# honglianghe/CDNet

Hardware: AMD Instinct MI355X
Metric: tiles/sec (train fwd+bwd+Adam), 256x256 (higher is better)
Workload: dtype fp32

## Files before the change

### cdnet_amd/_lib.py

```python
import ctypes as C
import os

_HERE = os.path.dirname(os.path.abspath(__file__))
LIB_PATH = os.environ.get('CDNET_LIB_PATH') or os.path.join(_HERE, 'libcdnet_hip.so')

_vp, _i, _sz, _f, _u = C.c_void_p, C.c_int, C.c_size_t, C.c_float, C.c_uint

class WgradReduceDesc(C.Structure):
    _fields_ = [('slab', C.c_void_p), ('dw', C.c_void_p)] + [(n, C.c_int) for n in (
        'ksplit', 'npar', 'ci_blocks', 'co_blocks', 'taps', 'CI', 'CO', 'Csrc_real', 'Cin_real', 'src_coff', 'Cout', 'mode', 'block0', 'blocks')]


SIGNATURES = {
    'cdnet_abi_version': (_i, []),
    'cdnet_abi_sizeof': (_sz, [C.c_char_p]),
    'cdnet_last_error': (C.c_char_p, []),
    'cdnet_build_info': (C.c_char_p, []),
    'cdnet_spin': (_i, [_i, _vp]),
    'cdnet_box_copy': (_i, [_vp, _vp, _sz, _vp]),
    'cdnet_box_mfma': (_i, [_vp, _vp, _vp, _i, _i, _i, _vp]),
    'cdnet_ddm_codes': (_i, [_vp, _i, _i, _i, _i, _vp, _i, _i, _vp, _vp, _vp]),
    'cdnet_ddm_normalize': (_i, [_vp, _vp, _i, _i, _i, _vp, _vp]),
    'cdnet_probmaps': (_i, [_vp, _vp, _i, _i, _i, _i, _vp, _vp, _vp]),
    'cdnet_tta_boost_argmax': (_i, [_vp, _vp, _vp, _vp, _i, _i, _vp, _i, _i, _vp, _vp, _vp, _vp, _vp, _vp]),
    'cdnet_fuse_sum': (_i, [_vp, _i, _i, _i, _i, _i, _i, _vp, _i, _i, _vp]),
    'cdnet_upsample_bilinear_backward': (_i, [_vp, _i, _i, _i, _i, _i, _i, _i, _i, _vp, _vp]),
    'cdnet_s2d_to_nhwc': (_i, [_vp, _i, _i, _i, _i, _vp, _vp]),
    'cdnet_fuse_sum_f32': (_i, [_vp, _i, _i, _i, _i, _i, _i, _vp, _i, _i, _vp]),
    'cdnet_upsample_bilinear_backward_f32': (_i, [_vp, _i, _i, _i, _i, _i, _i, _i, _i, _vp, _vp]),
    'cdnet_s2d_to_nhwc_f32': (_i, [_vp, _i, _i, _i, _i, _vp, _vp]),
    'cdnet_bn_backward_stats': (_i, [_vp, _vp, _vp, _vp, _vp, _sz, _vp, _vp]),
    'cdnet_bn_backward_apply': (_i, [_vp, _vp, _vp, _vp]),
    'cdnet_bn_backward_finalize': (_i, [_vp, _vp, _vp, _vp, _vp, _i, _vp, _vp]),
    'cdnet_conv_ws_eligible': (_i, [_vp]),
    'cdnet_grad_sum': (_i, [_vp, _i, _vp, C.c_longlong, _i, _vp, _vp]),
    'cdnet_grad_sum_f32': (_i, [_vp, _i, _vp, C.c_longlong, _i, _vp, _vp]),
    'cdnet_label_pair_histogram': (_i, [_vp, _vp, _i, _i, _i, _i, _vp, _vp, _vp, _vp, _vp, _vp]),
    'cdnet_remap_label': (_i, [_vp, _i, _i, _i, _vp, _vp, _vp, _vp]),
    'cdnet_label_areas': (_i, [_vp, _i, _i, _i, _vp, _vp, _vp]),
    'cdnet_label_apply': (_i, [_vp, _i, _i, _i, _vp, _vp, _vp]),
    'cdnet_label_csr_workspace_bytes': (_sz, [_i]),
    'cdnet_label_csr': (_i, [_vp, _i, _i, _i, _vp, _sz, _vp, _vp, _vp, _vp, _vp]),
    'cdnet_hausdorff_tile_pixels': (_i, []),
    'cdnet_hausdorff_chunk_pixels': (_i, []),
    'cdnet_hausdorff_pairs': (_i, [_vp] * 8 + [_i, _i, _i, _vp, _i, _vp, _i, _vp, _vp, _vp]),
    'cdnet_watershed_workspace_bytes': (_sz, [_i, _i, _i]),
    'cdnet_watershed_process': (_i, [_vp, _i, _i, _i, _i, _vp, _sz, _vp, _vp, _vp, _vp]),
    'cdnet_fill_label_process': (_i, [_vp, _i, _i, _i, _i, _vp, _sz, _vp, _vp]),
    'cdnet_label_process': (_i, [_vp, _i, _i, _i, _i, _vp, _sz, _vp, _vp]),
    'cdnet_instance_redilate_workspace_bytes': (_sz, [_i, _i, _i, _i]),
    'cdnet_instance_redilate': (_i, [_vp, _i, _i, _i, _i, _i, _vp, _sz, _vp, _vp, _vp]),
    'cdnet_instance_redilate_lds_rows': (_i, []),
    'cdnet_instance_redilate_lds_cols': (_i, []),
    'cdnet_label_count': (_i, [_vp, _i, _i, _i, _vp, _vp, _vp, _vp]),
    'cdnet_tile_postproc_workspace_bytes': (_sz, [_i, _i, _i, _i]),
    'cdnet_tile_postproc': (_i, [_vp, _vp, _vp, _i, _i, _i, _i, _vp, _i, _i, _i, _i, _vp, _sz] + [_vp] * 10),
    'cdnet_cc_workspace_bytes': (_sz, [_i, _i, _i]),
    'cdnet_cc_chain': (_i, [_vp, _i, _i, _i, _i, _i, _i, _vp, _sz, _vp, _vp, _vp, _vp, _vp, _vp]),
    'cdnet_mask_views_argmax': (_i, [_vp, _i, _i, _i, _vp, _i, _i, _vp, _vp, _vp]),
    'cdnet_tile_mask_postproc_workspace_bytes': (_sz, [_i, _i, _i, _i]),
    'cdnet_tile_mask_postproc': (_i, [_vp, _i, _i, _i, _i, _i, _i, _vp, _sz] + [_vp] * 8),
    'cdnet_dilate_labels': (_i, [_vp, _i, _i, _i, _i, _vp, _vp]),
    'cdnet_conv_packed_weight_elems': (_sz, [_i] * 6),
    'cdnet_pack_conv_weights': (_i, [_vp, _vp] + [_i] * 7 + [_vp]),
    'cdnet_pack_conv_weights_scaled': (_i, [_vp, _vp, _vp] + [_i] * 7 + [_vp]),
    'cdnet_pack_batch_table_bytes': (_sz, [_i]),
    'cdnet_pack_conv_weights_batch': (_i, [_vp, _i, _vp, _sz, _i, _vp]),
    'cdnet_conv_forward': (_i, [_vp, _vp]),
    'cdnet_src_materialize': (_i, [_vp, _i, _i, _i, _vp, _vp]),
    'cdnet_input_pack': (_i, [_vp, _i, _i, _i, _i, _vp, _vp]),
    'cdnet_input_pack_f32': (_i, [_vp, _i, _i, _i, _i, _vp, _vp]),
    'cdnet_bn_fold_eval': (_i, [_vp, _vp, _vp, _vp, _vp, _f, _i, _vp, _vp, _vp]),
    'cdnet_bn_finalize_train': (_i, [_vp, _i, _i, _f, _vp, _vp, _vp, _f, _f, _vp, _vp, _vp, _vp, _vp, _vp, _vp]),
    'cdnet_dam_head_forward': (_i, [_vp, _vp, _vp, _vp, _i, _i, _i, _vp, _vp, _vp, _vp]),
    'cdnet_final_conv1x1': (_i, [_vp, _vp, _vp, _i, _i, _i, _i, _vp, _vp]),
    'cdnet_bias_grad_workspace_floats': (_sz, [_i]),
    'cdnet_bias_grad': (_i, [_vp, _sz, _i, _vp, _sz, _vp, _vp]),
    'cdnet_bias_grad_f32': (_i, [_vp, _sz, _i, _vp, _sz, _vp, _vp]),
    'cdnet_final_conv1x1_backward_workspace_floats': (_sz, []),
    'cdnet_final_conv1x1_backward': (_i, [_vp, _vp, _vp, _i, _i, _i, _i, _vp, _vp, _sz, _vp, _vp, _vp]),
    'cdnet_conv_wgrad_slab_floats': (_sz, [_i] * 6),
    'cdnet_conv_backward_weight': (_i, [_vp, _i, _i, _i, _vp] + [_i] * 9 + [_vp, _vp, _i, _vp]),
    'cdnet_wgrad_reduce_desc_fill': (_i, [_i] * 9 + [_vp, _vp, _i, _i, _vp]),
    'cdnet_wgrad_reduce_batch': (_i, [_vp, _i, _i, _vp]),
    'cdnet_bn_backward_workspace_floats': (_sz, [_i]),
    'cdnet_bn_backward': (_i, [_vp, _vp, _vp, _vp, _vp, _sz, _vp, _vp, _vp]),
    'cdnet_dam_head_backward_workspace_floats': (_sz, [_i, _i, _i]),
    'cdnet_dam_head_backward': (_i, [_vp] * 7 + [_i, _i, _i, _vp, _vp, _vp, _vp, _sz, _vp, _vp]),
    'cdnet_dam_head_backward_fused_blocks': (_i, []),
    'cdnet_dam_head_backward_fused_scratch_bytes': (_i, []),
    'cdnet_dam_head_backward_fused_workspace_floats': (_sz, []),
    'cdnet_dam_head_backward_fused': (_i, [_vp] * 7 + [_i, _i, _i, _vp, _vp, _vp, _vp, _sz, _vp, _vp]),
    'cdnet_dam_loss_workspace_floats': (_sz, [_i, _i]),
    'cdnet_dam_loss': (_i, [_vp] * 7 + [_i, _i, _i, _i, _vp, _sz, _vp, _vp, _vp, _vp, _vp]),
    'cdnet_dam_loss_classes_workspace_floats': (_sz, [_i, _i, _i]),
    'cdnet_dam_loss_classes': (_i, [_vp] * 7 + [_i, _i, _i, _i, _i, _vp, _sz, _vp, _vp, _vp, _vp, _vp]),
    'cdnet_dam_loss_terms': (_i, [_vp] * 7 + [_i, _i, _i, _i, _i, _vp, _sz, _vp, _vp, _vp, _vp, _vp, _u]),
    'cdnet_mask_loss_workspace_floats': (_sz, [_i, _i]),
    'cdnet_mask_loss': (_i, [_vp, _vp, _vp, _i, _i, _i, _u, _vp, _sz, _vp, _vp, _vp]),
    'cdnet_variance_loss_workspace_bytes': (_sz, [_i, _i, _i, _i]),
    'cdnet_variance_loss': (_i, [_vp, _vp, _i, _i, _i, _i, _i, _f, _vp, _sz, _vp, _vp, _vp, _vp, _vp, _vp]),
    'cdnet_boundary_loss_workspace_bytes': (_sz, [_i, _i, _i, _i, _i]),
    'cdnet_boundary_loss': (_i, [_vp, _vp, _i, _i, _i, _i, _i, _f, _vp, _sz, _vp, _vp, _vp, _vp]),
    'cdnet_boundary_loss_scratch_bytes': (_i, []),
    'cdnet_dam_val_sums_workspace_floats': (_sz, [_i, _i]),
    'cdnet_dam_val_sums': (_i, [_vp] * 8 + [_i, _i, _i, _vp, _sz, _vp, _vp]),
    'cdnet_dam_val_sums_classes_workspace_floats': (_sz, [_i, _i, _i]),
    'cdnet_dam_val_sums_classes': (_i, [_vp] * 8 + [_i, _i, _i, _i, _vp, _sz, _vp, _vp]),
    'cdnet_adam_step': (_i, [_vp, _vp, _vp, _vp, _sz, _f, _f, _f, _f, _f, _i, _f, _vp]),
    'cdnet_moment_step': (_i, [_vp, _vp, _vp, _vp, _vp, _sz, C.c_double, C.c_double, _f, _i, _i, _f, _f, _f, _f, _i, _f, _vp]),
    'cdnet_sgd_step': (_i, [_vp, _vp, _vp, _sz, _f, _f, _f, _i, _f, _vp]),
    'cdnet_window_pack': (_i, [_vp] + [_i] * 9 + [_vp, _vp]),
    'cdnet_window_pack_f32': (_i, [_vp] + [_i] * 9 + [_vp, _vp]),
    'cdnet_window_stitch': (_i, [_vp] + [_i] * 9 + [_vp, _vp]),
    'cdnet_label_encoding_workspace_bytes': (_sz, [_i, _i, _i, _i]),
    'cdnet_label_encoding_instances_workspace_bytes': (_sz, [_i, _i, _i, _i]),
    'cdnet_label_encoding_instances': (_i, [_vp, _i, _i, _i, _i, _vp, _vp, _vp, _sz, _vp, _vp, _vp, _vp, _vp, _vp]),
    'cdnet_augment_workspace_bytes': (_sz, [_i, _i, _i]),
    'cdnet_augment_batch': (_i, [_vp, _vp, _i, _i, _vp, _vp, _sz, _vp, _vp, _vp, _i, _vp, _vp, _vp]),
    'cdnet_augment_geo_workspace_bytes': (_sz, [_i, _i, _i, _i]),
    'cdnet_augment_batch_geo': (_i, [_vp, _vp, _vp, _vp, _i, _i, _i, _vp, _vp, _sz, _vp, _vp, _vp, _i, _vp, _vp, _vp]),
    'cdnet_label_encoding': (_i, [_vp, _i, _i, _i, _i, _vp, _vp, _vp, _sz, _vp, _vp, _vp, _vp, _vp, _vp]),
    'cdnet_weight_map_radius': (_i, [C.c_double, C.c_double]),
    'cdnet_weight_map': (_i, [_vp, _i, _i, C.c_double, C.c_double, _vp, _vp]),
}

_lib = None


class CdnetHipError(RuntimeError):
    pass


def load():
    global _lib
    if _lib is not None:
        return _lib
    import torch
    if not os.path.exists(LIB_PATH):
        raise CdnetHipError('libcdnet_hip.so is not built: run `python -m cdnet_amd.csrc.build` '
                            '(or __graft_entry__.build()). There is no CPU fallback.')
    lib = C.CDLL(LIB_PATH)
    for name, (res, args) in SIGNATURES.items():
        fn = getattr(lib, name)
        fn.restype = res
        fn.argtypes = args
    if lib.cdnet_abi_version() != 5:
        raise CdnetHipError('ABI version mismatch (libcdnet_hip.so is version %d, this binding 5): rebuild with python -m cdnet_amd.csrc.build' % lib.cdnet_abi_version())
    _lib = lib
    return lib


def check(status, what=''):
    if status != 0:
        msg = load().cdnet_last_error().decode(errors='replace')
        raise CdnetHipError('%s failed (code %d): %s' % (what, status, msg))


def call(name, *args):
    check(getattr(load(), name)(*args), name)


def entry(name, f32):
    return name + '_f32' if f32 else name


_RAW_STREAM = None


# ... 18 lines not shown
```

### cdnet_amd/csrc/bn_bwd.hip

```cpp
#include "train_util.h"

using namespace cdnet;

namespace {

struct GradIn {
    const unsigned short *g;
    int Hg, Wg;
    int oy, ox;
    int pooled;
    int coff, cstride;
};

struct BnBwdArgs {
    const unsigned short *raw;
    const unsigned short *res;
    int f16;
    const float *scale, *shift;
    int relu;
    const float *mean, *invstd;
    GradIn gin[3];
    int ngin;
    int N, H, W, C;
    float *partial;
// ... 429 lines not shown
                const float v = fmaf(x[q][j], sc[j], sh[j]);
                a[q] = relu ? fmaxf(v, 0.f) : v;
            }
            int bi = 0;
            float best = a[0];
#pragma unroll
            for (int q = 1; q < 4; ++q)
                if (ok[q] && a[q] > best) { best = a[q]; bi = q; }
            const float gpool = pok ? gv[j] : 0.f;
#pragma unroll
            for (int q = 0; q < 4; ++q) {
                const float pt = (bi == q) ? gpool : 0.f;
                float gsum;
                if (NF == 0) gsum = 0.f + pt;
                else if (NF == 1) gsum = (0.f + (kp == 0 ? pt : g[q][0][j])) + (kp == 0 ? g[q][0][j] : pt);
                else gsum = ((0.f + (kp == 0 ? pt : g[q][0][j])) + (kp == 0 ? g[q][0][j] : (kp == 1 ? pt : g[q][NF - 1][j]))) +
                            (kp == 2 ? pt : g[q][NF - 1][j]);
                const float dz = (!ok[q] || (relu && !(a[q] > 0.f))) ? 0.f : gsum;
                const float xh = (x[q][j] - mu[j]) * is[j];
                if (APPLY) o[q][j] = k1[j] * (dz - k2[j] - xh * k3[j]);
                else { s1[j] += dz; s2[j] = fmaf(dz, xh, s2[j]); }
            }
        }
        if (APPLY) {
#pragma unroll
            for (int q = 0; q < 4; ++q)
                if (ok[q]) *reinterpret_cast<bn_f32x4 *>(draw + (size_t)pix[q] * A.C + c0) = o[q];
        }
    }
    if (!APPLY) bn_write_partial<4>(A.partial, A.C, VPP, s1, s2);
}

template <bool F32, bool APPLY>
__global__ __launch_bounds__(256) void bn_bwd_generic_kernel(BnBwdArgs A) {
    const int VPP = A.C / 8;
    const int slot = (int)threadIdx.x % VPP, c0 = slot * 8;
    float sc[8], sh[8], mu[8], is[8], k1[8], k2[8], k3[8], s1[8], s2[8];
    bn_load_const(A, c0, APPLY, sc, sh, mu, is, k1, k2, k3);
#pragma unroll
    for (int j = 0; j < 8; ++j) { s1[j] = 0.f; s2[j] = 0.f; }
    const unsigned HW = (unsigned)(A.H * A.W), npix = (unsigned)A.N * HW;
    const unsigned ppb = 256 / VPP;
    const unsigned step = gridDim.x * ppb;
    for (unsigned p0 = first_pixel(ppb, VPP); p0 < npix; p0 += step * BN_U) {
        float dz[BN_U][8], xh[BN_U][8];
#pragma unroll
        for (int u = 0; u < BN_U; ++u) {
            const unsigned p = p0 + u * step;
            if (p < npix) dz8_at<F32>(A, p, HW, c0, sc, sh, mu, is, dz[u], xh[u]);
            else if (!APPLY) {
#pragma unroll
                for (int j = 0; j < 8; ++j) { dz[u][j] = 0.f; xh[u][j] = 0.f; }
            }
        }
#pragma unroll
        for (int u = 0; u < BN_U; ++u) {
            const unsigned p = p0 + u * step;
            if (!APPLY) {
#pragma unroll
                for (int j = 0; j < 8; ++j) { s1[j] += dz[u][j]; s2[j] = fmaf(dz[u][j], xh[u][j], s2[j]); }
                continue;
            }
            if (p >= npix) continue;
            float o32[8];
#pragma unroll
            for (int j = 0; j < 8; ++j) o32[j] = k1[j] * (dz[u][j] - k2[j] - xh[u][j] * k3[j]);
            if (F32) {
                if (A.draw) stf8(A.draw, (size_t)p * A.C + c0, o32);
                if (A.dz_out) stf8(A.dz_out, (size_t)p * A.C + c0, dz[u]);
                continue;
            }
            V16 o, z;
#pragma unroll
            for (int j = 0; j < 8; ++j) { o.h[j] = f2bf(o32[j]); z.h[j] = f2bf(dz[u][j]); }
            if (A.draw) *reinterpret_cast<uint4 *>(A.draw + (size_t)p * A.C + c0) = o.u;
            if (A.dz_out) *reinterpret_cast<uint4 *>(A.dz_out + (size_t)p * A.C + c0) = z.u;
        }
    }
    if (!APPLY) bn_write_partial<8>(A.partial, A.C, VPP, s1, s2);
}

__global__ __launch_bounds__(256) void bn_bwd_finalize_kernel(const float *__restrict__ partial, int nb, int C, float M, const float *gamma,
                                                              const float *invstd, float *dgamma, float *dbeta, float *k1, float *k2,
                                                              float *k3) {
    __shared__ double s_a[256], s_b[256];
    const int c = blockIdx.x;
    const int lane = threadIdx.x;
    double s1 = 0.0, s2 = 0.0;
    for (int b = lane; b < nb; b += 256) { s1 += (double)partial[((size_t)b * 2) * C + c]; s2 += (double)partial[((size_t)b * 2 + 1) * C + c]; }
    s_a[lane] = s1; s_b[lane] = s2;
    __syncthreads();
#pragma unroll
    for (int o = 128; o > 0; o >>= 1) {
        if (lane < o) { s_a[lane] += s_a[lane + o]; s_b[lane] += s_b[lane + o]; }
        __syncthreads();
    }
    s1 = s_a[0]; s2 = s_b[0];
    if (lane == 0) {
        if (dbeta) dbeta[c] = (float)s1;
        if (dgamma) dgamma[c] = (float)s2;
        k1[c] = gamma[c] * invstd[c];
        k2[c] = (float)(s1 / M);
        k3[c] = (float)(s2 / M);
    }
}

__global__ void bn_ktab_copy_kernel(const float *scale, const float *shift, const float *mean, const float *invstd, int C, float *ktab) {
    const int c = blockIdx.x * blockDim.x + threadIdx.x;
    if (c < C) { ktab[c] = scale[c]; ktab[C + c] = shift[c]; ktab[2 * C + c] = mean[c]; ktab[3 * C + c] = invstd[c]; }
}

}

static int fill_bn_args(const cdnet_bn_bwd_args *a, BnBwdArgs &A, const char *who) {
    CDNET_REQUIRE(a && a->raw, "%s: null pointer", who);
    CDNET_REQUIRE(a->C % 8 == 0 && a->C >= 8 && a->C <= 2048 , "%s: C=%d unsupported", who, a->C);
    CDNET_REQUIRE(a->ngin >= 1 && a->ngin <= 3, "%s: ngin=%d", who, a->ngin);
    A.raw = a->raw; A.res = a->res; A.f16 = a->f16; A.scale = a->scale; A.shift = a->shift; A.relu = a->relu;
    A.mean = a->mean; A.invstd = a->invstd;
    for (int k = 0; k < 3; ++k) {
        A.gin[k].g = a->gin[k].g; A.gin[k].Hg = a->gin[k].Hg; A.gin[k].Wg = a->gin[k].Wg;
        A.gin[k].oy = a->gin[k].oy; A.gin[k].ox = a->gin[k].ox; A.gin[k].pooled = a->gin[k].pooled;
        A.gin[k].coff = a->gin[k].coff; A.gin[k].cstride = a->gin[k].cstride ? a->gin[k].cstride : a->C;
        if (k < a->ngin) CDNET_REQUIRE(a->gin[k].g, "%s: null gradient input %d", who, k);
    }
    A.ngin = a->ngin; A.N = a->N; A.H = a->H; A.W = a->W; A.C = a->C;
    A.partial = nullptr; A.k1 = A.k2 = A.k3 = nullptr; A.draw = nullptr; A.dz_out = nullptr;
    return CDNET_OK;
}

enum BnPath { BN_WINDOW, BN_FLAT, BN_GENERIC };
struct BnPlan {
    BnPath path;
    bool f32;
    int nb;
    int kp, nflat;
    bool flat_sources;
};

static size_t bn_npix(const BnBwdArgs &A) { return (size_t)A.N * A.H * A.W; }

static BnPlan bn_plan_plain(const BnBwdArgs &A) {
    const bool f32 = A.f16 == 2;
    return BnPlan{BN_FLAT, f32, bn_grid(bn_npix(A), A.C, f32 ? 4 : 8, BN_U), 0, 0, true};
}

static BnPlan bn_plan(const BnBwdArgs &A, const void *draw, const void *dz_out) {
    bool simple = true;
    int npool = 0, kp = 0, nflat = 0;
    for (int k = 0; k < A.ngin; ++k) {
        const GradIn &g = A.gin[k];
        const bool same = !g.pooled && g.oy == 0 && g.ox == 0 && g.Hg == A.H && g.Wg == A.W;
        simple = simple && same;
        if (g.pooled) { ++npool; kp = k; }
        else if (same) ++nflat;
    }
    const bool window = npool == 1 && nflat == A.ngin - 1 && nflat <= 2 && A.mean && A.scale && !A.res && draw && !dz_out;
    const bool flat = !window && simple && A.mean && A.scale && draw && ((A.res != nullptr) == (dz_out != nullptr));
    const bool f32 = A.f16 == 2, fits32 = A.C <= 1024;
    BnPlan P{BN_GENERIC, f32, 0, kp, nflat, flat};
    if (window && (!f32 || (fits32 && A.shift && A.invstd))) P.path = BN_WINDOW;
    else if (flat && (!f32 || fits32)) P.path = BN_FLAT;
    const int V = f32 && P.path != BN_GENERIC ? 4 : 8;
    P.nb = window ? bn_grid((size_t)A.N * ((A.H + 1) / 2) * ((A.W + 1) / 2), A.C, V, 1) : bn_grid(bn_npix(A), A.C, V, BN_U);
    return P;
}

template <bool APPLY>
static void launch(const BnPlan &P, const BnBwdArgs &A, hipStream_t st) {
    auto window = [&](auto nf) {
        constexpr int NF = decltype(nf)::value;
        if (P.f32) bn_bwd_window32_kernel<NF, APPLY><<<P.nb, 256, 0, st>>>(A, P.kp);
        else bn_bwd_window_kernel<NF, APPLY><<<P.nb, 256, 0, st>>>(A, P.kp);
    };
    auto flat = [&](auto ng, auto res) {
        constexpr int NG = decltype(ng)::value;
        constexpr bool RES = decltype(res)::value;
        if (P.f32) bn_bwd_flat32_kernel<NG, RES, APPLY><<<P.nb, 256, 0, st>>>(A);
        else bn_bwd_flat_kernel<NG, RES, APPLY><<<P.nb, 256, 0, st>>>(A);
    };
    using std::integral_constant;
    using std::true_type;
    using std::false_type;
    switch (P.path) {
        case BN_WINDOW:
            if (P.nflat == 0) window(integral_constant<int, 0>{});
            else if (P.nflat == 1) window(integral_constant<int, 1>{});
            else window(integral_constant<int, 2>{});
            break;
        case BN_FLAT:
            switch (A.ngin * 2 + (A.res ? 1 : 0)) {
                case 2: flat(integral_constant<int, 1>{}, false_type{}); break;
                case 3: flat(integral_constant<int, 1>{}, true_type{}); break;
                case 4: flat(integral_constant<int, 2>{}, false_type{}); break;
                case 5: flat(integral_constant<int, 2>{}, true_type{}); break;
                case 6: flat(integral_constant<int, 3>{}, false_type{}); break;
                default: flat(integral_constant<int, 3>{}, true_type{}); break;
            }
            break;
        case BN_GENERIC:
            if (P.f32) bn_bwd_generic_kernel<true, APPLY><<<P.nb, 256, 0, st>>>(A);
            else bn_bwd_generic_kernel<false, APPLY><<<P.nb, 256, 0, st>>>(A);
            break;
    }
}

static void bn_finalize(const BnBwdArgs &A, const float *partial, int nb, const float *gamma, float *dgamma, float *dbeta, float *k,
                        hipStream_t st) {
    bn_bwd_finalize_kernel<<<A.C, 256, 0, st>>>(partial, nb, A.C, (float)bn_npix(A), gamma, A.invstd, dgamma, dbeta, k, k + A.C, k + 2 * A.C);
}

static void bn_set_coeffs(BnBwdArgs &A, const float *k) { A.k1 = k; A.k2 = k + A.C; A.k3 = k + 2 * A.C; }

static BnBwdArgs bn_dz_as_source(const BnBwdArgs &A, const unsigned short *dz) {
    BnBwdArgs B = A;
    B.ngin = 1;
    B.gin[0].g = dz; B.gin[0].Hg = A.H; B.gin[0].Wg = A.W; B.gin[0].oy = 0; B.gin[0].ox = 0; B.gin[0].pooled = 0;
    B.gin[0].coff = 0; B.gin[0].cstride = A.C;
    B.res = nullptr; B.relu = 0; B.dz_out = nullptr;
    return B;
}

extern "C" int cdnet_bn_backward(const cdnet_bn_bwd_args *a, const float *gamma, float *dgamma, float *dbeta, float *workspace,
                                 size_t workspace_floats, uint16_t *draw, uint16_t *dz_out, void *stream) {
    BnBwdArgs A;
    int rc = fill_bn_args(a, A, "cdnet_bn_backward");
    if (rc) return rc;
    hipStream_t st = (hipStream_t)stream;
    const size_t npix = bn_npix(A);
    CDNET_REQUIRE(npix * (size_t)A.C < ((size_t)1 << 32) && npix < ((size_t)1 << 31), "cdnet_bn_backward: tensor too large for 32-bit pixel indexing");
    const BnPlan P = bn_plan(A, draw, dz_out);
    CDNET_REQUIRE(A.relu != 2 || (P.flat_sources && A.res), "cdnet_bn_backward: relu = 2 (mask from the stored output) needs same-size gradient sources and res");
    static const bool dz_reuse = !(getenv("CDNET_BN_DZ_REUSE") && atoi(getenv("CDNET_BN_DZ_REUSE")) == 0);
    const bool reuse = dz_reuse && P.path == BN_FLAT && A.mean && A.res && dz_out;
    A.draw = draw;
    A.rev = 1;
    if (A.mean) {
        CDNET_REQUIRE(gamma && A.invstd && workspace, "cdnet_bn_backward: BatchNorm layer needs gamma/invstd/workspace");
        const size_t need = (size_t)P.nb * 2 * A.C + 3 * (size_t)A.C;
        if (workspace_floats < need) { set_error("cdnet_bn_backward: workspace %zu < %zu floats", workspace_floats, need); return CDNET_E_WORKSPACE; }
        A.partial = workspace;
        A.dz_out = dz_reuse ? dz_out : nullptr;
        float *k = workspace + (size_t)P.nb * 2 * A.C;
        launch<false>(P, A, st);
        bn_finalize(A, A.partial, P.nb, gamma, dgamma, dbeta, k, st);
        bn_set_coeffs(A, k);
    }
    A.dz_out = dz_out;
    launch<true>(P, reuse ? bn_dz_as_source(A, dz_out) : A, st);
    return check_launch("cdnet_bn_backward");
}

static bool bn_plain_case(const BnBwdArgs &A, bool masked = false) {
    const GradIn &g = A.gin[0];
    return A.ngin == 1 && !g.pooled && g.oy == 0 && g.ox == 0 && g.Hg == A.H && g.Wg == A.W && A.mean && A.scale && A.shift && A.invstd && !A.res &&
           (A.relu == 1 || (masked && A.relu == 0)) && (g.cstride == 0 || g.cstride == A.C) && g.coff == 0;
}

extern "C" int cdnet_bn_backward_stats(const cdnet_bn_bwd_args *a, const float *gamma, float *dgamma, float *dbeta, float *workspace,
                                       size_t workspace_floats, float *ktab, void *stream) {
    BnBwdArgs A;
    int rc = fill_bn_args(a, A, "cdnet_bn_backward_stats");
    if (rc) return rc;
    CDNET_REQUIRE(bn_plain_case(A) && A.f16 != 2 && gamma && workspace && ktab, "cdnet_bn_backward_stats: plain 16-bit case only (one same-size gradient, BatchNorm + ReLU, no residual)");
    hipStream_t st = (hipStream_t)stream;
    const size_t npix = bn_npix(A);
    CDNET_REQUIRE(npix * (size_t)A.C < ((size_t)1 << 32) && npix < ((size_t)1 << 31), "cdnet_bn_backward_stats: tensor too large for 32-bit pixel indexing");
    const BnPlan P = bn_plan_plain(A);
    const size_t need = (size_t)P.nb * 2 * A.C;
    if (workspace_floats < need) { set_error("cdnet_bn_backward_stats: workspace %zu < %zu floats", workspace_floats, need); return CDNET_E_WORKSPACE; }
    A.partial = workspace;
    A.rev = 0;
    bn_ktab_copy_kernel<<<cdiv(A.C, 256), 256, 0, st>>>(A.scale, A.shift, A.mean, A.invstd, A.C, ktab);
    launch<false>(P, A, st);
    bn_finalize(A, A.partial, P.nb, gamma, dgamma, dbeta, ktab + 4 * A.C, st);
    return check_launch("cdnet_bn_backward_stats");
}

extern "C" int cdnet_bn_backward_finalize(const cdnet_bn_bwd_args *a, const float *gamma, float *dgamma, float *dbeta, const float *partial,
                                          int nb, float *ktab, void *stream) {
    BnBwdArgs A;
    int rc = fill_bn_args(a, A, "cdnet_bn_backward_finalize");
    if (rc) return rc;
    CDNET_REQUIRE(bn_plain_case(A) && gamma && partial && ktab && nb >= 1, "cdnet_bn_backward_finalize: plain case only");
    bn_finalize(A, partial, nb, gamma, dgamma, dbeta, ktab + 4 * A.C, (hipStream_t)stream);
    return check_launch("cdnet_bn_backward_finalize");
}

extern "C" int cdnet_bn_backward_apply(const cdnet_bn_bwd_args *a, const float *ktab, uint16_t *draw, void *stream) {
    BnBwdArgs A;
    int rc = fill_bn_args(a, A, "cdnet_bn_backward_apply");
    if (rc) return rc;
    CDNET_REQUIRE(bn_plain_case(A, true) && ktab && draw, "cdnet_bn_backward_apply: plain case only");
    CDNET_REQUIRE(A.f16 != 2 || A.C <= 1024, "cdnet_bn_backward_apply(f32): C=%d > 1024", A.C);
    A.rev = 1;
    A.draw = draw;
    bn_set_coeffs(A, ktab + 4 * A.C);
    launch<true>(bn_plan_plain(A), A, (hipStream_t)stream);
    return check_launch("cdnet_bn_backward_apply");
}

extern "C" size_t cdnet_bn_backward_workspace_floats(int C) { return (size_t)BN_MAX_BLOCKS * 2 * C + 3 * (size_t)C; }
```

### cdnet_amd/csrc/conv32ws.hip

```cpp
#include <type_traits>
#include "common.h"
#include "conv_args.h"
#include "launch.h"
#include <stdlib.h>

using namespace cdnet;


typedef __attribute__((ext_vector_type(8))) __bf16 bf16x8;
typedef __attribute__((ext_vector_type(2))) __bf16 bf16x2;
typedef __attribute__((ext_vector_type(16))) float f32x16;
typedef __attribute__((ext_vector_type(2))) float f32x2;
typedef unsigned u32x4 __attribute__((ext_vector_type(4)));
typedef float f32x4 __attribute__((ext_vector_type(4)));

namespace {

__device__ __forceinline__ void split8(const float *v, u32x4 &hi, u32x4 &lo) {
#pragma unroll
    for (int k = 0; k < 4; ++k) {
        const f32x2 x = {v[2 * k], v[2 * k + 1]};
        const bf16x2 h = __builtin_convertvector(x, bf16x2);
        const unsigned hb = __builtin_bit_cast(unsigned, h);
        float d0, d1;
        asm("v_sub_f32 %0, %1, %2" : "=v"(d0) : "v"(x[0]), "v"(__builtin_bit_cast(float, hb << 16)));
        asm("v_sub_f32 %0, %1, %2" : "=v"(d1) : "v"(x[1]), "v"(__builtin_bit_cast(float, hb & 0xffff0000u)));
        const f32x2 df = {d0, d1};
        const bf16x2 l = __builtin_convertvector(df, bf16x2);
        hi[k] = hb;
        lo[k] = __builtin_bit_cast(unsigned, l);
    }
}

__device__ __forceinline__ void glds_piece(const void *gbase, unsigned lane_bytes, unsigned lds_dst) {
    unsigned keep;
    asm volatile("s_mov_b32 %0, m0\n\ts_mov_b32 m0, %3\n\ts_nop 0\n\tglobal_load_lds_dwordx4 %1, %2\n\ts_mov_b32 m0, %0"
                 : "=&s"(keep) : "v"(lane_bytes), "s"(gbase), "s"(lds_dst) : "memory");
}

template <int BN>
struct Ws32Lds {
    static constexpr int TH = 16, TW = 16, CK = 16, TAPS = 9;
    static constexpr int PSTR = 32;
    static constexpr int NPIX = (TH + 2) * (TW + 2);
    static constexpr int A_PLANE = NPIX * PSTR;
    static constexpr int A_SLOT = 2 * A_PLANE;
    static constexpr int B_PLANE = TAPS * CK * BN * 2;
    static constexpr int W_SLOT = 2 * B_PLANE;
    static constexpr int STATS_BYTES = 2 * 4 * 2 * BN * 4;
    static constexpr int RAW_Q = 4 * 32 * 32 * 4;
    __host__ __device__ static int bytes(int ctot, bool bns = false) { return 2 * A_SLOT + 2 * W_SLOT + STATS_BYTES + 2 * ((ctot + 7) / 8 * 8) * 4 + (bns ? 2 * RAW_Q : 0); }
};

template <int BN, int XF, bool STATS, bool BNS = false, int NCS = 0, bool MIX = false, bool POOL = false>
__global__ __launch_bounds__(512) void conv_ws32_kernel(ConvArgs A) {
    static_assert(!BNS || (BN == 64 && !STATS), "the BatchNorm-backward statistics epilogue serves 64-channel blocks of backward-data launches");
    static_assert(!MIX || (!STATS && !BNS && NCS == 0), "one-tap chunks: inference launches with at least four nine-tap chunks");
    static_assert(!POOL || (!STATS && !BNS && !MIX && NCS == 0), "fused max-pool: plain inference launches with at least four chunks");
    using L = Ws32Lds<BN>;
    constexpr int TH = 16, TW = 16, CK = 16, TAPS = 9, PSTR = L::PSTR, HW_ = TW + 2, NPIX = L::NPIX;
    constexpr int NPW = BN / 32, MPW = 2;
    constexpr int VPP = CK / 8, NA = (NPIX * VPP + 255) / 256;
    const int NCH = A.nchunk;
    const int n0c = A.src[0].C / CK;
    constexpr int W1_SLOT = 2 * CK * BN * 2;

    extern __shared__ __attribute__((aligned(16))) unsigned char smem[];
    unsigned char *lds_a = smem;
    unsigned char *lds_w = smem + 2 * L::A_SLOT;
    float *s_stats = reinterpret_cast<float *>(lds_w + 2 * L::W_SLOT);
    float *s_xf = reinterpret_cast<float *>(lds_w + 2 * L::W_SLOT + L::STATS_BYTES);
    const int xfs_ = ((A.src[0].C + (A.nsrc > 1 ? A.src[1].C : 0)) + 7) / 8 * 8;
    unsigned char *lds_raw = lds_w + 2 * L::W_SLOT + L::STATS_BYTES + 2 * xfs_ * 4;

    const int tid = threadIdx.x, lane = tid & 63;
    const int wave = __builtin_amdgcn_readfirstlane(tid >> 6);
    const int c0n = A.src[0].C, ctot = c0n + (A.nsrc > 1 ? A.src[1].C : 0);
    const int xfs = (ctot + 7) / 8 * 8;
    const int cout_tile = blockIdx.y;
    const int cout0 = cout_tile * BN;

    const int tiles_x = A.W / TW, tiles_y = A.H / TH;
    const int tiles_img = tiles_x * tiles_y;
    const int T = A.N * tiles_img;
    int t_lo, t_hi;
    {
        const int G = (int)gridDim.x, b = (int)blockIdx.x;
        if ((G & 7) == 0) {
            const int xcd = b & 7, idx = b >> 3, nw = G >> 3;
            const long long x0 = (long long)T * xcd / 8, x1 = (long long)T * (xcd + 1) / 8;
            t_lo = (int)(x0 + (x1 - x0) * idx / nw);
            t_hi = (int)(x0 + (x1 - x0) * (idx + 1) / nw);
        } else {
            t_lo = (int)((long long)T * b / G);
            t_hi = (int)((long long)T * (b + 1) / G);
        }
    }
    const int ntl = t_hi - t_lo;
    const int S = ntl * NCH;
    if (S == 0) return;

    if (wave >= 4) {
        const int ptid = tid - 256, pw = wave - 4;
        const int slot = ptid % VPP;
        f32x4 pa[2][NA][2];
        unsigned eo[2][NA];
        int hyx[NA], doff[NA];
#pragma unroll
        for (int i = 0; i < NA; ++i) {
            const int pix = (ptid + i * 256) / VPP;
            const int hy = pix / HW_, hx = pix - hy * HW_;
            hyx[i] = ptid + i * 256 < NPIX * VPP ? ((hy << 8) | hx) : 0x1f1f;
            doff[i] = pix * PSTR + ((slot ^ (hy & 1)) * 16);
        }
        const unsigned src_bytes0 = (unsigned)A.N * A.src[0].Hs * (A.src[0].row_stride ? A.src[0].row_stride : A.src[0].Ws * A.src[0].C) * 4u;
        const unsigned src_bytes1 = A.nsrc > 1 ? (unsigned)A.N * A.src[1].Hs * (A.src[1].row_stride ? A.src[1].row_stride : A.src[1].Ws * A.src[1].C) * 4u : 0u;
        const __amdgpu_buffer_rsrc_t rsx0 = __builtin_amdgcn_make_buffer_rsrc(const_cast<unsigned short *>(A.src[0].x), 0, (int)src_bytes0, 0x00020000);
        const __amdgpu_buffer_rsrc_t rsx1 = __builtin_amdgcn_make_buffer_rsrc(const_cast<unsigned short *>(A.nsrc > 1 ? A.src[1].x : A.src[0].x), 0, (int)src_bytes1, 0x00020000);
        const __amdgpu_buffer_rsrc_t rsr0 = __builtin_amdgcn_make_buffer_rsrc(const_cast<unsigned short *>(A.src[0].res ? A.src[0].res : A.src[0].x), 0, (int)src_bytes0, 0x00020000);
        const __amdgpu_buffer_rsrc_t rsr1 = __builtin_amdgcn_make_buffer_rsrc(const_cast<unsigned short *>(A.nsrc > 1 && A.src[1].res ? A.src[1].res : A.src[0].x), 0, (int)src_bytes1, 0x00020000);
        auto bload = [](__amdgpu_buffer_rsrc_t r, unsigned voff) -> f32x4 {
            return __builtin_bit_cast(f32x4, __builtin_amdgcn_raw_buffer_load_b128(r, (int)voff, 0, 0));
        };
        auto bad_mask = [](int lo, int hi) -> unsigned {
            lo = lo < 0 ? 0 : (lo > 31 ? 31 : lo);
            hi = hi < lo ? lo : (hi > 31 ? 31 : hi);
            return ~(((1u << hi) - 1u) & ~((1u << lo) - 1u));
        };
        int ik = 0, ic = 0, in_, iy0, ix0;
        {
            in_ = t_lo / tiles_img;
            const int r = t_lo - in_ * tiles_img, ty = r / tiles_x;
            iy0 = ty * TH; ix0 = (r - ty * tiles_x) * TW;
        }
        int o_n = in_, o_y0 = iy0, o_x0 = ix0;
        int s_n = 0, s_y0 = 0, s_x0 = 0;
        bool s_ok = false;
        int kt = 0;
        int ck = 0;
        unsigned ge[NA];
        const int n0 = A.src[0].C / CK;
// ... 133 lines not shown
        auto stream_sync = [](auto n_c) {
            constexpr int N = decltype(n_c)::value;
            asm volatile("" ::: "memory");
            __builtin_amdgcn_s_waitcnt((N & 15) | (7 << 4) | (0 << 8) | ((N >> 4) << 14));
            __builtin_amdgcn_s_barrier();
            asm volatile("" ::: "memory");
        };
        using NHL = std::integral_constant<int, 2 * NA>;
        using I0 = std::integral_constant<int, 0>;
        using I1 = std::integral_constant<int, 1>;
        issue(I0{});
        issue(I1{});
        for (int c = ptid; c < ctot; c += 256) {
            const ConvSrc &Sx = c < c0n ? A.src[0] : A.src[1];
            const int cc = c < c0n ? c : c - c0n;
            s_xf[c] = Sx.scale ? Sx.scale[cc] : 1.f;
            s_xf[xfs + c] = Sx.shift ? Sx.shift[cc] : 0.f;
        }
        __syncthreads();
        dma_w(0);
        commit(I0{}, 0);
        issue(I0{});
        stream_sync(NHL{});
        auto interval = [&](auto rc, int k) {
            constexpr int R = decltype(rc)::value;
            dma_w(R);
            if (BNS) {
                if (kt == NCH - 1) dma_raw(0, o_n, o_y0, o_x0);
                else if (kt < 3 && s_ok) dma_raw(kt + 1, s_n, s_y0, s_x0);
            }
            commit(rc, k + 1);
            asm volatile("" ::: "memory");
            issue(rc);
            stream_sync(NHL{});
            if (BNS && ++kt == NCH) {
                kt = 0;
                s_n = o_n; s_y0 = o_y0; s_x0 = o_x0; s_ok = true;
                o_x0 += TW;
                if (o_x0 >= A.W) { o_x0 = 0; o_y0 += TH; if (o_y0 >= A.H) { o_y0 = 0; ++o_n; } }
            }
        };
        for (int k = 0; k < S; k += 2) {
            interval(I1{}, k);
            interval(I0{}, k + 1);
        }
        __syncthreads();
        return;
    }

    __syncthreads();
    const int wm = wave;
    const int half = lane >> 5, l31 = lane & 31;
    int abase[MPW][2];
#pragma unroll
    for (int mi = 0; mi < MPW; ++mi) {
        const int m = (wm * MPW + mi) * 32 + l31;
#pragma unroll
        for (int par = 0; par < 2; ++par) abase[mi][par] = ((m / TW) * HW_ + m % TW) * PSTR + ((half ^ ((m / TW + par) & 1)) * 16);
    }
    auto tpar = [](int t) { return (t / 3) & 1; };
    auto toff = [](int t) { return ((t / 3) * HW_ + (t % 3)) * PSTR; };
    const int bbase = half * BN * 16 + l31 * 16;
    f32x16 accA[MPW][NPW], accB[MPW][NPW];
    const unsigned pix_b = (unsigned)A.out_cstride * 4u;
    const unsigned l_off = (unsigned)(4 * half) * pix_b + (unsigned)l31 * 4u;
    char *const out_b = reinterpret_cast<char *>(reinterpret_cast<float *>(A.out) + A.out_coff + cout0);
    int p_n, p_y0, p_x0;
    {
        p_n = t_lo / tiles_img;
        const int r = t_lo - p_n * tiles_img, ty = r / tiles_x;
        p_y0 = ty * TH; p_x0 = (r - ty * tiles_x) * TW;
    }
    float e_osc[NPW], e_osh[NPW];
    bool e_ok[NPW];
#pragma unroll
    for (int ni = 0; ni < NPW; ++ni) {
        const int co = cout0 + ni * 32 + l31;
        const bool cok = co < A.Cout;
        e_ok[ni] = cok && !(A.debug & 8);
        e_osc[ni] = (!BNS && A.oscale && cok) ? A.oscale[co] : 1.f;
        e_osh[ni] = BNS ? 0.f : fmaf((A.bias && cok) ? A.bias[co] : 0.f, e_osc[ni], (A.oshift && cok) ? A.oshift[co] : 0.f);
    }
    const bool orelu = A.orelu != 0;
    float b_sc[NPW], b_sh[NPW], b_mu[NPW], b_is[NPW], b_s1[NPW], b_s2[NPW], b_x = 0.f;
    if (BNS) {
#pragma unroll
        for (int ni = 0; ni < NPW; ++ni) {
            const int co = cout0 + ni * 32 + l31;
            b_sc[ni] = A.oscale[co]; b_sh[ni] = A.oshift[co]; b_mu[ni] = A.eres_scale[co]; b_is[ni] = A.eres_shift[co];
            b_s1[ni] = 0.f; b_s2[ni] = 0.f;
            e_osc[ni] = 1.f; e_osh[ni] = 0.f;
        }
    }
    const unsigned char *raw_w = lds_raw + wave * 4096 + (4 * half) * 128 + l31 * 4;
    auto bns_read = [&](int buf, int r) { b_x = *reinterpret_cast<const float *>(raw_w + buf * L::RAW_Q + ((r & 3) + 8 * (r >> 2)) * 128); };
    auto bns_acc = [&](const f32x16 (&P)[MPW][NPW], int e, float x) {
        const int b_ = e / 16, r = e % 16, mi = b_ / NPW, ni = b_ % NPW;
        const float act = fmaf(x, b_sc[ni], b_sh[ni]);
        const float dz = act > 0.f ? P[mi][ni][r] : 0.f;
        b_s1[ni] += dz;
        b_s2[ni] = fmaf(dz, (x - b_mu[ni]) * b_is[ni], b_s2[ni]);
    };

    float st_sum = 0.f, st_sq = 0.f;
    auto stat_elem = [&](const f32x16 (&P)[MPW][NPW], int s_, int par) {
        const int ni = s_ / (MPW * 16), mi = (s_ / 16) % MPW, r = s_ % 16;
        if (mi == 0 && r == 0) { st_sum = 0.f; st_sq = 0.f; }
        const float v = P[mi][ni][r];
        st_sum += v;
        st_sq = fmaf(v, v, st_sq);
        if (mi == MPW - 1 && r == 15) {
            float *sp = s_stats + par * (4 * 2 * BN);
            const float a = st_sum + __shfl_xor(st_sum, 32), b2 = st_sq + __shfl_xor(st_sq, 32);
            if (half == 0) {
                sp[(wave * 2 + 0) * BN + ni * 32 + l31] = a;
                sp[(wave * 2 + 1) * BN + ni * 32 + l31] = b2;
            }
        }
    };
    unsigned s_col[8];
#pragma unroll
    for (int c = 0; c < 8; ++c) s_col[c] = (unsigned)(c & 3) * pix_b + (unsigned)(c >> 2) * 8u * pix_b;
    char *row_base[4];
    const unsigned ppix_b = (unsigned)A.Cout * 4u;
    const unsigned pl_off = (unsigned)(2 * half) * ppix_b + (unsigned)l31 * 4u;
    char *const pool_b = POOL ? reinterpret_cast<char *>(reinterpret_cast<float *>(A.pool_out) + cout0) : nullptr;
    char *prow_base[2] = {nullptr, nullptr};
    float pl_t0 = 0.f, pl_t1 = 0.f;
    auto set_row_bases = [&]() {
        char *t0 = out_b + ((size_t)(p_n * A.H + p_y0 + wm * 4) * A.W + p_x0) * pix_b;
#pragma unroll
        for (int r = 0; r < 4; ++r) row_base[r] = t0 + (size_t)r * A.W * pix_b;
        if (POOL) {
            char *q0 = pool_b + ((size_t)(p_n * (A.H >> 1) + ((p_y0 + wm * 4) >> 1)) * (A.W >> 1) + (p_x0 >> 1)) * ppix_b;
            prow_base[0] = q0;
            prow_base[1] = q0 + (size_t)(A.W >> 1) * ppix_b;
        }
    };
    auto img_elem = [&](const f32x16 (&P)[MPW][NPW], int e) {
        const int b_ = e / 16, r = e % 16, mi = b_ / NPW, ni = b_ % NPW;
        float v = fmaf(P[mi][ni][r], e_osc[ni], e_osh[ni]);
        if (orelu) v = fmaxf(v, 0.f);
        if (e_ok[ni]) {
            char *sb = row_base[mi * 2 + (r >> 3)] + (s_col[((r >> 2) & 1) * 4 + (r & 3)] + (unsigned)(ni * 128));
            asm volatile("" : "+s"(sb));
            __builtin_nontemporal_store(v, (__attribute__((address_space(1))) float *)((__attribute__((address_space(1))) char *)sb + l_off));
        }
    };
    auto pool_sub = [&](const f32x16 (&P)[MPW][NPW], int u, int sub) {
        const int b_ = u / 4, k = u % 4, mi = b_ / NPW, ni = b_ % NPW, r0 = 2 * k;
        if (sub == 0) pl_t0 = fmaxf(fmaf(P[mi][ni][r0], e_osc[ni], e_osh[ni]), fmaf(P[mi][ni][r0 + 1], e_osc[ni], e_osh[ni]));
        else if (sub == 1) pl_t1 = fmaxf(fmaf(P[mi][ni][r0 + 8], e_osc[ni], e_osh[ni]), fmaf(P[mi][ni][r0 + 9], e_osc[ni], e_osh[ni]));
        else {
            float v = fmaxf(pl_t0, pl_t1);
            if (orelu) v = fmaxf(v, 0.f);
            if (e_ok[ni]) {
                char *sb = prow_base[mi] + ((unsigned)(((r0 >> 2) & 1) * 4 + ((r0 & 3) >> 1)) * ppix_b + (unsigned)(ni * 128));
                asm volatile("" : "+s"(sb));
                *(__attribute__((address_space(1))) float *)((__attribute__((address_space(1))) char *)sb + pl_off) = v;
            }
        }
    };
    constexpr int NEL = MPW * NPW * 16;

    int stats_tile = -1, stats_par = 0;
    auto flush_stats = [&]() {
        if (STATS && stats_tile >= 0 && tid < 2 * BN) {
            const int which = tid / BN, col = tid % BN;
            const float *sp = s_stats + stats_par * (4 * 2 * BN);
            float v = 0.f;
#pragma unroll
            for (int w4 = 0; w4 < 4; ++w4) v += sp[(w4 * 2 + which) * BN + col];
            const int co = cout0 + col;
            if (co < A.Cout) A.stats[((size_t)stats_tile * 2 + which) * A.Cout + co] = v;
        }
        stats_tile = -1;
    };

    auto interval_nt = [&](auto nt_c, auto first_c, auto epi_c, f32x16 (&C)[MPW][NPW], const f32x16 (&P)[MPW][NPW], int par, int sl) {
        constexpr int NT = decltype(nt_c)::value;
        constexpr int BPL = NT * CK * BN * 2;
        constexpr bool FIRST = decltype(first_c)::value;
        constexpr int EPI = decltype(epi_c)::value;
        static_assert(NT == 9 || (EPI == 0 && !FIRST), "one-tap chunks come after the nine-tap ones");
        if (A.debug & 1) return;
        bf16x8 ah[2][MPW], al[2][MPW], bh[2][NPW], bl[2][NPW];
        const unsigned char *la = lds_a + sl * L::A_SLOT, *lw = lds_w + sl * L::W_SLOT;
        constexpr int NRD = 2 * MPW + 2 * NPW;
        auto request_one = [&](int t, int i) {
            const int s2 = t & 1;
            const int tq = NT == 9 ? t : 4;
            const int ao = toff(tq), bo = bbase + t * 2 * BN * 16;
            if (i == 0) al[s2][0] = *reinterpret_cast<const bf16x8 *>(la + L::A_PLANE + abase[0][tpar(tq)] + ao);
            else if (i == 1) bh[s2][0] = *reinterpret_cast<const bf16x8 *>(lw + bo);
            else if (i == 2) ah[s2][0] = *reinterpret_cast<const bf16x8 *>(la + abase[0][tpar(tq)] + ao);
            else if (i == 3) bl[s2][0] = *reinterpret_cast<const bf16x8 *>(lw + BPL + bo);
            else if (NPW == 2 && i == 4) bh[s2][NPW - 1] = *reinterpret_cast<const bf16x8 *>(lw + bo + 512);
            else if (NPW == 2 && i == 5) bl[s2][NPW - 1] = *reinterpret_cast<const bf16x8 *>(lw + BPL + bo + 512);
            else if (i == NRD - 2) al[s2][1] = *reinterpret_cast<const bf16x8 *>(la + L::A_PLANE + abase[1][tpar(tq)] + ao);
            else if (i == NRD - 1) ah[s2][1] = *reinterpret_cast<const bf16x8 *>(la + abase[1][tpar(tq)] + ao);
        };
        auto gap = [&](int t, int m, int g) {
            if (t + 1 < NT && m < NRD) request_one(t + 1, m);
            if (EPI != 0) {
                constexpr int QEL = NEL / 4;
                if ((EPI == 1 || EPI == 5 || EPI == 6) && STATS && g % 3 == 1 && 2 * (g / 3) + 1 < NEL) { stat_elem(P, 2 * (g / 3), par); stat_elem(P, 2 * (g / 3) + 1, par); }
                if (EPI <= 4 && g % 6 == 3 && g / 6 < QEL) img_elem(P, (EPI - 1) * QEL + g / 6);
                if (POOL && EPI <= 4 && g % 6 == 5 && g / 6 < 12) pool_sub(P, (EPI - 1) * 4 + (g / 6) / 3, (g / 6) % 3);
                if (EPI == 5 && g % 3 != 1 && 2 * (g / 3) + (g % 3 == 2 ? 1 : 0) < NEL) img_elem(P, 2 * (g / 3) + (g % 3 == 2 ? 1 : 0));
                if ((EPI == 6 || EPI == 7) && g % 3 == 0 && g / 3 < NEL / 2) img_elem(P, (EPI - 6) * (NEL / 2) + g / 3);
                if (BNS && EPI <= 4) {
                    if (g == 1) bns_read((EPI - 1) & 1, 0);
                    if (g % 6 == 0 && g >= 6 && g / 6 - 1 < QEL) {
                        const int i = g / 6 - 1;
                        const float x = b_x;
                        if (i + 1 < QEL) bns_read((EPI - 1) & 1, i + 1);
                        bns_acc(P, (EPI - 1) * QEL + i, x);
                    }
                }
            }
            __builtin_amdgcn_sched_barrier(0);
        };
        static_assert(NT != 9 || (3 * (NEL / 2) <= TAPS * MPW * NPW * 3 && 6 * (NEL / 4) <= TAPS * MPW * NPW * 3 && 2 * (TAPS * MPW * NPW) >= NEL),
                      "the deferred epilogue fits the MFMA gaps of an interval");
#pragma unroll
        for (int i = 0; i < NRD; ++i) request_one(0, i);
        __builtin_amdgcn_sched_barrier(0);
#pragma unroll
        for (int t = 0; t < NT; ++t) {
#pragma unroll
            for (int mi = 0; mi < MPW; ++mi)
#pragma unroll
                for (int ni = 0; ni < NPW; ++ni) {
                    const int m0 = (mi * NPW + ni) * 3, g0 = t * MPW * NPW * 3 + m0;
                    if (FIRST && t == 0) {
                        const f32x16 z = {0.f, 0.f, 0.f, 0.f, 0.f, 0.f, 0.f, 0.f, 0.f, 0.f, 0.f, 0.f, 0.f, 0.f, 0.f, 0.f};
                        C[mi][ni] = __builtin_amdgcn_mfma_f32_32x32x16_bf16(al[t & 1][mi], bh[t & 1][ni], z, 0, 0, 0);
                    } else {
                        C[mi][ni] = __builtin_amdgcn_mfma_f32_32x32x16_bf16(al[t & 1][mi], bh[t & 1][ni], C[mi][ni], 0, 0, 0);
                    }
                    gap(t, m0, g0);
                    C[mi][ni] = __builtin_amdgcn_mfma_f32_32x32x16_bf16(ah[t & 1][mi], bl[t & 1][ni], C[mi][ni], 0, 0, 0);
                    gap(t, m0 + 1, g0 + 1);
                    C[mi][ni] = __builtin_amdgcn_mfma_f32_32x32x16_bf16(ah[t & 1][mi], bh[t & 1][ni], C[mi][ni], 0, 0, 0);
                    gap(t, m0 + 2, g0 + 2);
                }
        }
    };
    auto interval = [&](auto first_c, auto epi_c, f32x16 (&C)[MPW][NPW], const f32x16 (&P)[MPW][NPW], int par, int sl) {
        interval_nt(std::integral_constant<int, 9>{}, first_c, epi_c, C, P, par, sl);
    };
    using F_ = std::false_type;
    using T_ = std::true_type;
    using E0 = std::integral_constant<int, 0>;
    using E1 = std::integral_constant<int, 1>;
    using E2 = std::integral_constant<int, 2>;
    using E3 = std::integral_constant<int, 3>;
    using E4 = std::integral_constant<int, 4>;
    using E5 = std::integral_constant<int, 5>;
    using E6 = std::integral_constant<int, 6>;
    using E7 = std::integral_constant<int, 7>;
    auto tile_step = [&](auto has_prev, f32x16 (&C)[MPW][NPW], const f32x16 (&P)[MPW][NPW], int j, int q) {
        constexpr bool HP = decltype(has_prev)::value;
        const int par = (j + 1) & 1;
        if (HP) set_row_bases();
        if constexpr (NCS != 0) {
            if constexpr (NCS == 1) { if (HP) interval(T_{}, E5{}, C, P, par, q & 1); else interval(T_{}, E0{}, C, P, par, q & 1); }
            else { if (HP) interval(T_{}, E6{}, C, P, par, q & 1); else interval(T_{}, E0{}, C, P, par, q & 1); }
            if (HP && STATS) { stats_tile = t_lo + j - 1; stats_par = par; }
            __syncthreads();
            flush_stats();
            if constexpr (NCS == 2) {
                if (HP) interval(F_{}, E7{}, C, P, par, (q + 1) & 1); else interval(F_{}, E0{}, C, P, par, (q + 1) & 1);
                __syncthreads();
                if (NCH == 3) {
                    interval(F_{}, E0{}, C, P, par, (q + 2) & 1);
                    __syncthreads();
                }
            }
        } else {
            if (HP) interval(T_{}, E1{}, C, P, par, q & 1); else interval(T_{}, E0{}, C, P, par, q & 1);
            if (HP && STATS) { stats_tile = t_lo + j - 1; stats_par = par; }
            __syncthreads();
            flush_stats();
            if (HP) interval(F_{}, E2{}, C, P, par, (q + 1) & 1); else interval(F_{}, E0{}, C, P, par, (q + 1) & 1);
            __syncthreads();
            if (HP) interval(F_{}, E3{}, C, P, par, (q + 2) & 1); else interval(F_{}, E0{}, C, P, par, (q + 2) & 1);
            __syncthreads();
            if (HP) interval(F_{}, E4{}, C, P, par, (q + 3) & 1); else interval(F_{}, E0{}, C, P, par, (q + 3) & 1);
            __syncthreads();
            for (int i = 4; i < NCH; ++i) {
// ... 28 lines not shown
            for (int b_ = 0; b_ < NEL / 16; ++b_) {
                const int mi = b_ / NPW, ni = b_ % NPW;
                float xs[16];
#pragma unroll
                for (int r = 0; r < 16; ++r) xs[r] = rw[((size_t)(mi * 2 + (r >> 3)) * A.W + ((r >> 2) & 1) * 8 + (r & 3)) * A.Cout + ni * 32];
#pragma unroll
                for (int r = 0; r < 16; ++r) bns_acc(P, b_ * 16 + r, xs[r]);
            }
            float *row = A.stats + (size_t)(blockIdx.x * 4 + wave) * 2 * A.Cout + cout0 + l31;
#pragma unroll
            for (int ni = 0; ni < NPW; ++ni) {
                const float a = b_s1[ni] + __shfl_xor(b_s1[ni], 32), b2 = b_s2[ni] + __shfl_xor(b_s2[ni], 32);
                if (half == 0) { row[ni * 32] = a; row[A.Cout + ni * 32] = b2; }
            }
        }
        __syncthreads();
        flush_stats();
    };

    __syncthreads();
    tile_step(F_{}, accA, accB, 0, 0);
    int j = 1, q = NCH;
    for (; j + 1 < ntl; j += 2, q += 2 * NCH) {
        tile_step(T_{}, accB, accA, j, q);
        tile_step(T_{}, accA, accB, j + 1, q + NCH);
    }
    const bool tail = j < ntl;
    if (tail) tile_step(T_{}, accB, accA, j, q);
    if (S & 1) __syncthreads();
    if (tail) serial_epilogue(accB, j); else serial_epilogue(accA, ntl - 1);
}

}

namespace cdnet {

template <int BN>
static int try_launch_ws32(const ConvArgs &A, hipStream_t st, bool dry_run) {
    using L = Ws32Lds<BN>;
    int ctot = 0;
    for (int i = 0; i < A.nsrc; ++i) {
        if (A.src[i].pool) return -1;
        ctot += A.src[i].C;
        if (!in_mover_reach(A.src[i], A.N, 4)) return -1;
    }
    const bool bns = A.ws == 2;
    const bool mix = A.taps1 == 1 && A.nsrc == 2;
    if (mix && (bns || A.stats || A.src[0].C < 64)) return -1;
    if (bns && (BN != 64 || A.Cout % 64 != 0 || !A.eres || !A.oscale || !A.oshift || !A.eres_scale || !A.eres_shift || !A.stats || A.bias ||
                A.orelu || A.out_cstride != A.Cout || A.out_coff)) return -1;
    const int smem = L::bytes(ctot, bns);
    if (smem > 160 * 1024) return -1;
    const int T = (A.W / 16) * (A.H / 16) * A.N;
    int n_cu = 0;
    if (const int rc = cu_count(&n_cu)) return rc;
    const int ctiles = cdiv(A.Cout, BN);
    const int Gmax = n_cu / ctiles > 0 ? n_cu / ctiles : 1;
    if (!(A.debug & CONV_DBG_PERSIST_SMALL) && (long long)T * A.nchunk < 16LL * Gmax) return -1;
    bool all_plain = true, all_fast = true;
    for (int i = 0; i < A.nsrc; ++i) {
        const ConvSrc &s = A.src[i];
        all_plain = all_plain && !s.scale && !s.relu && !s.res;
        all_fast = all_fast && s.scale && s.shift && s.relu == 1 && !s.res;
    }
    dim3 grid(persistent_grid(n_cu, ctiles, T, bns ? 256 : 0, A.debug >> CONV_DBG_GRID_SHIFT), ctiles, 1);
    auto launch_n = [&](auto xf_c, auto st_c, auto ncs_c) -> int {
        constexpr int XF = decltype(xf_c)::value;
        constexpr bool STATS = decltype(st_c)::value;
        constexpr int NCS = decltype(ncs_c)::value;
        return launch_lds<conv_ws32_kernel<BN, XF, STATS, false, NCS>>(grid, 512, 160 * 1024, smem, st, "hipFuncSetAttribute(conv_ws32)", "conv_ws32_kernel", A);
    };
    auto launch = [&](auto xf_c, auto st_c) -> int {
        constexpr int XF = decltype(xf_c)::value;
        if (A.nchunk >= 4) return launch_n(xf_c, st_c, std::integral_constant<int, 0>{});
        if constexpr (BN == 64 && XF != 2) {
            if (A.nchunk == 1) return launch_n(xf_c, st_c, std::integral_constant<int, 1>{});
            return launch_n(xf_c, st_c, std::integral_constant<int, 2>{});
        }
        return -1;
    };
    const int xf = all_plain ? 0 : (all_fast ? 1 : 2);
    if (A.nchunk < 4 && (BN != 64 || xf == 2)) return -1;
    const bool pool = A.pool_out != nullptr;
    if (pool && (BN != 64 || bns || mix || A.stats || A.nchunk < 4 || xf != 0 || !A.orelu || A.out_coff || A.out_cstride != A.Cout)) return -1;
    if (dry_run) return CDNET_OK;
    if (bns) {
        if constexpr (BN == 64) {
            return with_int<0, 1, 2>(xf, [&](auto xf_c) {
                return launch_lds<conv_ws32_kernel<64, decltype(xf_c)::value, false, true>>(grid, 512, 160 * 1024, smem, st, "hipFuncSetAttribute(conv_ws32 bns)", "conv_ws32_kernel(bns)", A);
            });
        }
        return -1;
    }
    if (mix) {
        return with_int<0, 2>(xf == 1 ? 2 : xf, [&](auto xf_c) {
            return launch_lds<conv_ws32_kernel<BN, decltype(xf_c)::value, false, false, 0, true>>(grid, 512, 160 * 1024, smem, st, "hipFuncSetAttribute(conv_ws32 mix)", "conv_ws32_kernel(mix)", A);
        });
    }
    if (!pool) return with_bool(A.stats != nullptr, [&](auto st_c) { return with_int<0, 1, 2>(xf, [&](auto xf_c) { return launch(xf_c, st_c); }); });
    if constexpr (BN == 64) {
        return launch_lds<conv_ws32_kernel<64, 0, false, false, 0, false, true>>(grid, 512, 160 * 1024, smem, st, "hipFuncSetAttribute(conv_ws32 pool)", "conv_ws32_kernel(pool)", A);
    }
    return -1;
}

int conv_forward_f32_ws(const ConvArgs &A, hipStream_t st, bool dry_run) {
    if (A.debug & CONV_DBG_ONE_TILE) return -1;
    if (A.taps != 9 || A.npar != 1 || A.ostride != 1 || A.tile != 16 || A.CK != 16 || (A.eres && A.ws != 2) || (A.ws && A.ws != 2)) return -1;
    if (A.taps1 != 0 && A.taps1 != 9 && !(A.taps1 == 1 && A.nsrc == 2)) return -1;
    if (A.H % 16 != 0 || A.W % 16 != 0 || A.nchunk < (A.ws == 2 ? 4 : 1)) return -1;
    if (A.BN == 64) return try_launch_ws32<64>(A, st, dry_run);
    if (A.BN == 32) return try_launch_ws32<32>(A, st, dry_run);
    return -1;
}

}
```

### cdnet_amd/csrc/dam_loss.hip

```cpp
#include "loss_util.h"
#include "launch.h"
#include "stage16.h"

using namespace cdnet;

namespace {

template <int ND> struct LossLay {
    static constexpr int PW = 9, TW = 9 + ND, SS = 9 + 2 * ND, SN = 9 + 3 * ND, SP = 9 + 4 * ND, SC = 9 + 5 * ND, SUMS = SC + 6;
    static constexpr int COEF = 6 + 4 * ND;
    static constexpr int TPB = ND > 9 ? 128 : 256;
};
template <int ND> __device__ __forceinline__ int dnext(int i) { return i == ND - 1 ? 1 : i + 1; }
template <int ND> __device__ __forceinline__ int dprev(int i) { return i == 1 ? ND - 1 : i - 1; }

struct LossIn {
    const float *mask, *point, *dirn;
    const unsigned char *label, *dirlab;
    const unsigned short *point_t;
    const unsigned char *weight;
    const int *single;
    int B, P;
    int quirk0;
    unsigned terms;
};

__global__ __launch_bounds__(1024) void loss_single_kernel(const unsigned char *dirlab, const unsigned char *label, int P, int nd, int *single, int *err) {
    __shared__ int s_min[16], s_max[16], s_lmax[16];
    const unsigned char *d = dirlab + (size_t)blockIdx.x * P;
    const unsigned char *l = label + (size_t)blockIdx.x * P;
    int mn = 255, mx = 0, lm = 0;
    const int tid = threadIdx.x;
    const bool vec = (P % 16 == 0) && ((reinterpret_cast<size_t>(d) | reinterpret_cast<size_t>(l)) % 16 == 0);
    if (vec) {
        const uint4 *d4 = reinterpret_cast<const uint4 *>(d), *l4 = reinterpret_cast<const uint4 *>(l);
        for (int i = tid; i < P / 16; i += 1024) {
            const uint4 dv = d4[i], lv = l4[i];
            const unsigned dw[4] = {dv.x, dv.y, dv.z, dv.w}, lw[4] = {lv.x, lv.y, lv.z, lv.w};
#pragma unroll
            for (int k = 0; k < 4; ++k)
#pragma unroll
                for (int b8 = 0; b8 < 4; ++b8) {
                    const int v = (dw[k] >> (8 * b8)) & 0xff, w = (lw[k] >> (8 * b8)) & 0xff;
                    mn = v < mn ? v : mn; mx = v > mx ? v : mx; lm = w > lm ? w : lm;
                }
        }
    } else {
        for (int i = tid; i < P; i += 1024) {
            int v = d[i]; mn = v < mn ? v : mn; mx = v > mx ? v : mx;
            v = l[i]; lm = v > lm ? v : lm;
        }
    }
#pragma unroll
    for (int m = 1; m < 64; m <<= 1) {
        const int a = __shfl_xor(mn, m), b2 = __shfl_xor(mx, m), c = __shfl_xor(lm, m);
        mn = a < mn ? a : mn; mx = b2 > mx ? b2 : mx; lm = c > lm ? c : lm;
    }
    if ((tid & 63) == 0) { s_min[tid >> 6] = mn; s_max[tid >> 6] = mx; s_lmax[tid >> 6] = lm; }
    __syncthreads();
    if (tid == 0) {
        for (int i = 1; i < 16; ++i) {
            mn = s_min[i] < mn ? s_min[i] : mn; mx = s_max[i] > mx ? s_max[i] : mx; lm = s_lmax[i] > lm ? s_lmax[i] : lm;
        }
        single[blockIdx.x] = (mn == mx) ? 1 : 0;
        if (mx > nd - 1 || lm > 2) atomicOr(err, 1);
    }
}

template <int ND>
__device__ __forceinline__ int dice_target(const LossIn &L, int b, int i) {
    if (L.single[b]) return 0;
    int t = L.dirlab[(size_t)b * L.P + i];
    t = t > ND - 1 ? ND - 1 : t;
    if (L.quirk0) return L.label[i] != 0 ? t : -1;
    return L.label[(size_t)b * L.P + i] != 0 ? t : -1;
}

template <int ND>
__global__ __launch_bounds__(LossLay<ND>::TPB) void loss_reduce_kernel(LossIn L, float *__restrict__ partial) {
    using Y = LossLay<ND>;
    constexpr int TPB = Y::TPB;
    __shared__ float acc[Y::SUMS][TPB];
    const int tid = threadIdx.x, b = blockIdx.y;
#pragma unroll
    for (int k = 0; k < Y::SUMS; ++k) acc[k][tid] = 0.f;
    const size_t ob = (size_t)b * L.P;
    for (int i = blockIdx.x * TPB + tid; i < L.P; i += gridDim.x * TPB) {
        float l3[3], p3[3], lp3[3], l9[ND], p9[ND], lp9[ND];
#pragma unroll
        for (int c = 0; c < 3; ++c) l3[c] = L.mask[((size_t)b * 3 + c) * L.P + i];
#pragma unroll
        for (int c = 0; c < ND; ++c) l9[c] = L.dirn[((size_t)b * ND + c) * L.P + i];
        softmax3(l3, p3, lp3);
        softmax_n<ND>(l9, p9, lp9);
        const float w = (L.terms & CDNET_LOSS_WMAP) ? (float)L.weight[ob + i] / 20.f : 1.f;
        int lab = L.label[ob + i], dl = L.dirlab[ob + i];
        lab = lab > 2 ? 2 : lab; dl = dl > ND - 1 ? ND - 1 : dl;
        acc[lab][tid] += p3[lab];
        acc[6 + lab][tid] += 1.f;
#pragma unroll
        for (int c = 0; c < 3; ++c) acc[3 + c][tid] += p3[c];
#pragma unroll
        for (int c = 0; c < ND; ++c) acc[Y::PW + c][tid] = fmaf(w, p9[c], acc[Y::PW + c][tid]);
        const int t = dice_target<ND>(L, b, i);
        if (t >= 0) {
            acc[Y::TW + t][tid] += w;
            acc[Y::SS + t][tid] = fmaf(w, p9[t], acc[Y::SS + t][tid]);
            if (t >= 1) {
                acc[Y::SN + t][tid] = fmaf(w, p9[dnext<ND>(t)], acc[Y::SN + t][tid]);
                acc[Y::SP + t][tid] = fmaf(w, p9[dprev<ND>(t)], acc[Y::SP + t][tid]);
            }
        }
        acc[Y::SC][tid] -= lp3[lab] * w;
        acc[Y::SC + 1][tid] -= lp9[dl] * w;
        const float dpt = L.point[ob + i] - h2f(L.point_t[ob + i]);
        acc[Y::SC + 2][tid] = fmaf(dpt, dpt, acc[Y::SC + 2][tid]);
        {
            int am = 0;
            float best = l9[0];
#pragma unroll
            for (int c = 1; c < ND; ++c) if (l9[c] > best) { best = l9[c]; am = c; }
            const bool pi = am == 1, ti = dl == 1;
            if (pi && ti) acc[Y::SC + 3][tid] += 1.f;
            if (pi && !ti) acc[Y::SC + 4][tid] += 1.f;
            if (!pi && ti) acc[Y::SC + 5][tid] += 1.f;
        }
    }
    __syncthreads();
    row_sum<TPB>(acc, tid, b, partial);
}

template <int ND>
__global__ __launch_bounds__(256) void loss_finalize_kernel(const float *__restrict__ partial, int nchunk, int B, int P,
                                                            float *__restrict__ sums, float *__restrict__ coef,
                                                            float *__restrict__ losses, const int *__restrict__ err, unsigned terms) {
    using Y = LossLay<ND>;
    constexpr int NS = Y::SUMS;
    const bool plain = !(terms & CDNET_LOSS_WMAP);
    __shared__ float s_sum[64 * NS];
    const int tid = threadIdx.x;
    for (int idx = tid; idx < B * NS; idx += 256) {
        const int b = idx / NS, k = idx % NS;
        const float s = chunk_sum<NS>(partial + (size_t)b * nchunk * NS + k, nchunk);
        s_sum[idx] = s;
        if (sums) sums[idx] = s;
    }
    __syncthreads();
    const float fB = (float)B;
    for (int b = tid; b < B; b += 256) {
        const float *S = s_sum + b * NS;
        float *cf = coef + (size_t)b * Y::COEF;
        mask_dice_coef(S, fB, cf);
        float bsum[ND];
        for (int i = 0; i < ND; ++i) bsum[i] = 0.f;
        for (int j = 0; j < ND; ++j) {
            {
                const float U = S[Y::PW + j] + S[Y::TW + j], Sij = S[Y::SS + j], m = j == 0 && !plain ? 2.f : 1.f;
                cf[6 + ND + j] = m * -2.f / (fB * (U + 1.f));
                bsum[j] += m * 2.f * (Sij + 1.f) / (fB * (U + 1.f) * (U + 1.f));
            }
            if (plain) { cf[6 + 2 * ND + j] = 0.f; cf[6 + 3 * ND + j] = 0.f; }
            else if (j >= 1) {
                const int in = dnext<ND>(j), ip = dprev<ND>(j);
                {   const float U = S[Y::PW + in] + S[Y::TW + j], Sij = S[Y::SN + j];
                    cf[6 + 2 * ND + j] = -2.f / (fB * (U + 1.f));
                    bsum[in] += 2.f * (Sij + 1.f) / (fB * (U + 1.f) * (U + 1.f)); }
                {   const float U = S[Y::PW + ip] + S[Y::TW + j], Sij = S[Y::SP + j];
                    cf[6 + 3 * ND + j] = -2.f / (fB * (U + 1.f));
                    bsum[ip] += 2.f * (Sij + 1.f) / (fB * (U + 1.f) * (U + 1.f)); }
            } else { cf[6 + 2 * ND] = 0.f; cf[6 + 3 * ND] = 0.f; }
        }
        for (int i = 0; i < ND; ++i) cf[6 + i] = bsum[i];
    }
    constexpr int T_PREV = 3 + ND, T_NEXT = T_PREV + ND - 1, NT = T_NEXT + ND - 1;
    __shared__ float s_term[NT];
    if (tid < NT) {
        int num, da, db;
        if (tid < 3) { num = tid; da = 3 + tid; db = 6 + tid; }
        else if (tid < T_PREV) { const int i = tid - 3; num = Y::SS + i; da = Y::PW + i; db = Y::TW + i; }
        else if (tid < T_NEXT) { const int i = tid - T_PREV + 1, j = dprev<ND>(i); num = Y::SN + j; da = Y::PW + i; db = Y::TW + j; }
        else { const int i = tid - T_NEXT + 1, j = dnext<ND>(i); num = Y::SP + j; da = Y::PW + i; db = Y::TW + j; }
        s_term[tid] = dice_term<NS>(s_sum, B, fB, num, da, db);
    }
    __syncthreads();
    if (tid == 0) {
        const float n = (float)B * (float)P;
        float ce = 0.f, dce = 0.f, mse = 0.f;
        for (int b = 0; b < B; ++b) { ce += s_sum[b * NS + Y::SC]; dce += s_sum[b * NS + Y::SC + 1]; mse += s_sum[b * NS + Y::SC + 2]; }
        ce /= n; dce /= n; mse /= n;
        float dice = 0.f;
        for (int c = 0; c < 3; ++c) dice += s_term[c];
        float wd = 0.f;
        for (int i = 0; i < ND; ++i) {
            if (i == 0) wd += 2.f * s_term[3];
            else wd += s_term[3 + i] - (1.f - s_term[T_PREV + i - 1]) - (1.f - s_term[T_NEXT + i - 1]);
        }
        wd /= (float)ND;
        if (plain) {
            wd = 0.f;
            for (int i = 0; i < ND; ++i) wd += s_term[3 + i];
        }
        losses[0] = (terms & CDNET_LOSS_CE) ? ce + dice + dce + wd + mse : dice + dce + wd + mse;
        losses[1] = dce; losses[2] = wd; losses[3] = mse; losses[4] = ce; losses[5] = dice;
        pixel_metrics<NS>(s_sum, Y::SC + 3, B, P, losses + 6);
        poison_on_error(err, losses, 11);
    }
}

template <int ND>
__global__ __launch_bounds__(256) void loss_grad_kernel(LossIn L, const float *__restrict__ coef, float *__restrict__ dmask,
                                                        float *__restrict__ dpoint, float *__restrict__ ddir) {
    const int b = blockIdx.y;
    const float *cf = coef + (size_t)b * LossLay<ND>::COEF;
    const float inv_n = 1.f / ((float)L.B * (float)L.P);
    const size_t ob = (size_t)b * L.P;
    for (int i = blockIdx.x * 256 + threadIdx.x; i < L.P; i += gridDim.x * 256) {
        float l3[3], p3[3], lp3[3], l9[ND], p9[ND], lp9[ND];
#pragma unroll
        for (int c = 0; c < 3; ++c) l3[c] = L.mask[((size_t)b * 3 + c) * L.P + i];
#pragma unroll
        for (int c = 0; c < ND; ++c) l9[c] = L.dirn[((size_t)b * ND + c) * L.P + i];
        softmax3(l3, p3, lp3);
        softmax_n<ND>(l9, p9, lp9);
        const float w = (L.terms & CDNET_LOSS_WMAP) ? (float)L.weight[ob + i] / 20.f : 1.f;
        int lab = L.label[ob + i], dl = L.dirlab[ob + i];
        lab = lab > 2 ? 2 : lab; dl = dl > ND - 1 ? ND - 1 : dl;
        float gp[3], dot = 0.f;
#pragma unroll
        for (int c = 0; c < 3; ++c) { gp[c] = cf[3 + c] + (c == lab ? cf[c] : 0.f); dot = fmaf(p3[c], gp[c], dot); }
#pragma unroll
        for (int c = 0; c < 3; ++c)
            dmask[((size_t)b * 3 + c) * L.P + i] = (L.terms & CDNET_LOSS_CE) ? p3[c] * (gp[c] - dot) + w * inv_n * (p3[c] - (c == lab ? 1.f : 0.f))
                                                                              : p3[c] * (gp[c] - dot);
        const int t = dice_target<ND>(L, b, i);
        float gq[ND], dotq = 0.f;
#pragma unroll
        for (int c = 0; c < ND; ++c) gq[c] = cf[6 + c];
        if (t >= 0) {
#pragma unroll
            for (int c = 0; c < ND; ++c) {
                float a = 0.f;
                if (c == t) a = cf[6 + ND + t];
                else if (t >= 1 && c == dnext<ND>(t)) a = cf[6 + 2 * ND + t];
                else if (t >= 1 && c == dprev<ND>(t)) a = cf[6 + 3 * ND + t];
                gq[c] += a;
            }
        }
#pragma unroll
        for (int c = 0; c < ND; ++c) { if (L.terms & CDNET_LOSS_WMAP) gq[c] *= w * (1.f / (float)ND); dotq = fmaf(p9[c], gq[c], dotq); }
#pragma unroll
        for (int c = 0; c < ND; ++c)
            ddir[((size_t)b * ND + c) * L.P + i] = p9[c] * (gq[c] - dotq) + w * inv_n * (p9[c] - (c == dl ? 1.f : 0.f));
        if (dpoint) dpoint[ob + i] = 2.f * inv_n * (L.point[ob + i] - h2f(L.point_t[ob + i]));
    }
}

template <int ND> struct ValLay {
    static constexpr int IQ = 10, PQ = 10 + ND, TQ = 10 + 2 * ND, VS = 10 + 3 * ND, SUMS = VS + 5;
    static constexpr int TPB = ND > 9 ? 128 : 256;
};
static_assert(ValLay<9>::SUMS == CDNET_VAL_SUMS, "cdnet_dam_val_sums row layout");

struct ValIn {
    const float *mask, *point, *dirn;
    const unsigned char *label, *dirlab, *weight;
    const unsigned short *point_t;
    int lut[17];
    int B, P;
};

template <int ND>
__global__ __launch_bounds__(ValLay<ND>::TPB) void val_sums_kernel(ValIn L, float *__restrict__ partial) {
    using Y = ValLay<ND>;
    constexpr int TPB = Y::TPB;
    __shared__ float acc[Y::SUMS][TPB];
    const int tid = threadIdx.x, b = blockIdx.y;
#pragma unroll
    for (int k = 0; k < Y::SUMS; ++k) acc[k][tid] = 0.f;
    const size_t ob = (size_t)b * L.P;
    for (int i = blockIdx.x * TPB + tid; i < L.P; i += gridDim.x * TPB) {
        float l3[3], p3[3], lp3[3], l9[ND], p9[ND], lp9[ND];
#pragma unroll
        for (int c = 0; c < 3; ++c) l3[c] = L.mask[((size_t)b * 3 + c) * L.P + i];
#pragma unroll
        for (int c = 0; c < ND; ++c) l9[c] = L.dirn[((size_t)b * ND + c) * L.P + i];
        softmax3(l3, p3, lp3);
        softmax_n<ND>(l9, p9, lp9);
        int lab = L.label[ob + i], dl = L.dirlab[ob + i];
        lab = lab > 2 ? 2 : lab; dl = dl > ND - 1 ? ND - 1 : dl;
        const float w = (float)L.weight[ob + i] / 20.f;
#pragma unroll
        for (int c = 0; c < 3; ++c) {
            acc[3 + c][tid] += p3[c];
            if (c == lab) { acc[c][tid] += p3[c]; acc[6 + c][tid] += 1.f; }
        }
        acc[9][tid] -= lp3[lab];
        p9[0] *= p3[0];
        const bool fg0 = L.label[i] != 0;
        const int tch = (fg0 && L.lut[dl] >= 0) ? L.lut[dl] : -1;
#pragma unroll
        for (int c = 0; c < ND; ++c) {
            acc[Y::PQ + c][tid] += p9[c];
            if (c == tch) { acc[Y::IQ + c][tid] += p9[c]; acc[Y::TQ + c][tid] += 1.f; }
        }
        acc[Y::VS][tid] -= w * lp9[dl];
        const float dpt = L.point[ob + i] - h2f(L.point_t[ob + i]) / 255.f;
        acc[Y::VS + 1][tid] = fmaf(dpt, dpt, acc[Y::VS + 1][tid]);
        int am = 0;
        if (l3[1] > l3[am]) am = 1;
        if (l3[2] > l3[am]) am = 2;
        const bool pi = am == 1, ti = lab == 1;
        if (pi && ti) acc[Y::VS + 2][tid] += 1.f;
        if (pi && !ti) acc[Y::VS + 3][tid] += 1.f;
        if (!pi && ti) acc[Y::VS + 4][tid] += 1.f;
    }
    __syncthreads();
    row_sum<TPB>(acc, tid, b, partial);
}

__global__ void val_sums_reduce_kernel(const float *__restrict__ partial, int nchunk, int B, int nsums, float *__restrict__ sums) {
    const int idx = blockIdx.x * blockDim.x + threadIdx.x;
    if (idx >= B * nsums) return;
    const int b = idx / nsums, k = idx % nsums;
    double s = 0.0;
    for (int ch = 0; ch < nchunk; ++ch) s += (double)partial[((size_t)b * nchunk + ch) * nsums + k];
    sums[idx] = (float)s;
}

}

static int known_classes(int direction_classes) { return direction_classes == 5 || direction_classes == 17 ? direction_classes : 9; }

template <int ND>
static size_t dam_loss_ws(int B, int P) {
    using Y = LossLay<ND>;
    const int nchunk = loss_nchunk(P, Y::TPB);
    return (size_t)B * nchunk * Y::SUMS + (size_t)B * Y::COEF + (size_t)B * Y::SUMS + 16 + (size_t)B;
}

template <int ND>
static int dam_loss_impl(LossIn L, int B, int P, float *workspace, float *losses, float *dmask, float *dpoint, float *ddir, hipStream_t st) {
    using Y = LossLay<ND>;
    const int nchunk = loss_nchunk(P, Y::TPB);
    float *partial = workspace;
    float *coef = partial + (size_t)B * nchunk * Y::SUMS;
    float *sums = coef + (size_t)B * Y::COEF;
    int *err = reinterpret_cast<int *>(sums + (size_t)B * Y::SUMS);
    int *single = reinterpret_cast<int *>(sums + (size_t)B * Y::SUMS + 16);
    if (hipMemsetAsync(err, 0, sizeof(int), st) != hipSuccess) return check_launch("cdnet_dam_loss(memset)");
    L.single = single;
    loss_single_kernel<<<B, 1024, 0, st>>>(L.dirlab, L.label, P, ND, single, err);
    loss_reduce_kernel<ND><<<dim3(nchunk, B), Y::TPB, 0, st>>>(L, partial);
    loss_finalize_kernel<ND><<<1, 256, 0, st>>>(partial, nchunk, B, P, sums, coef, losses, err, L.terms);
    if (dmask) loss_grad_kernel<ND><<<dim3(lin_grid((size_t)P, 256), B), 256, 0, st>>>(L, coef, dmask, dpoint, ddir);
    return check_launch("cdnet_dam_loss");
}

extern "C" size_t cdnet_dam_loss_classes_workspace_floats(int B, int P, int direction_classes) {
    size_t n = 0;
    with_int<5, 9, 17>(known_classes(direction_classes), [&](auto nd) { n = dam_loss_ws<decltype(nd)::value>(B, P); return CDNET_OK; });
    return n;
}
extern "C" size_t cdnet_dam_loss_workspace_floats(int B, int P) { return dam_loss_ws<9>(B, P); }

extern "C" int cdnet_dam_loss_terms(const float *mask, const float *point, const float *dirn, const uint8_t *label, const uint8_t *dirlab,
                                    const uint16_t *point_target_f16, const uint8_t *weight_u8, int B, int H, int W, int direction_classes,
                                    int quirk_sample0, float *workspace, size_t workspace_floats, float *losses, float *dmask,
                                    float *dpoint, float *ddir, void *stream, unsigned terms) {
    CDNET_REQUIRE(mask && point && dirn && label && dirlab && point_target_f16 && workspace && losses, "cdnet_dam_loss: null pointer");
    CDNET_REQUIRE((terms & ~(CDNET_LOSS_WMAP | CDNET_LOSS_CE | CDNET_LOSS_DICE)) == 0, "cdnet_dam_loss: terms %u has unknown bits", terms);
    CDNET_REQUIRE(terms & CDNET_LOSS_DICE, "cdnet_dam_loss: the DAM loss has no configuration without the dice terms (train_util_dam.py:297)");
    CDNET_REQUIRE(weight_u8 || !(terms & CDNET_LOSS_WMAP), "cdnet_dam_loss: CDNET_LOSS_WMAP needs the weight map");
    CDNET_REQUIRE(B >= 1 && B <= 64 && H > 0 && W > 0, "cdnet_dam_loss: batch %d not in [1,64]", B);
    CDNET_REQUIRE(direction_classes == 5 || direction_classes == 9 || direction_classes == 17,
                  "cdnet_dam_loss: direction_classes %d must be 5, 9 or 17 (options.py:45)", direction_classes);
    const int P = H * W;
    if (workspace_floats < cdnet_dam_loss_classes_workspace_floats(B, P, direction_classes)) { set_error("cdnet_dam_loss: workspace too small"); return CDNET_E_WORKSPACE; }
    if (dmask) CDNET_REQUIRE(dpoint && ddir, "cdnet_dam_loss: all three gradient outputs or none");
    LossIn L;
    L.mask = mask; L.point = point; L.dirn = dirn; L.label = label; L.dirlab = dirlab; L.point_t = point_target_f16;
    L.weight = weight_u8; L.single = nullptr; L.B = B; L.P = P; L.quirk0 = quirk_sample0; L.terms = terms;
    hipStream_t st = (hipStream_t)stream;
    return with_int<5, 9, 17>(direction_classes, [&](auto nd) { return dam_loss_impl<decltype(nd)::value>(L, B, P, workspace, losses, dmask, dpoint, ddir, st); });
}

extern "C" int cdnet_dam_loss_classes(const float *mask, const float *point, const float *dirn, const uint8_t *label, const uint8_t *dirlab,
                                      const uint16_t *point_target_f16, const uint8_t *weight_u8, int B, int H, int W, int direction_classes,
                                      int quirk_sample0, float *workspace, size_t workspace_floats, float *losses, float *dmask,
                                      float *dpoint, float *ddir, void *stream) {
    CDNET_REQUIRE(weight_u8, "cdnet_dam_loss: null pointer");
    return cdnet_dam_loss_terms(mask, point, dirn, label, dirlab, point_target_f16, weight_u8, B, H, W, direction_classes, quirk_sample0,
                                workspace, workspace_floats, losses, dmask, dpoint, ddir, stream,
                                CDNET_LOSS_WMAP | CDNET_LOSS_CE | CDNET_LOSS_DICE);
}

extern "C" int cdnet_dam_loss(const float *mask, const float *point, const float *dirn, const uint8_t *label, const uint8_t *dirlab,
                              const uint16_t *point_target_f16, const uint8_t *weight_u8, int B, int H, int W, int quirk_sample0,
                              float *workspace, size_t workspace_floats, float *losses, float *dmask, float *dpoint, float *ddir,
                              void *stream) {
    return cdnet_dam_loss_classes(mask, point, dirn, label, dirlab, point_target_f16, weight_u8, B, H, W, 9, quirk_sample0, workspace,
                                  workspace_floats, losses, dmask, dpoint, ddir, stream);
}

template <int ND>
static int val_sums_impl(ValIn L, int B, int P, float *workspace, float *sums, hipStream_t st) {
    using Y = ValLay<ND>;
    const int nchunk = loss_nchunk(P, Y::TPB);
    val_sums_kernel<ND><<<dim3(nchunk, B), Y::TPB, 0, st>>>(L, workspace);
    val_sums_reduce_kernel<<<cdiv(B * Y::SUMS, 256), 256, 0, st>>>(workspace, nchunk, B, Y::SUMS, sums);
    return check_launch("cdnet_dam_val_sums");
}

extern "C" size_t cdnet_dam_val_sums_classes_workspace_floats(int B, int P, int direction_classes) {
    size_t n = 0;
    with_int<5, 9, 17>(known_classes(direction_classes), [&](auto nd) {
        using Y = ValLay<decltype(nd)::value>;
        n = (size_t)B * loss_nchunk(P, Y::TPB) * Y::SUMS;
        return CDNET_OK;
    });
    return n;
}
extern "C" size_t cdnet_dam_val_sums_workspace_floats(int B, int P) { return cdnet_dam_val_sums_classes_workspace_floats(B, P, 9); }

extern "C" int cdnet_dam_val_sums_classes(const float *mask, const float *point, const float *dirn, const uint8_t *label, const uint8_t *dirlab,
                                          const uint16_t *point_target_f16, const uint8_t *weight_u8, const int *dir_rank_host,
                                          int direction_classes, int B, int H, int W, float *workspace, size_t workspace_floats, float *sums,
                                          void *stream) {
    CDNET_REQUIRE(mask && point && dirn && label && dirlab && point_target_f16 && weight_u8 && dir_rank_host && workspace && sums,
                  "cdnet_dam_val_sums: null pointer");
    CDNET_REQUIRE(B >= 1 && B <= 64 && H > 0 && W > 0, "cdnet_dam_val_sums: batch %d not in [1,64]", B);
    CDNET_REQUIRE(direction_classes == 5 || direction_classes == 9 || direction_classes == 17,
                  "cdnet_dam_val_sums: direction_classes %d must be 5, 9 or 17 (options.py:45)", direction_classes);
    const int P = H * W;
    if (workspace_floats < cdnet_dam_val_sums_classes_workspace_floats(B, P, direction_classes)) { set_error("cdnet_dam_val_sums: workspace too small"); return CDNET_E_WORKSPACE; }
    ValIn L;
    L.mask = mask; L.point = point; L.dirn = dirn; L.label = label; L.dirlab = dirlab; L.weight = weight_u8; L.point_t = point_target_f16;
    for (int k = 0; k < 17; ++k) L.lut[k] = k < direction_classes ? dir_rank_host[k] : -1;
// ... 12 lines not shown
```

### cdnet_amd/engine.py

```python
import ctypes as C
import os
import torch

from . import _lib


class ConvSrc(C.Structure):
    _fields_ = [('x', C.c_void_p), ('res', C.c_void_p), ('scale', C.c_void_p), ('shift', C.c_void_p),
                ('C', C.c_int), ('Hs', C.c_int), ('Ws', C.c_int), ('pool', C.c_int), ('relu', C.c_int),
                ('off_y', C.c_int), ('off_x', C.c_int), ('f16', C.c_int), ('row_stride', C.c_int)]


class ConvArgs(C.Structure):
    _fields_ = [('src', ConvSrc * 2), ('nsrc', C.c_int), ('w', C.c_void_p), ('bias', C.c_void_p),
                ('oscale', C.c_void_p), ('oshift', C.c_void_p), ('orelu', C.c_int), ('out', C.c_void_p),
                ('Cout', C.c_int), ('out_cstride', C.c_int), ('out_coff', C.c_int), ('stats', C.c_void_p),
                ('N', C.c_int), ('H', C.c_int), ('W', C.c_int), ('taps', C.c_int), ('npar', C.c_int),
                ('ostride', C.c_int), ('nchunk', C.c_int), ('tile', C.c_int), ('CK', C.c_int), ('BN', C.c_int),
                ('out_f16', C.c_int), ('debug', C.c_int), ('ws', C.c_int), ('f32', C.c_int),
                ('eres', C.c_void_p), ('eres_scale', C.c_void_p), ('eres_shift', C.c_void_p), ('eres_f16', C.c_int), ('eres_relu', C.c_int),
                ('taps1', C.c_int), ('pad_', C.c_int), ('pool_out', C.c_void_p),
                ('dot_w', C.c_void_p), ('dot_b', C.c_void_p), ('dot_out', C.c_void_p)]


# ... 85 lines not shown
    if ck >= 16:
        ck = 16
    if ck == 16 and bn > 64:
        bn = 64
    return (16, ck, bn)


def dominant_kernel_name(precision, tiles=16):
    if precision == 'fp32':
        return 'conv_ws32_kernel<64,0,false>'
    quad = tiles * 256 * 256 * (64 + 64) * 2 >= (512 << 20)
    return 'conv_ws16_kernel<64,0,false,false,0,4,4,true,false,true,%s>' % ('true' if quad else 'false')


def packed_elems(Cout, nchunk, taps, CK, BN, npar):
    return _lib.load().cdnet_conv_packed_weight_elems(Cout, nchunk, taps, CK, BN, npar)


def _pack_dims(w, cfg, mode):
    _, CK, BN = cfg[:3]
    if mode == 0:
        Cout, Cin, KH, KW = w.shape
    elif mode == 1:
        Cin, Cout, KH, KW = w.shape
    elif mode in (4, 5, 6):
        Cout, ct, KH, KW = w.shape
        Cin = 4 * ct
    elif mode == 7:
        Cin, ct, KH, KW = w.shape
        Cout = 4 * ct
    else:
        Cin, Cout, KH, KW = w.shape
    taps = {2: 4, 3: 1, 4: 9, 5: 1, 6: 9, 7: 9}.get(mode, KH * KW)
    npar = 4 if mode in (2, 3) else 1
    return Cout, Cin, KH, KW, CK, BN, taps, npar


class PackJob(C.Structure):
    _fields_ = [('w', C.c_void_p), ('packed', C.c_void_p), ('Cout', C.c_int), ('Cin', C.c_int), ('KH', C.c_int), ('KW', C.c_int),
                ('CK', C.c_int), ('BN', C.c_int), ('mode', C.c_int), ('pad_', C.c_int)]


def pack_job(w, cfg, mode, out, split=False):
    Cout, Cin, KH, KW, CK, BN, taps, npar = _pack_dims(w, cfg, mode)
    assert out.numel() == packed_elems(Cout, Cin // CK, taps, CK, BN, npar) * (2 if split else 1)
    j = PackJob()
    j.w, j.packed, j.Cout, j.Cin, j.KH, j.KW, j.CK, j.BN = w.data_ptr(), out.data_ptr(), Cout, Cin, KH, KW, CK, BN
    j.mode = mode | (PACK_SPLIT if split else 0)
    return j


PACK_SPLIT = 16


def pack_weights(w, cfg, mode, Cin_pad=None, out=None, split=False, cout_scale=None):
    assert w.dtype == torch.float32 and w.is_cuda and w.is_contiguous()
    Cout, Cin, KH, KW, CK, BN, taps, npar = _pack_dims(w, cfg, mode)
    Cin_p = Cin if Cin_pad is None else Cin_pad
    if Cin_p != Cin:
        if mode == 0:
            wp = torch.zeros((Cout, Cin_p, KH, KW), dtype=torch.float32, device=w.device)
            wp[:, :Cin] = w
        else:
            raise NotImplementedError
        w, Cin = wp.contiguous(), Cin_p
    n = packed_elems(Cout, Cin // CK, taps, CK, BN, npar) * (2 if split else 1)
    if out is None or out.numel() != n:
        out = torch.empty((n,), dtype=torch.int16, device=w.device)
    if cout_scale is not None:
        assert mode == 0 and cout_scale.dtype == torch.float32 and cout_scale.numel() == Cout
        _lib.call('cdnet_pack_conv_weights_scaled', _lib.ptr(w), _lib.ptr(cout_scale), _lib.ptr(out), Cout, Cin, KH, KW, CK, BN,
                  mode | (PACK_SPLIT if split else 0), _lib.stream_ptr())
        return out
    _lib.call('cdnet_pack_conv_weights', _lib.ptr(w), _lib.ptr(out), Cout, Cin, KH, KW, CK, BN, mode | (PACK_SPLIT if split else 0),
              _lib.stream_ptr())
    return out


CONV_DEBUG = 0


def conv_forward(srcs, wpacked, Cout, cfg, taps=9, transposed=False, bias=None, oscale=None, oshift=None,
                 orelu=False, out=None, stats=None, H=None, W=None, out_dtype=torch.bfloat16, eres=None, query_ws=False, bns=None, taps1=0, pool_out=None, dot=None,
                 pad_chunks=0, debug_or=0):
    tile, CK, BN = cfg[:3]
    s0 = srcs[0]
    f32 = s0.f32
    assert all(s.f32 == f32 for s in srcs)
    if f32:
        out_dtype = torch.float32
    N = s0.N
    if H is None:
        H, W = s0.logical_hw()
        H, W = H + 0, W + 0
    ostride = 2 if transposed else 1
    npar = 4 if transposed else 1
    a = ConvArgs()
    nchunk = 0
    for i, s in enumerate(srcs):
        assert s.C % CK == 0, (s.C, CK)
        s.fill(a.src[i])
        nchunk += s.C // CK
    a.nsrc = len(srcs)
    if dot is not None:
        assert out is None and stats is None and eres is None and bns is None and pool_out is None and not f32 and not transposed
        a.dot_w, a.dot_b, a.dot_out = dot[0].data_ptr(), dot[1].data_ptr(), dot[2].data_ptr()
        assert dot[0].numel() == Cout and dot[0].dtype == torch.float32 and dot[2].dtype == torch.float32 and dot[2].numel() == N * H * W
    elif out is None:
        out = torch.empty((N, H * ostride, W * ostride, Cout), dtype=out_dtype, device=s0.x.device)
    ntiles = ((H + tile - 1) // tile) * ((W + tile - 1) // tile)
    if stats is True:
        stats = torch.empty((N * npar * ntiles, 2, Cout), dtype=torch.float32, device=s0.x.device)
    a.w, a.bias, a.oscale, a.oshift = _dp(wpacked), _dp(bias), _dp(oscale), _dp(oshift)
    a.orelu = int(orelu)
    a.out, a.Cout, a.out_cstride, a.out_coff = (None if out is None else out.data_ptr()), Cout, (Cout if out is None else out.shape[3]), 0
    a.stats = _dp(stats)
    a.N, a.H, a.W = N, H, W
    assert pad_chunks == 0 or (len(srcs) == 2 and taps == 9 and not f32 and all(s.scale is None and not s.relu and s.res is None and not s.f16 for s in srcs))
    a.taps, a.npar, a.ostride, a.nchunk = taps, npar, ostride, nchunk + pad_chunks
    a.tile, a.CK, a.BN = tile, CK, BN
    a.out_f16 = int(out is not None and out.dtype == torch.float16)
    a.ws = 0
    a.taps1 = taps1
    a.pool_out = _dp(pool_out)
    a.debug = CONV_DEBUG | debug_or
    a.f32 = int(f32)
    assert out is None or (out.dtype == torch.float32) == f32
    if eres is not None:
        assert not transposed and stats is None and not orelu and out.dtype == (torch.float32 if f32 else torch.bfloat16) and tuple(eres.x.shape) == tuple(out.shape)
        assert eres.f32 == f32
        a.eres, a.eres_scale, a.eres_shift = eres.x.data_ptr(), _dp(eres.scale), _dp(eres.shift)
        a.eres_f16, a.eres_relu = int(eres.f16), int(eres.relu)
    if bns is not None:
        raw, sc, sh, mu, inv, partial = bns
        assert eres is None and stats is None and bias is None and oscale is None and oshift is None and tuple(raw.shape) == tuple(out.shape)
        a.ws = 2
        a.eres, a.oscale, a.oshift, a.eres_scale, a.eres_shift, a.stats = raw.data_ptr(), sc.data_ptr(), sh.data_ptr(), mu.data_ptr(), inv.data_ptr(), partial.data_ptr()
    if query_ws:
        return int(_lib.load().cdnet_conv_ws_eligible(C.byref(a)))
    _lib.call('cdnet_conv_forward', C.byref(a), _lib.stream_ptr())
    return out, stats
```

### cdnet_amd/models/dam/model_unet_rev1.py

```python
import torch
import torch.nn as nn

from ... import _lib, runtime
from ...runtime import ConvLayer, Src, pooled, pad_offsets

VGG16_CFG = [64, 64, 'M', 128, 128, 'M', 256, 256, 256, 'M', 512, 512, 512, 'M', 512, 512, 512, 'M']


def vgg16_bn_features():
    layers, c = [], 3
    for v in VGG16_CFG:
        if v == 'M':
            layers.append(nn.MaxPool2d(kernel_size=2, stride=2))
        else:
            layers += [nn.Conv2d(c, v, kernel_size=3, padding=1), nn.BatchNorm2d(v), nn.ReLU(inplace=True)]
            c = v
    return nn.Sequential(*layers)


class revAttention(nn.Module):
    def __init__(self, in_channels):
        super().__init__()
        self.Conv1x1 = nn.Conv2d(in_channels, 1, kernel_size=1, bias=False)

# ... 93 lines not shown
        self.direction_conv = nn.Conv2d(64, self.DIRECTION_OUT, kernel_size=1)
        self.maskAtt = revAttention(self.DIRECTION_OUT)
        self.mask_conv = nn.Conv2d(64, 3, kernel_size=1)
        if self.VARIANT != 'rev1':
            self.residual = ResidualUnit(64, 64)
        if encoder_freeze:
            self.freeze_encoder()
        self._rt = None
        self._head_w = None
        self._head_ver = None

    def freeze_encoder(self):
        for p in self.backbone.parameters():
            p.requires_grad = False

    UNUSED_PREFIXES = ('final_conv.', 'child0.', 'child_conv1.')

    def _build_runtime(self):
        enc, i = [], 0
        mods = list(self.backbone.children())
        while i < len(mods):
            if isinstance(mods[i], nn.Conv2d):
                enc.append(('conv', ConvLayer('backbone.%d' % i, 'conv3', mods[i].weight, mods[i].bias, mods[i + 1]), str(i + 2)))
                i += 3
            else:
                enc.append(('pool', None, str(i)))
                i += 1
        dec = []
        for k, b in enumerate(self.upsample_blocks):
            dec.append((ConvLayer('upsample_blocks.%d.up' % k, 'convT4', b.up.weight, None, b.bn1),
                        ConvLayer('upsample_blocks.%d.conv2' % k, 'conv3', b.conv2.weight, None, b.bn2)))
        self._rt = dict(enc=enc, dec=dec, ru=[_RU('mask_feature', self.mask_feature),
                                               _RU('direction_feature', self.direction_feature),
                                               _RU('point_feature', self.point_feature)])
        if self.VARIANT != 'rev1':
            self._rt['ru_res'] = _RU('residual', self.residual)

    def conv_layers(self):
        if self._rt is None:
            self._build_runtime()
        out = [l for kind, l, _ in self._rt['enc'] if kind == 'conv']
        for up, c2 in self._rt['dec']:
            out += [up, c2]
        for ru in self._rt['ru']:
            out += ru.layers()
        if 'ru_res' in self._rt:
            out += self._rt['ru_res'].layers()
        return out

    def head_weight_block(self):
        ps = [self.point_conv.weight, self.direction_conv.weight, self.mask_conv.weight, self.point_conv.bias,
              self.direction_conv.bias, self.mask_conv.bias, self.directionAtt.Conv1x1.weight, self.maskAtt.Conv1x1.weight]
        if getattr(self, '_head_flat', None) is not None:
            return self._head_flat
        ver = tuple(p._version for p in ps)
        if self._head_w is None or self._head_ver != ver:
            with torch.no_grad():
                self._head_w = torch.cat([p.detach().reshape(-1).float() for p in ps]).contiguous()
            assert self._head_w.numel() == 855
            self._head_ver = ver
        return self._head_w

    def forward_features(self, x, training):
        if self._rt is None:
            self._build_runtime()
        if not x.is_cuda:
            raise RuntimeError('cdnet_amd.models.dam.model_unet_rev1.Unet runs on the MI355X only (no CPU fallback)')
        assert x.shape[1] == 3, 'the CDNet path feeds 3-channel tiles (child0/child_conv1 branches are never taken)'
        return self.forward_features_packed(runtime.input_pack(x.float()), training)

    def forward_features_packed(self, x16, training):
        if self._rt is None:
            self._build_runtime()
        t = Src(x16)
        t.is_input = True
        self._rt['enc'][0][1].needs_input_grad = False
        feats = {}
        enc, tp = self._rt['enc'], None
        for idx, (kind, layer, out_name) in enumerate(enc):
            if kind == 'conv':
                if not training and idx + 1 < len(enc) and enc[idx + 1][0] == 'pool' and not getattr(runtime, 'DEBUG_NORELU', False):
                    t, tp = layer.forward_eval_pool([t])
                else:
                    t = layer.forward([t], training)
            else:
                t, tp = (tp if tp is not None else pooled(t)), None
            if out_name in self.shortcut_features:
                feats[out_name] = t
            if out_name == self.bb_out_name:
                break
        for skip_name, (up, conv2) in zip(self.shortcut_features[::-1], self._rt['dec']):
            skip = feats[skip_name]
            u = up.forward([t], training)
            sh, sw = skip.logical_hw()
            uh, uw = u.logical_hw()
            u.off = pad_offsets((uh, uw), (sh, sw))
            tt = None if training else conv2.forward_eval_swapped([u, skip], H=sh, W=sw)
            t = tt if tt is not None else conv2.forward([u, skip], training, H=sh, W=sw)
        f1 = self._rt['ru'][0].forward(t, training, store=True)
        f2 = self._rt['ru'][1].forward(f1, training, store=True)
        if self.VARIANT == 'rev1':
            dot = None
            if not training and runtime.PRECISION != 'fp32':
                hw = self.head_weight_block()
                dot = (hw[0:64], hw[832:833])
            f3 = self._rt['ru'][2].forward(f2, training, dot=dot)
            return f1, f2, f3
        f3 = self._rt['ru'][2].forward(f2, training) if self.VARIANT == 'MandDandP' else None
        f1m = self._rt['ru_res'].forward(f1, training)
        return f1m, f2, f3

    def forward(self, *input):
        x = input[0]
        return self._head(self.forward_features(x, self.training))

    def forward_packed(self, x16):
        return self._head(self.forward_features_packed(x16, self.training))

    def _plain_head(self, feats):
        import ctypes as C
        f1m, f2, f3 = feats
        self._last_feats = feats
        N, H, W, _ = f1m.x.shape
        dev = f1m.x.device

        def cls(f, conv):
            K = conv.out_channels
            out = torch.empty((N, K, H, W), dtype=torch.float32, device=dev)
            hf = runtime.head_feat(f)
            w = conv.weight.detach().reshape(K, 64).contiguous()
            _lib.call('cdnet_final_conv1x1', C.byref(hf), _lib.ptr(w), _lib.ptr(conv.bias.detach()), K, N, H, W, _lib.ptr(out), _lib.stream_ptr())
            return out
        mask, direction = cls(f1m, self.mask_conv), cls(f2, self.direction_conv)
        if self.VARIANT == 'MandDandP':
            return mask, cls(f3, self.point_conv), direction
        return mask, direction

    def _head(self, feats):
        if getattr(self, 'VARIANT', 'rev1') != 'rev1':
            return self._plain_head(feats)
        f1, f2, f3 = feats
        N, H, W, _ = f1.x.shape
        dev = f1.x.device
        mask = torch.empty((N, 3, H, W), dtype=torch.float32, device=dev)
        direction = torch.empty((N, 9, H, W), dtype=torch.float32, device=dev)
        import ctypes as C
        if isinstance(f3, runtime.PointLogit):
            point = f3.point
            hf = [runtime.head_feat(f1), runtime.head_feat(f2), runtime.HeadFeat()]
        else:
            point = torch.empty((N, 1, H, W), dtype=torch.float32, device=dev)
            hf = [runtime.head_feat(f) for f in (f1, f2, f3)]
        _lib.call('cdnet_dam_head_forward', C.byref(hf[0]), C.byref(hf[1]), C.byref(hf[2]), _lib.ptr(self.head_weight_block()),
                  N, H, W, _lib.ptr(mask), _lib.ptr(point), _lib.ptr(direction), _lib.stream_ptr())
        self._last_feats = (f1, f2, f3)
        return mask, point, direction
```

### cdnet_amd/runtime.py

```python
import ctypes as C
import weakref
import torch

from . import _lib, engine
from .engine import Src

BN_EPS = 1e-5
BN_MOMENTUM = 0.1

import os as _os

PRECISION = _os.environ.get('CDNET_PRECISION', 'bf16')
assert PRECISION in ('bf16', 'fp32'), PRECISION


def set_precision(p):
    global PRECISION
    assert p in ('bf16', 'fp32'), p
    if p != PRECISION:
        PRECISION = p
        WEIGHTS_EPOCH[0] += 1


def act_dtype():
# ... 107 lines not shown
        if self.fold is None or self.fold_version != ver:
            if self.fold is None:
                self.fold = (torch.empty_like(self.scale), torch.empty_like(self.shift))
            _lib.call('cdnet_bn_fold_eval', _lib.ptr(bn.weight.detach()), _lib.ptr(bn.bias.detach()),
                      _lib.ptr(bn.running_mean), _lib.ptr(bn.running_var),
                      None if self.bias is None else _lib.ptr(self.bias.detach()), BN_EPS, self.Cout,
                      _lib.ptr(self.fold[0]), _lib.ptr(self.fold[1]), _lib.stream_ptr())
            self.fold_version = ver
        return self.fold

    def eval_pack(self, src_channels, allow_f32=False):
        if not EVAL_FOLD_WEIGHTS or not getattr(self, 'fold_eval', True) or self.kind not in ('conv3', 'conv1') or self.bn is None:
            return None
        f32 = PRECISION == 'fp32'
        if f32 and not allow_f32:
            return None
        cin_total = sum(src_channels)
        pad = cin_total if cin_total != self.Cin else None
        sc, sh = self.eval_fold()
        ver = (self.weight._version, self.fold_version, WEIGHTS_EPOCH[0], tuple(self.cfg), f32)
        if getattr(self, 'wpe', None) is None or self.wpe_version != ver:
            self.wpe = engine.pack_weights(self.weight.detach(), self.cfg, 0, Cin_pad=pad, out=getattr(self, 'wpe', None), cout_scale=sc, split=f32)
            self.wpe_version = ver
        return self.wpe, sh

    def forward_eval_swapped(self, srcs, relu=True, H=None, W=None):
        if PRECISION != 'bf16' or self.kind != 'conv3' or self.bn is None or len(srcs) != 2 or not EVAL_FOLD_WEIGHTS or not getattr(self, 'fold_eval', True):
            return None
        a, b = srcs
        if (a.C // 16) % 2 == 0 or (b.C // 16) % 2 or a.C % 16 or b.C % 16 or a.C + b.C != self.Cin:
            return None
        if any(s.scale is not None or s.relu or s.res is not None or s.f16 or s.pool for s in srcs):
            return None
        if H is None:
            H, W = b.logical_hw()
        if H % 16 or W % 16:
            return None
        self.prepare([s.C for s in srcs], H, W, a.N)
        if tuple(self.cfg[:2]) != (16, 16):
            return None
        sc, sh = self.eval_fold()
        ver = (self.weight._version, self.fold_version, WEIGHTS_EPOCH[0], tuple(self.cfg), a.C)
        if getattr(self, 'wps', None) is None or self.wps_version != ver:
            w = self.weight.detach()
            wz = torch.zeros((w.shape[0], 16, w.shape[2], w.shape[3]), dtype=w.dtype, device=w.device)
            wperm = torch.cat([w[:, a.C:], w[:, :a.C], wz], 1).contiguous()
            self.wps = engine.pack_weights(wperm, self.cfg, 0, cout_scale=sc)
            self.wps_version = ver
        kw = dict(oshift=sh, orelu=relu and not DEBUG_NORELU, H=H, W=W, pad_chunks=1)
        key = (a.N, H, W, a.C, b.C, a.off, b.off, engine.CONV_DEBUG, PRECISION)
        elig = self.__dict__.setdefault('_swapped_eligible', {})
        if key not in elig:
            elig[key] = engine.conv_forward([b, a], self.wps, self.Cout, self.cfg, 9, query_ws=True, **kw) == 2
        if not elig[key]:
            return None
        out, _ = engine.conv_forward([b, a], self.wps, self.Cout, self.cfg, 9, **kw)
        return Src(out)

    def forward_eval_pool(self, srcs):
        H, W = srcs[0].logical_hw()
        if PRECISION == 'bf16' and H % 2 == 0 and W % 2 == 0:
            self.prepare([s.C for s in srcs], H, W, srcs[0].N)
            ep = self.eval_pack([s.C for s in srcs])
            if ep is not None:
                N = srcs[0].N
                out = torch.empty((N, H, W, self.Cout), dtype=torch.bfloat16, device=srcs[0].x.device)
                pout = torch.empty((N, H // 2, W // 2, self.Cout), dtype=torch.bfloat16, device=srcs[0].x.device)
                kw = dict(oshift=ep[1], orelu=True, H=H, W=W, out=out, pool_out=pout)
                if engine.conv_forward(srcs, ep[0], self.Cout, self.cfg, self.taps, self.transposed, query_ws=True, **kw) == 2:
                    engine.conv_forward(srcs, ep[0], self.Cout, self.cfg, self.taps, self.transposed, **kw)
                    return Src(out), Src(pout)
        if PRECISION == 'fp32' and H % 2 == 0 and W % 2 == 0 and self.bn is not None and not DEBUG_NORELU:
            self.prepare([s.C for s in srcs], H, W, srcs[0].N)
            sc, sh = self.eval_fold()
            N = srcs[0].N
            out = torch.empty((N, H, W, self.Cout), dtype=torch.float32, device=srcs[0].x.device)
            pout = torch.empty((N, H // 2, W // 2, self.Cout), dtype=torch.float32, device=srcs[0].x.device)
            kw = dict(oscale=sc, oshift=sh, orelu=True, H=H, W=W, out=out, pool_out=pout)
            if engine.conv_forward(srcs, self.wp, self.Cout, self.cfg, self.taps, self.transposed, query_ws=True, **kw) == 1:
                engine.conv_forward(srcs, self.wp, self.Cout, self.cfg, self.taps, self.transposed, **kw)
                return Src(out), Src(pout)
        return self.forward(srcs, False), None

    def forward(self, srcs, training, relu=True, H=None, W=None, out_dtype=None, eres=None, debug_or=0):
        if PRECISION == 'fp32':
            out_dtype = torch.float32
        elif out_dtype is None:
            out_dtype = torch.bfloat16
        if H is None:
            H, W = srcs[0].logical_hw()
        if DEBUG_NORELU:
            relu = False
        self.prepare([s.C for s in srcs], H, W, srcs[0].N)
        bias = None if self.bias is None else self.bias.detach()
        if self.bn is None:
            out, _ = engine.conv_forward(srcs, self.wp, self.Cout, self.cfg, self.taps, self.transposed, bias=bias, H=H, W=W,
                                         out_dtype=out_dtype, eres=eres)
            if training:
                self.saved = (srcs, out, H, W)
                self.node_relu, self.node_res = False, None
                if TAPE is not None:
                    TAPE.append(self)
            return Src(out)
        if not training:
            ep = self.eval_pack([s.C for s in srcs])
            if ep is not None:
                out, _ = engine.conv_forward(srcs, ep[0], self.Cout, self.cfg, self.taps, self.transposed, oshift=ep[1],
                                             orelu=relu and eres is None, H=H, W=W, out_dtype=out_dtype, eres=eres, debug_or=debug_or)
                return Src(out)
            sc, sh = self.eval_fold()
            out, _ = engine.conv_forward(srcs, self.wp, self.Cout, self.cfg, self.taps, self.transposed, oscale=sc,
                                         oshift=sh, orelu=relu and eres is None, H=H, W=W, out_dtype=out_dtype, eres=eres, debug_or=debug_or)
            return Src(out)
        tile = self.cfg[0]
        N = srcs[0].N
        npar = 4 if self.transposed else 1
        T = N * npar * ((H + tile - 1) // tile) * ((W + tile - 1) // tile)
        if self.stats is None or self.stats.shape[0] != T:
            self.stats = torch.empty((T, 2, self.Cout), dtype=torch.float32, device=self.weight.device)
        raw, _ = engine.conv_forward(srcs, self.wp, self.Cout, self.cfg, self.taps, self.transposed, stats=self.stats,
                                     H=H, W=W, out_dtype=raw_dtype())
        count = float(N * H * W * npar)
        bn = self.bn
        _lib.call('cdnet_bn_finalize_train', _lib.ptr(self.stats), T, self.Cout, count, _lib.ptr(bn.weight.detach()),
                  _lib.ptr(bn.bias.detach()), None if bias is None else _lib.ptr(bias), BN_EPS,
                  BN_MOMENTUM if getattr(bn, 'momentum', None) is None else float(bn.momentum),
                  _lib.ptr(bn.running_mean), _lib.ptr(bn.running_var), _lib.ptr(self.scale), _lib.ptr(self.shift),
                  _lib.ptr(self.save_mean), _lib.ptr(self.save_invstd), _lib.stream_ptr())
        self.saved = (srcs, raw, H, W)
        self.node_relu, self.node_res = relu, None
        self.fold_version = None
        if TAPE is not None:
            TAPE.append(self)
        return Src(raw, self.scale, self.shift, relu=relu)


class FuseTerm(C.Structure):
    _fields_ = [('x', C.c_void_p), ('Hs', C.c_int), ('Ws', C.c_int), ('scale', C.c_void_p), ('shift', C.c_void_p),
                ('f16', C.c_int), ('pad_', C.c_int)]


class GradTerm(C.Structure):
    _fields_ = [('g', C.c_void_p), ('cstride', C.c_int), ('coff', C.c_int)]


class FuseNode:

    def __init__(self, name):
        self.name = name
        self.saved = None

    def forward(self, terms, relu, out=None, out_coff=0, training=False):
        for t in terms:
            assert t.res is None and not t.pool and not t.relu and t.row_stride == 0 and t.x.is_contiguous()
        N, Cc = terms[0].N, terms[0].C
        H, W = (max(t.Hs for t in terms), max(t.Ws for t in terms)) if out is None else (out.shape[1], out.shape[2])
        arr = (FuseTerm * len(terms))()
        for k, t in enumerate(terms):
            assert t.C == Cc
            arr[k].x, arr[k].Hs, arr[k].Ws = t.x.data_ptr(), t.Hs, t.Ws
            arr[k].scale, arr[k].shift = (None if t.scale is None else t.scale.data_ptr()), (None if t.shift is None else t.shift.data_ptr())
            arr[k].f16 = int(t.f16)
        f32 = terms[0].f32
        assert all(t.f32 == f32 for t in terms)
        if out is None:
            o, cs = torch.empty((N, H, W, Cc), dtype=torch.float32 if f32 else torch.bfloat16, device=terms[0].x.device), Cc
        else:
            o, cs = out, out.shape[3]
        assert (o.dtype == torch.float32) == f32
        if DEBUG_NORELU:
            relu = False
        _lib.call(_lib.entry('cdnet_fuse_sum', f32), C.byref(arr), len(terms), N, H, W, Cc, int(relu), _lib.ptr(o), cs, out_coff,
                  _lib.stream_ptr())
        if training:
            self.saved = (list(terms), o, relu, H, W, Cc, out_coff)
            if TAPE is not None:
                TAPE.append(self)
        return Src(o) if out is None else None

    def backward(self, tr, grads, add):
        terms, o, relu, H, W, Cc, coff = self.saved
        sliced = o.shape[3] != Cc
        if sliced:
            d, dcs, dco = tr.cat_grad(o, grads), o.shape[3], coff
            if d is None:
                return
        else:
            gl = tr.take(grads, id(o))
            if gl is None:
                return
            if relu and self._residual_tail(tr, grads, gl, terms, o, H, W, Cc):
                return
            if relu or len(gl) > 1 or gl[0].coff or gl[0].cstride not in (0, Cc):
                d = tr.buf(('dfuse', self.name), o.shape, o.dtype)
                tr.grad_sum(gl, o if relu else None, o.shape[0] * H * W, Cc, d)
            else:
                d = gl[0].t
            dcs, dco = 0, 0
        N = o.shape[0]
        for k, t in enumerate(terms):
            if t.Hs == H and t.Ws == W:
                add(t.x, tr.G(d, H, W, coff=dco, cstride=dcs))
            else:
                din = tr.buf(('dup', self.name, k), (N, t.Hs, t.Ws, Cc), d.dtype)
                _lib.call(_lib.entry('cdnet_upsample_bilinear_backward', d.dtype == torch.float32), _lib.ptr(d),
                          N, H, W, Cc, dcs, dco, t.Hs, t.Ws, _lib.ptr(din), _lib.stream_ptr())
                add(t.x, tr.G(din, t.Hs, t.Ws))


def _residual_tail(self, tr, grads, gl, terms, o, H, W, Cc):
    if DEBUG_NORELU:
        return False
    if len(terms) == 1:
        y = terms[0]
        P = tr._producer.get(id(y.x)) if y.scale is not None else None
        if P is None or P.bn is None or getattr(P, 'node_res', None) is not None or tr._readers.get(id(y.x), 0) != 1 or id(y.x) in grads \
                or tuple(y.x.shape) != tuple(o.shape) or getattr(P, 'fused_res_of', None) is not None or (y.Hs, y.Ws) != (H, W):
            return False
        P.node_relu, P.node_res = True, None
        grads[id(y.x)] = gl
        return True
    if len(terms) != 2 or len(gl) > 3:
        return False
    bn_t = [t for t in terms if t.scale is not None]
    if not bn_t or any((t.Hs, t.Ws) != (H, W) for t in terms):
        return False
    y = max(bn_t, key=lambda t: tr._tape_pos.get(id(tr._producer.get(id(t.x))), -1))
    x = terms[1] if terms[0] is y else terms[0]
    P = tr._producer.get(id(y.x))
    if P is None or P.bn is None or getattr(P, 'node_res', None) is not None or tr._readers.get(id(y.x), 0) != 1 or id(y.x) in grads \
            or tuple(y.x.shape) != tuple(o.shape) or getattr(P, 'fused_res_of', None) is not None:
        return False
    if any(g.pooled or g.oy or g.ox or (g.Hg, g.Wg) != (H, W) for g in gl):
        return False
    P.node_relu, P.node_res, P.node_res_grad_to = 2, o, x.x
    grads[id(y.x)] = gl
    return True


FuseNode._residual_tail = _residual_tail


def input_pack(x):
    assert x.dtype == torch.float32 and x.is_cuda and x.dim() == 4
    x = x.contiguous()
    N, Cc, H, W = x.shape
    out = torch.empty((N, H, W, 16), dtype=act_dtype(), device=x.device)
    _lib.call(_lib.entry('cdnet_input_pack', PRECISION == 'fp32'), _lib.ptr(x), N, Cc, H, W, _lib.ptr(out),
              _lib.stream_ptr())
    return out


POOL_MATERIALIZE = True
RU_MATERIALIZE = True
RU_FUSE = True
EVAL_FOLD_WEIGHTS = True
RU_EVAL_ONE_LAUNCH = True
RU_EVAL_POINT_DOT = True


class PointLogit:

    def __init__(self, point):
        self.point = point


def residual_unit_eval(c1, c2, cr, x, relu2=True, dot=None):
    if not (RU_EVAL_ONE_LAUNCH and EVAL_FOLD_WEIGHTS) or not getattr(c2, 'fold_eval', True) or x.pool or x.C % 16 or c2.Cout % 16:
        return None
    H, W = x.logical_hw()
    if H % 16 or W % 16 or x.C != cr.Cin:
        return None
    c2.prepare([c2.Cin], H, W, x.N)
    if tuple(c2.cfg[:2]) != (16, 16):
        return None
    ep = c2.eval_pack([c1.Cout], allow_f32=True)
    if ep is None:
        return None
    f32 = PRECISION == 'fp32'
    rver = (cr.weight._version, WEIGHTS_EPOCH[0], tuple(c2.cfg), f32)
    if getattr(c2, 'ru_wr', None) is None or c2.ru_wr_version != rver:
        c2.ru_wr = engine.pack_weights(cr.weight.detach(), c2.cfg, 0, out=getattr(c2, 'ru_wr', None), split=f32)
        c2.ru_wr_version = rver
    pad = 1 if (not f32 and (x.C // 16) % 2 == 1 and c2.cfg[1] == 16) else 0
    ver = (c2.wpe_version, rver, None if cr.bias is None else cr.bias._version, PRECISION, pad)
    if getattr(c2, 'ru_pack', None) is None or c2.ru_pack_version != ver:
        BN = c2.cfg[2]
        ntile = -(-c2.Cout // BN)
        a, b = ep[0].view(ntile, -1), c2.ru_wr.view(ntile, -1)
        parts = [a, b]
        if pad:
            parts.append(torch.zeros((ntile, 16 * BN), dtype=a.dtype, device=a.device))
        c2.ru_pack = torch.cat(parts, 1).contiguous().view(-1)
        c2.ru_shift = ep[1] if cr.bias is None else ep[1] + cr.bias.detach()
        c2.ru_pack_version = ver
    hC = c1.Cout
    keep = engine.CONV_DEBUG
    elig = c2.__dict__.setdefault('_ru_eligible', {})
    key = (x.N, H, W, x.C, hC, PRECISION, keep, bool(relu2))
    want_dot = dot is not None and RU_EVAL_POINT_DOT and relu2
    kw = dict(oshift=c2.ru_shift, H=H, W=W, taps1=1, pad_chunks=pad, debug_or=64)
    if key not in elig or (want_dot and key + ('dot',) not in elig):
        hp = Src(torch.empty((x.N, H, W, hC), dtype=act_dtype(), device=x.x.device))
        elig[key] = bool(not (keep & 32) and engine.conv_forward([hp, x], c2.ru_pack, c2.Cout, c2.cfg, 9, orelu=relu2, query_ws=True, **kw))
        if want_dot:
            d0 = (dot[0], dot[1], torch.empty((x.N, 1, H, W), dtype=torch.float32, device=x.x.device))
            elig[key + ('dot',)] = elig[key] and engine.conv_forward([hp, x], c2.ru_pack, c2.Cout, c2.cfg, 9, orelu=True, dot=d0, query_ws=True, **kw) == 2
    if not elig[key]:
        return None
    h = c1.forward([x], False, relu=True, debug_or=64)
    assert h.C == hC and not h.pool and h.scale is None
    if want_dot and elig[key + ('dot',)]:
        point = torch.empty((x.N, 1, H, W), dtype=torch.float32, device=x.x.device)
        engine.conv_forward([h, x], c2.ru_pack, c2.Cout, c2.cfg, 9, orelu=True, dot=(dot[0], dot[1], point), **kw)
        return PointLogit(point)
    out, _ = engine.conv_forward([h, x], c2.ru_pack, c2.Cout, c2.cfg, 9, orelu=relu2, **kw)
    return Src(out)


def materialize(s, H=None, W=None):
    if H is None:
        H, W = s.logical_hw()
    out = torch.empty((s.N, H, W, s.C), dtype=(torch.float32 if s.f32 else torch.bfloat16), device=s.x.device)
    cs = engine.ConvSrc()
    s.fill(cs)
    _lib.call('cdnet_src_materialize', C.byref(cs), s.N, H, W, _lib.ptr(out), _lib.stream_ptr())
    return Src(out)


def pooled(s, ceil_mode=False, materialized=None):
    assert not s.pool and s.res is None
    mode = 2 if ceil_mode else 1
    lazy = Src(s.x, s.scale, s.shift, relu=s.relu, pool=mode)
    if not (POOL_MATERIALIZE if materialized is None else materialized) and not s.f32:
        return lazy
# ... 9 lines not shown
```

### cdnet_amd/trainer.py

```python
import ctypes as C
import os

import torch

from . import _lib, engine, optim, runtime, streams
from .allreduce import BucketReducer, bucketed_allreduce
from .engine import Src
from .optim import HEAD_PARAMS, FlatState
from .synth import synthetic_batch


class GradIn(C.Structure):
    _fields_ = [('g', C.c_void_p), ('Hg', C.c_int), ('Wg', C.c_int), ('oy', C.c_int), ('ox', C.c_int),
                ('pooled', C.c_int), ('coff', C.c_int), ('cstride', C.c_int), ('pad_', C.c_int)]


class BnBwdArgs(C.Structure):
    _fields_ = [('raw', C.c_void_p), ('res', C.c_void_p), ('scale', C.c_void_p), ('shift', C.c_void_p),
                ('mean', C.c_void_p), ('invstd', C.c_void_p), ('gin', GradIn * 3), ('ngin', C.c_int),
                ('f16', C.c_int), ('relu', C.c_int), ('N', C.c_int), ('H', C.c_int), ('W', C.c_int), ('C', C.c_int)]


_WGRAD_WGS_DEEP, _WGRAD_WGS_SHALLOW = 128, 160
_WGRAD_WGS_KQ = 128
_WGRAD_WGS_F32 = 160
_RU_1X1_SIDE = True
WGRAD_STREAM = True
HEAD_BWD_FUSE = True
_WGRAD_DEFER = 0x100
_WGRAD_DEEP_HW = 16384


class _on_stream:
    __slots__ = ('s', 'prev')

    def __init__(self, s):
        self.s = s

    def __enter__(self):
        self.prev = torch.cuda.current_stream()
        torch.cuda.set_stream(self.s)

    def __exit__(self, *exc):
        torch.cuda.set_stream(self.prev)
        return False


class _G:
    __slots__ = ('t', 'Hg', 'Wg', 'oy', 'ox', 'pooled', 'coff', 'cstride', 'event', 'masked')

    def __init__(self, t, Hg, Wg, oy=0, ox=0, pooled=0, coff=0, cstride=0):
        self.t, self.Hg, self.Wg, self.oy, self.ox, self.pooled, self.coff, self.cstride = t, Hg, Wg, oy, ox, pooled, coff, cstride
        self.event = None
        self.masked = False


def _choose_ci_tiles(C_src, Cout):
    if Cout <= 32 and runtime.PRECISION != 'fp32':
        return 1
    best, best_cost = 2, None
    for ci_t in (2, 1, 4):
        CI, CO = ci_t * 32, (4 // ci_t) * 32
        cost = -(-C_src // CI) * CI * -(-Cout // CO) * CO
        if best_cost is None or cost < best_cost:
            best, best_cost = ci_t, cost
    return best


def _wgrad_wgs(beside, HW, Cout):
    if not beside:
        return 256
    if runtime.PRECISION == 'fp32':
        return _WGRAD_WGS_F32
    if Cout <= 32 and HW > 65536:
        return _WGRAD_WGS_KQ
    return _WGRAD_WGS_DEEP if HW <= _WGRAD_DEEP_HW or HW > 65536 else _WGRAD_WGS_SHALLOW


class GradTerm(C.Structure):
    _fields_ = [('g', C.c_void_p), ('cstride', C.c_int), ('coff', C.c_int)]


class Trainer:
    G = _G

    def __init__(self, model, lr=1e-3, weight_decay=1e-4, betas=(0.9, 0.99), eps=None, quirk_sample0=True,
                 world_size=1, bucket_mb=25, optimizer='adam', momentum=0.95):
        self.model = model
        self._pack_jobs = None
        self._pack_prec = None
        self._ar = None
        self.optimizer = str(optimizer).lower()
        if self.optimizer not in optim.OPTIMIZERS:
            raise ValueError('Optimizer {} not available (one of {})'.format(optimizer, ', '.join(optim.OPTIMIZERS)))
        if eps is None:
            eps = optim.RANGER_EPS if self.optimizer == 'ranger' else 1e-8
        self.lr, self.wd, self.betas, self.eps, self.momentum = lr, weight_decay, betas, eps, momentum
        self.quirk = int(quirk_sample0)
        self.world = world_size
        self.bucket = int(float(bucket_mb) * (1 << 20) // 4)
        self.flat = FlatState(model, self.optimizer)
        model._head_flat = self.flat.P[:self.flat.n_head] if self.flat.n_head == 855 else None
        self.dev = self.flat.P.device
        self._bufs = {}
        self._wss = {}
        self.losses = torch.zeros((11,), dtype=torch.float32, device=self.dev)
        self.alpha = 0.0
        self.dice, self.weight_map = 1, 1
        self.loss_var = torch.full((1,), -1.0, dtype=torch.float32, device=self.dev)
        self.boundary = 0
# ... 269 lines not shown
            torch.cuda.current_stream().wait_event(ev)
        else:
            self._flush_reduces()

    def _weights_done(self, params):
        if not self._rd_pending:
            self._overlap_done(params)
            return
        self._rd_params.append(params)
        if self._rd_bytes >= self._rd_mb * (1 << 20):
            self._flush_reduces()

    def _flush_reduces(self):
        if self._rd_pending:
            key = tuple(self._rd_pending)
            tab = self._rd_tables.get(key)
            if tab is None:
                lib = _lib.load()
                descs = (_lib.WgradReduceDesc * len(key))()
                b0 = 0
                for i, a in enumerate(key):
                    _lib.call('cdnet_wgrad_reduce_desc_fill', *a, b0, C.byref(descs[i]))
                    b0 += descs[i].blocks
                dev_tab = torch.frombuffer(bytearray(bytes(descs)), dtype=torch.uint8).to(self.dev)
                tab = self._rd_tables[key] = (dev_tab, len(key), b0)
            _lib.call('cdnet_wgrad_reduce_batch', _lib.ptr(tab[0]), tab[1], tab[2], _lib.stream_ptr())
        for params in self._rd_params:
            self._overlap_done(params)
        self._rd_pending, self._rd_params, self._rd_bytes = [], [], 0

    def _layer_backward(self, k, L, gl, grads, add, side):
        srcs, out, Hl, Wl = L.saved
        No, Ho, Wo, Co = out.shape
        params = (L.weight, L.bias, None if L.bn is None else L.bn.weight, None if L.bn is None else L.bn.bias)
        part = self._bn_partials.pop(id(out), None)
        if len(gl) == 1 and gl[0].masked:
            g = self._bn_backward_masked(L, out, gl[0], add)
        elif part is not None:
            assert len(gl) == 1, (L.name, len(gl))
            a, ktab = self._bn_backward_stats(L, out, gl[0], partial=part)
            g = self.buf(('draw', L.name), (No, Ho, Wo, Co), runtime.act_dtype())
            _lib.call('cdnet_bn_backward_apply', C.byref(a), _lib.ptr(ktab), _lib.ptr(g), _lib.stream_ptr())
        elif L.bn is not None or len(gl) > 1 or gl[0].pooled or gl[0].coff or (gl[0].cstride not in (0, Co)):
            g = self._bn_backward(L, out, gl, add)
        else:
            g = gl[0].t
        if side is None:
            self._weight_backward(L, srcs, g, Hl, Wl)
            self._weights_done(params)
            self._input_backward(L, srcs, g, Hl, Wl, add)
        else:
            ev = self._event(k)
            ev.record()
            beside = _RU_1X1_SIDE and L.kind == 'conv1' and isinstance(k, tuple) and getattr(L, 'needs_input_grad', True)
            if not beside:
                self._input_backward(L, srcs, g, Hl, Wl, add)
            side.wait_event(ev)
            with _on_stream(side):
                if beside:
                    ev2 = self._event(('beside', k))

                    def add_beside(tgt, g_):
                        g_.event = ev2
                        add(tgt, g_)
                    self._input_backward(L, srcs, g, Hl, Wl, add_beside)
                    ev2.record()
                self._weight_backward(L, srcs, g, Hl, Wl)
                self._weights_done(params)

    def _bn_backward_stats(self, L, out, g, partial):
        a = self._bn_args(L, out, [_G(g.t, g.Hg, g.Wg)], res=None, relu=1)
        ktab = self.buf(('ktab', L.name), (7, out.shape[3]), torch.float32)
        bn = L.bn
        _lib.call('cdnet_bn_backward_finalize', C.byref(a), _lib.ptr(bn.weight.detach()), _lib.ptr(bn.weight.grad), _lib.ptr(bn.bias.grad),
                  _lib.ptr(partial), partial.shape[0], _lib.ptr(ktab), _lib.stream_ptr())
        return a, ktab

    def _bn_backward_masked(self, L, out, g, add):
        No, Ho, Wo, Co = out.shape
        a = self._bn_args(L, out, [_G(g.t, g.Hg, g.Wg)], res=None, relu=0)
        draw = self.buf(('draw', L.name), (No, Ho, Wo, Co), runtime.act_dtype())
        ws = self._ws('bn', _lib.load().cdnet_bn_backward_workspace_floats(Co))
        bn = L.bn
        _lib.call('cdnet_bn_backward', C.byref(a), _lib.ptr(bn.weight.detach()), _lib.ptr(bn.weight.grad), _lib.ptr(bn.bias.grad),
                  _lib.ptr(ws), ws.numel(), _lib.ptr(draw), None, _lib.stream_ptr())
        add(L.node_res, _G(g.t, Ho, Wo))
        return draw

    def _stats_fusable(self, L, srcs, H, W, N, wpb, cfgb, cin_total):
        f32 = runtime.PRECISION == 'fp32'
        if not f32 or os.environ.get('CDNET_BN_STATS_FUSE', '1') != '1' or getattr(runtime, 'DEBUG_NORELU', False):
            return None
        if L.kind != 'conv3' or L.transposed or len(srcs) != 1:
            return None
        sx = srcs[0]
        if getattr(sx, 'is_input', False) or sx.scale is None or sx.shift is None or sx.relu is not True or sx.res is not None or sx.pool \
                or tuple(sx.off) != (0, 0) or sx.x.dtype != runtime.raw_dtype() or hasattr(sx, 'grad_to') or sx.row_stride:
            return None
        if f32 and cin_total % 64:
            return None
        P = self._producer.get(id(sx.x))
        if P is None or P.bn is None or getattr(P, 'node_res', None) is not None or getattr(P, 'node_relu', True) is not True \
                or self._readers.get(id(sx.x), 0) != 1 or tuple(sx.x.shape) != (N, H, W, cin_total):
            return None
        key = ('statsfusable', L.name, N, H, W, runtime.PRECISION)
        hit = self._bufs.get(key)
        if hit is None:
            part = torch.zeros((1024, 2, cin_total), dtype=torch.float32, device=self.dev)
            gin = self.buf(('din', L.name), (N, H, W, cin_total), runtime.act_dtype())
            gdummy = self.buf(('draw', L.name), (N, H, W, L.Cout), runtime.act_dtype())
            ok = engine.conv_forward([Src(gdummy)], wpb, cin_total, cfgb, taps=L.taps, out=gin, H=H, W=W, query_ws=True,
                                     bns=(sx.x, P.scale, P.shift, P.save_mean, P.save_invstd, part))
            hit = self._bufs[key] = (part if ok else False)
        if hit is False:
            return None
        return P, hit

    def _bn_args(self, L, out, gl, res, relu):
        a = BnBwdArgs()
        a.raw = out.data_ptr()
        a.res = None if res is None else res.data_ptr()
        if L.bn is not None:
            a.scale, a.shift = L.scale.data_ptr(), L.shift.data_ptr()
            a.mean, a.invstd = L.save_mean.data_ptr(), L.save_invstd.data_ptr()
        a.ngin = len(gl)
        assert 1 <= len(gl) <= 3, (L.name, len(gl))
        for k, g in enumerate(gl):
            a.gin[k].g = g.t.data_ptr()
            a.gin[k].Hg, a.gin[k].Wg, a.gin[k].oy, a.gin[k].ox = g.Hg, g.Wg, g.oy, g.ox
            a.gin[k].pooled, a.gin[k].coff, a.gin[k].cstride = int(g.pooled), g.coff, g.cstride or out.shape[3]
        a.f16 = {torch.bfloat16: 0, torch.float16: 1, torch.float32: 2}[out.dtype]
        a.relu = relu
        a.N, a.H, a.W, a.C = out.shape
        return a

    def _bn_backward(self, L, out, gl, add):
        No, Ho, Wo, Co = out.shape
        res = getattr(L, 'node_res', None)
        has_bn = L.bn is not None
        if len(gl) > 3:
            plain = [g for g in gl if not g.pooled and g.oy == 0 and g.ox == 0 and (g.Hg, g.Wg) == (Ho, Wo)]
            rest = [g for g in gl if g not in plain]
            assert len(rest) <= 2 and len(plain) >= 2, (L.name, len(gl))
            d = self.buf(('gsum', L.name), (No, Ho, Wo, Co), runtime.act_dtype())
            self.grad_sum(plain, None, No * Ho * Wo, Co, d)
            gl = rest + [_G(d, Ho, Wo)]
        a = self._bn_args(L, out, gl, res, int(getattr(L, 'node_relu', True)))
        draw = self.buf(('draw', L.name), (No, Ho, Wo, Co), runtime.act_dtype())
        dz = None
        if res is not None:
            dz = self.buf(('dz', L.name), (No, Ho, Wo, Co), runtime.act_dtype())
        ws = self._ws('bn', _lib.load().cdnet_bn_backward_workspace_floats(Co))
        bn = L.bn
        _lib.call('cdnet_bn_backward', C.byref(a), _lib.ptr(bn.weight.detach()) if has_bn else None,
                  _lib.ptr(bn.weight.grad) if has_bn else None, _lib.ptr(bn.bias.grad) if has_bn else None,
                  _lib.ptr(ws), ws.numel(), _lib.ptr(draw), _lib.ptr(dz), _lib.stream_ptr())
        if res is not None:
            add(getattr(L, 'node_res_grad_to', None) if getattr(L, 'node_res_grad_to', None) is not None else res, _G(dz, Ho, Wo))
            L.node_res_grad_to = None
        return draw

    def _side_stream(self):
        if not WGRAD_STREAM or self.dev.type != 'cuda':
            return None
        if self._wstream is None:
            self._wstream = streams.side_stream(self.dev)
            self._events = {}
        return self._wstream

    def _event(self, k):
        e = self._events.get(k)
        if e is None:
            e = self._events[k] = torch.cuda.Event()
        return e

    def _weight_backward(self, L, srcs, g, H, W):
        lib = _lib.load()
        N = g.shape[0]
        Cout = L.Cout
        cin_total = sum(s.C for s in srcs)
        cin_real = L.Cin
        mode = {'conv3': 0, 'conv1': 0, 'convT4': 2, 'convT2': 3, 'conv3s2': 6}[L.kind]
        taps, npar, ostride = L.taps, (4 if L.transposed else 1), (2 if L.transposed else 1)
        cap = _wgrad_wgs(self._side_active and getattr(L, 'needs_input_grad', True), H * W, Cout)
        coff = 0
        for s in srcs:
            ci_t = _choose_ci_tiles(s.C, Cout)
            CI, CO = ci_t * 32, (4 // ci_t) * 32
            other = -(-s.C // CI) * -(-Cout // CO) * npar
            ntiles = N * (-(-H // 8)) * (-(-W // 16))
            ksplit = max(1, min(ntiles, cap // other if other < cap else 1))
            nslab = lib.cdnet_conv_wgrad_slab_floats(s.C, Cout, taps, npar, ci_t, ksplit)
            defer = self._rd_mb > 0
            slab = self.buf(('wslab', L.name, coff), (nslab,), torch.float32) if defer else self._ws('slab', nslab, side=True)
            cs = engine.ConvSrc()
            s.fill(cs)
            csrc_real = min(s.C, cin_real - coff) if cin_total != cin_real else s.C
            _lib.call('cdnet_conv_backward_weight', C.byref(cs), coff, csrc_real, cin_real, _lib.ptr(g), Cout, N, H, W, taps,
                      npar, ostride, ci_t, ksplit, _lib.ptr(slab), _lib.ptr(L.weight.grad), mode | (_WGRAD_DEFER if defer else 0),
                      _lib.stream_ptr())
            if defer:
                self._rd_pending.append((s.C, coff, csrc_real, cin_real, Cout, taps, npar, ci_t, ksplit, slab.data_ptr(),
                                         L.weight.grad.data_ptr(), mode))
                self._rd_bytes += nslab * 4
            coff += s.C
        if L.bias is not None and L.bn is None:
            owner = getattr(L, 'bias_grad_from', None)
            if owner is not None:
                L.bias.grad.copy_(owner.bn.bias.grad)
            else:
                ws = self._ws('slab', lib.cdnet_bias_grad_workspace_floats(Cout), side=True)
                _lib.call(_lib.entry('cdnet_bias_grad', g.dtype == torch.float32), _lib.ptr(g), g.numel() // Cout, Cout,
                          _lib.ptr(ws), ws.numel(), _lib.ptr(L.bias.grad), _lib.stream_ptr())

    def _input_backward(self, L, srcs, g, H, W, add):
        if not getattr(L, 'needs_input_grad', True):
            return
        N = g.N if isinstance(g, Src) else g.shape[0]
        Cout = L.Cout
        cin_total = sum(s.C for s in srcs)
        wpb, cfgb = L.backward_pack(cin_total, H, W)
        if L.kind == 'conv3s2':
            Cp = cin_total // 4
            gs2d = self.buf(('ds2d', L.name), (N, H, W, cin_total), runtime.act_dtype())
            engine.conv_forward([Src(g)], wpb, cin_total, cfgb, taps=9, out=gs2d, H=H, W=W)
            gin = self.buf(('din', L.name), (N, 2 * H, 2 * W, Cp), runtime.act_dtype())
            _lib.call(_lib.entry('cdnet_s2d_to_nhwc', gin.dtype == torch.float32), _lib.ptr(gs2d), N, H, W, Cp, _lib.ptr(gin),
                      _lib.stream_ptr())
            add(srcs[0].x, _G(gin, 2 * H, 2 * W))
            return
        if not L.transposed:
            gin = self.buf(('din', L.name), (N, H, W, cin_total), runtime.act_dtype())
            fuse = None if isinstance(g, Src) else self._stats_fusable(L, srcs, H, W, N, wpb, cfgb, cin_total)
            if fuse is not None:
                P, part = fuse
                engine.conv_forward([Src(g)], wpb, cin_total, cfgb, taps=L.taps, out=gin, H=H, W=W,
                                    bns=(srcs[0].x, P.scale, P.shift, P.save_mean, P.save_invstd, part))
                self._bn_partials[id(srcs[0].x)] = part
            else:
                engine.conv_forward([g if isinstance(g, Src) else Src(g)], wpb, cin_total, cfgb, taps=L.taps, out=gin, H=H, W=W)
        else:
            gin = self.buf(('din', L.name), (N, H, W, cin_total), runtime.act_dtype())
            views = [Src(g, view=(a * 2 * W * Cout, H, W, 2 * Cout, 4 * W * Cout)) for a in (0, 1)]
            engine.conv_forward(views, wpb, cin_total, cfgb, taps=(9 if L.kind == 'convT4' else 1), out=gin, H=H, W=W)
        coff = 0
        for s in srcs:
            if getattr(s, 'is_input', False):
                coff += s.C
                continue
            tgt, pool = getattr(s, 'grad_to', (s.x, int(s.pool)))
            add(tgt, _G(gin, H, W, oy=s.off[0], ox=s.off[1], pooled=pool, coff=coff, cstride=cin_total))
            coff += s.C

    def _overlap_begin(self):
        self._ar = None
        if not self._reduce_active() or os.environ.get('CDNET_ALLREDUCE_OVERLAP', '1') == '0':
            return
        f = self.flat
        base = f.G.data_ptr()
        pend = {}
        owners = [p for L in self.tape if not isinstance(L, runtime.FuseNode) for p in (L.weight, L.bias, None if L.bn is None else L.bn.weight,
                                                 None if L.bn is None else L.bn.bias) if p is not None]
        for p in owners:
            off = (p.grad.data_ptr() - base) // 4
            if 0 <= off < f.n_used:
                pend[off] = off + p.numel()
        if f.n_head:
            pend[0] = f.n_head
        self._ar = BucketReducer(f.G, f.n_used, self.bucket, pend)

    def _overlap_done(self, params):
        if self._ar is None:
            return
        if params is None:
            self._ar.done([0])
        else:
            base = self.flat.G.data_ptr()
            self._ar.done([(p.grad.data_ptr() - base) // 4 for p in params if p is not None])

    def _reduce_active(self):
        return self.world > 1 or os.environ.get('CDNET_FORCE_ALLREDUCE', '0') == '1'

    def allreduce_and_step(self):
        f = self.flat
        gscale = 1.0
        works = None
        if self._reduce_active():
            if self._ar is not None:
                ranges = self._ar.finish(wait=False)
                works = self._ar.works
                self.ar_stats = dict(buckets=len(works), released_during_backward=self._ar.early)
                self._ar = None
# ... 179 lines not shown
```

### include/cdnet_hip.h

```cpp
#ifndef CDNET_HIP_H
#define CDNET_HIP_H

#include <stddef.h>
#include <stdint.h>

#ifdef __cplusplus
extern "C" {
#endif

#define CDNET_OK            0
#define CDNET_E_ARG         1
#define CDNET_E_WORKSPACE   2
#define CDNET_E_LAUNCH      3

#define CDNET_ABI_VERSION   5

int         cdnet_abi_version(void);
size_t      cdnet_abi_sizeof(const char *struct_name);
const char *cdnet_last_error(void);
const char *cdnet_build_info(void);
int         cdnet_spin(int microseconds, void *stream);
int         cdnet_box_copy(const void *src, void *dst, size_t bytes, void *stream);
int         cdnet_box_mfma(const uint32_t *seed, float *sink, unsigned long long *stamps, int workgroups, int waves_per_wg, int iters, void *stream);

// ... 107 lines not shown
int cdnet_pack_conv_weights_batch(const cdnet_pack_job *jobs, int n_jobs, void *table, size_t table_bytes, int upload,
                                  void *stream);
int cdnet_conv_forward(const cdnet_conv_args *args, void *stream);

int cdnet_input_pack(const float *x, int N, int C, int H, int W, void *out_bf16_nhwc16, void *stream);
int cdnet_input_pack_f32(const float *x, int N, int C, int H, int W, float *out_f32_nhwc16, void *stream);
int cdnet_bn_fold_eval(const float *gamma, const float *beta, const float *running_mean, const float *running_var,
                       const float *conv_bias, float eps, int C, float *scale, float *shift, void *stream);
int cdnet_bn_finalize_train(const float *stats, int T, int C, float count, const float *gamma, const float *beta,
                            const float *conv_bias, float eps, float momentum, float *running_mean,
                            float *running_var, float *scale, float *shift, float *save_mean, float *save_invstd,
                            void *stream);

typedef struct cdnet_head_feat {
    const uint16_t *raw;
    const uint16_t *res;
    const float *scale;
    const float *shift;
    int relu;
    int f16;
} cdnet_head_feat;

#define CDNET_HEAD_WEIGHT_FLOATS 855
int cdnet_dam_head_forward(const cdnet_head_feat *f1, const cdnet_head_feat *f2, const cdnet_head_feat *f3,
                           const float *head_weights, int N, int H, int W, float *mask, float *point,
                           float *direction, void *stream);
int cdnet_final_conv1x1(const cdnet_head_feat *f, const float *w, const float *b, int K, int N, int H, int W,
                        float *out, void *stream);
size_t cdnet_bias_grad_workspace_floats(int C);
int cdnet_bias_grad(const uint16_t *grad_out, size_t npix, int C, float *workspace, size_t workspace_floats, float *db, void *stream);
int cdnet_bias_grad_f32(const float *grad_out, size_t npix, int C, float *workspace, size_t workspace_floats, float *db, void *stream);
size_t cdnet_final_conv1x1_backward_workspace_floats(void);
int cdnet_final_conv1x1_backward(const cdnet_head_feat *f, const float *w, const float *dlogits, int K, int N, int H, int W,
                                 uint16_t *df, float *workspace, size_t workspace_floats, float *dw, float *db, void *stream);

int cdnet_conv_ws_eligible(const cdnet_conv_args *args);

int cdnet_src_materialize(const cdnet_conv_src *src, int N, int H, int W, uint16_t *out, void *stream);

size_t cdnet_conv_wgrad_slab_floats(int C_src, int Cout, int taps, int npar, int ci_tiles, int ksplit);
int cdnet_conv_backward_weight(const cdnet_conv_src *src, int src_coff, int Csrc_real, int Cin_real,
                               const uint16_t *grad_out, int Cout, int N, int H, int W, int taps, int npar,
                               int ostride, int ci_tiles, int ksplit, float *slab, float *dw, int mode, void *stream);

#define CDNET_WGRAD_DEFER_REDUCE 0x100
typedef struct cdnet_wgrad_reduce_desc {
    const float *slab;
    float *dw;
    int ksplit, npar, ci_blocks, co_blocks, taps, CI, CO, Csrc_real, Cin_real, src_coff, Cout, mode;
    int block0, blocks;
} cdnet_wgrad_reduce_desc;
int cdnet_wgrad_reduce_desc_fill(int C_src, int src_coff, int Csrc_real, int Cin_real, int Cout, int taps, int npar, int ci_tiles,
                                 int ksplit, const float *slab, float *dw, int mode, int block0, cdnet_wgrad_reduce_desc *out);
int cdnet_wgrad_reduce_batch(const cdnet_wgrad_reduce_desc *table_dev, int n, int total_blocks, void *stream);

typedef struct cdnet_grad_in {
    const uint16_t *g;
    int Hg, Wg;
    int oy, ox;
    int pooled;
    int coff, cstride;
    int pad_;
} cdnet_grad_in;

typedef struct cdnet_bn_bwd_args {
    const uint16_t *raw;
    const uint16_t *res;
    const float *scale, *shift;
    const float *mean, *invstd;
    cdnet_grad_in gin[3];
    int ngin;
    int f16, relu;
    int N, H, W, C;
} cdnet_bn_bwd_args;

size_t cdnet_bn_backward_workspace_floats(int C);
int cdnet_bn_backward_stats(const cdnet_bn_bwd_args *args, const float *gamma, float *dgamma, float *dbeta, float *workspace,
                            size_t workspace_floats, float *ktab, void *stream);
int cdnet_bn_backward_apply(const cdnet_bn_bwd_args *args, const float *ktab, uint16_t *draw, void *stream);
int cdnet_bn_backward_finalize(const cdnet_bn_bwd_args *args, const float *gamma, float *dgamma, float *dbeta, const float *partial,
                               int nb, float *ktab, void *stream);
int cdnet_bn_backward(const cdnet_bn_bwd_args *args, const float *gamma, float *dgamma, float *dbeta, float *workspace,
                      size_t workspace_floats, uint16_t *draw, uint16_t *dz_out, void *stream);

size_t cdnet_dam_head_backward_workspace_floats(int N, int H, int W);
int cdnet_dam_head_backward(const cdnet_head_feat *f1, const cdnet_head_feat *f2, const cdnet_head_feat *f3,
                            const float *head_weights, const float *dmask, const float *dpoint, const float *ddir,
                            int N, int H, int W, uint16_t *df1, uint16_t *df2, uint16_t *df3, float *workspace,
                            size_t workspace_floats, float *dhead_weights, void *stream);
int cdnet_dam_head_backward_fused_blocks(void);
int cdnet_dam_head_backward_fused_scratch_bytes(void);
size_t cdnet_dam_head_backward_fused_workspace_floats(void);
int cdnet_dam_head_backward_fused(const cdnet_head_feat *f1, const cdnet_head_feat *f2, const cdnet_head_feat *f3,
                                  const float *head_weights, const float *dmask, const float *dpoint, const float *ddir, int N, int H,
                                  int W, float *df1, float *df2, float *dz3, float *workspace, size_t workspace_floats,
                                  float *dhead_weights, void *stream);

size_t cdnet_dam_loss_workspace_floats(int B, int P);
int cdnet_dam_loss(const float *mask, const float *point, const float *direction, const uint8_t *label,
                   const uint8_t *dirlab, const uint16_t *point_target_f16, const uint8_t *weight_u8, int B, int H, int W,
                   int quirk_sample0, float *workspace, size_t workspace_floats, float *losses, float *dmask,
                   float *dpoint, float *ddir, void *stream);
size_t cdnet_dam_loss_classes_workspace_floats(int B, int P, int direction_classes);
int cdnet_dam_loss_classes(const float *mask, const float *point, const float *direction, const uint8_t *label,
                           const uint8_t *dirlab, const uint16_t *point_target_f16, const uint8_t *weight_u8, int B, int H, int W,
                           int direction_classes, int quirk_sample0, float *workspace, size_t workspace_floats, float *losses,
                           float *dmask, float *dpoint, float *ddir, void *stream);

#define CDNET_LOSS_WMAP 1u
#define CDNET_LOSS_CE   2u
#define CDNET_LOSS_DICE 4u

int cdnet_dam_loss_terms(const float *mask, const float *point, const float *direction, const uint8_t *label,
                         const uint8_t *dirlab, const uint16_t *point_target_f16, const uint8_t *weight_u8, int B, int H, int W,
                         int direction_classes, int quirk_sample0, float *workspace, size_t workspace_floats, float *losses,
                         float *dmask, float *dpoint, float *ddir, void *stream, unsigned terms);

size_t cdnet_mask_loss_workspace_floats(int B, int P);
int cdnet_mask_loss(const float *mask_logits, const uint8_t *label, const uint8_t *weight_u8, int B, int H, int W, unsigned terms,
                    float *workspace, size_t workspace_floats, float *losses, float *dmask, void *stream);

size_t cdnet_variance_loss_workspace_bytes(int B, int K, int H, int W);
int cdnet_variance_loss(const float *mask_logits, const uint8_t *label, int fg_value, int B, int K, int H, int W, float alpha,
                        void *workspace, size_t workspace_bytes, float *loss_var, float *total, float *dmask, int32_t *root_out,
                        int32_t *counts, void *stream);

size_t cdnet_boundary_loss_workspace_bytes(int kind, int B, int K, int H, int W);
int cdnet_boundary_loss(const float *mask_logits, const uint8_t *label, int kind, int B, int K, int H, int W, float beta,
                        void *workspace, size_t workspace_bytes, float *loss_out, float *total, float *dmask, void *stream);
int cdnet_boundary_loss_scratch_bytes(void);

#define CDNET_VAL_SUMS 42
size_t cdnet_dam_val_sums_workspace_floats(int B, int P);
int cdnet_dam_val_sums(const float *mask, const float *point, const float *dirn, const uint8_t *label, const uint8_t *dirlab,
                       const uint16_t *point_target_f16, const uint8_t *weight_u8, const int *dir_rank_host, int B, int H, int W,
                       float *workspace, size_t workspace_floats, float *sums, void *stream);
size_t cdnet_dam_val_sums_classes_workspace_floats(int B, int P, int direction_classes);
int cdnet_dam_val_sums_classes(const float *mask, const float *point, const float *dirn, const uint8_t *label, const uint8_t *dirlab,
                               const uint16_t *point_target_f16, const uint8_t *weight_u8, const int *dir_rank_host,
                               int direction_classes, int B, int H, int W, float *workspace, size_t workspace_floats, float *sums,
                               void *stream);

int cdnet_adam_step(float *param, const float *grad, float *exp_avg, float *exp_avg_sq, size_t n, float lr, float beta1,
                    float beta2, float eps, float weight_decay, int step, float grad_scale, void *stream);

int cdnet_moment_step(float *param, const float *grad, float *exp_avg, float *exp_avg_sq, float *slow, size_t n, double beta1,
                      double beta2, float grad_scale, int move, int rect, float decay, float step_size, float v_div, float eps,
                      int sync, float alpha, void *stream);
int cdnet_sgd_step(float *param, const float *grad, float *momentum_buffer, size_t n, float lr, float momentum, float weight_decay,
                   int step, float grad_scale, void *stream);

int cdnet_window_pack(const float *img, int C, int H, int W, int view_xform, int tile_h, int tile_w, int stride, int ny,
                      int nx, void *out_bf16_nhwc16, void *stream);
int cdnet_window_pack_f32(const float *img, int C, int H, int W, int view_xform, int tile_h, int tile_w, int stride, int ny,
                          int nx, float *out_f32_nhwc16, void *stream);
int cdnet_window_stitch(const float *tiles, int K, int tile_h, int tile_w, int stride, int overlap, int ny, int nx, int Hv,
                        int Wv, float *out, void *stream);

typedef struct cdnet_aug_sample {
    double minv[6];
    const uint8_t *img;
    const uint8_t *weight;
    const void *label;
    int32_t H, W, img_stride, weight_stride, label_stride, label_i32;
    float color[4];
    int32_t hflip, vflip, filter, y0, x0;
// ... 81 lines not shown
```

Measured before the change: 1082.

## Fuse max-pool into training conv, write dbias in BN backward, restructure loss finalize

Several independent changes. In training, the conv forward that precedes a pool can now emit the pooled raw output directly. It uses a sign-aware med3 so the result matches the pool taken after the BN affine, which removes a separate pooling pass. The BN backward finalize can also write the bias gradient of a tied layer directly, removing a later copy. The loss kernels are refactored so the error flag can be carried in the per-sample single array instead of an atomic. Together these add complexity in the conv epilogue and an eligibility probe on each new shape.

Result: no change. 1089 (median of 6 runs) (+0.7%).

```diff
diff --git a/cdnet_amd/_lib.py b/cdnet_amd/_lib.py
--- a/cdnet_amd/_lib.py
+++ b/cdnet_amd/_lib.py
@@ -85,6 +85,7 @@
     'cdnet_wgrad_reduce_batch': (_i, [_vp, _i, _i, _vp]),
     'cdnet_bn_backward_workspace_floats': (_sz, [_i]),
     'cdnet_bn_backward': (_i, [_vp, _vp, _vp, _vp, _vp, _sz, _vp, _vp, _vp]),
+    'cdnet_bn_backward_dbias': (_i, [_vp, _vp, _vp, _vp, _vp, _vp, _sz, _vp, _vp, _vp]),
     'cdnet_dam_head_backward_workspace_floats': (_sz, [_i, _i, _i]),
     'cdnet_dam_head_backward': (_i, [_vp] * 7 + [_i, _i, _i, _vp, _vp, _vp, _vp, _sz, _vp, _vp]),
     'cdnet_dam_head_backward_fused_blocks': (_i, []),
diff --git a/cdnet_amd/csrc/bn_bwd.hip b/cdnet_amd/csrc/bn_bwd.hip
--- a/cdnet_amd/csrc/bn_bwd.hip
+++ b/cdnet_amd/csrc/bn_bwd.hip
@@ -535,7 +535,7 @@
 
 __global__ __launch_bounds__(256) void bn_bwd_finalize_kernel(const float *__restrict__ partial, int nb, int C, float M, const float *gamma,
                                                               const float *invstd, float *dgamma, float *dbeta, float *k1, float *k2,
-                                                              float *k3) {
+                                                              float *k3, float *dbeta2) {
     __shared__ double s_a[256], s_b[256];
     const int c = blockIdx.x;
     const int lane = threadIdx.x;
@@ -551,6 +551,7 @@
     s1 = s_a[0]; s2 = s_b[0];
     if (lane == 0) {
         if (dbeta) dbeta[c] = (float)s1;
+        if (dbeta2) dbeta2[c] = (float)s1;
         if (dgamma) dgamma[c] = (float)s2;
         k1[c] = gamma[c] * invstd[c];
         k2[c] = (float)(s1 / M);
@@ -659,8 +660,8 @@
 }
 
 static void bn_finalize(const BnBwdArgs &A, const float *partial, int nb, const float *gamma, float *dgamma, float *dbeta, float *k,
-                        hipStream_t st) {
-    bn_bwd_finalize_kernel<<<A.C, 256, 0, st>>>(partial, nb, A.C, (float)bn_npix(A), gamma, A.invstd, dgamma, dbeta, k, k + A.C, k + 2 * A.C);
+                        hipStream_t st, float *dbeta2 = nullptr) {
+    bn_bwd_finalize_kernel<<<A.C, 256, 0, st>>>(partial, nb, A.C, (float)bn_npix(A), gamma, A.invstd, dgamma, dbeta, k, k + A.C, k + 2 * A.C, dbeta2);
 }
 
 static void bn_set_coeffs(BnBwdArgs &A, const float *k) { A.k1 = k; A.k2 = k + A.C; A.k3 = k + 2 * A.C; }
@@ -674,8 +675,8 @@
     return B;
 }
 
-extern "C" int cdnet_bn_backward(const cdnet_bn_bwd_args *a, const float *gamma, float *dgamma, float *dbeta, float *workspace,
-                                 size_t workspace_floats, uint16_t *draw, uint16_t *dz_out, void *stream) {
+static int bn_backward_impl(const cdnet_bn_bwd_args *a, const float *gamma, float *dgamma, float *dbeta, float *dbeta2, float *workspace,
+                            size_t workspace_floats, uint16_t *draw, uint16_t *dz_out, void *stream) {
     BnBwdArgs A;
     int rc = fill_bn_args(a, A, "cdnet_bn_backward");
     if (rc) return rc;
@@ -696,12 +697,23 @@
         A.dz_out = dz_reuse ? dz_out : nullptr;
         float *k = workspace + (size_t)P.nb * 2 * A.C;
         launch<false>(P, A, st);
-        bn_finalize(A, A.partial, P.nb, gamma, dgamma, dbeta, k, st);
+        bn_finalize(A, A.partial, P.nb, gamma, dgamma, dbeta, k, st, dbeta2);
         bn_set_coeffs(A, k);
     }
     A.dz_out = dz_out;
     launch<true>(P, reuse ? bn_dz_as_source(A, dz_out) : A, st);
     return check_launch("cdnet_bn_backward");
+}
+
+extern "C" int cdnet_bn_backward(const cdnet_bn_bwd_args *a, const float *gamma, float *dgamma, float *dbeta, float *workspace,
+                                 size_t workspace_floats, uint16_t *draw, uint16_t *dz_out, void *stream) {
+    return bn_backward_impl(a, gamma, dgamma, dbeta, nullptr, workspace, workspace_floats, draw, dz_out, stream);
+}
+
+extern "C" int cdnet_bn_backward_dbias(const cdnet_bn_bwd_args *a, const float *gamma, float *dgamma, float *dbeta, float *dbias, float *workspace,
+                                       size_t workspace_floats, uint16_t *draw, uint16_t *dz_out, void *stream) {
+    CDNET_REQUIRE(a && a->mean && dbias, "cdnet_bn_backward_dbias: a BatchNorm layer and the second destination");
+    return bn_backward_impl(a, gamma, dgamma, dbeta, dbias, workspace, workspace_floats, draw, dz_out, stream);
 }
 
 static bool bn_plain_case(const BnBwdArgs &A, bool masked = false) {
diff --git a/cdnet_amd/csrc/conv32ws.hip b/cdnet_amd/csrc/conv32ws.hip
--- a/cdnet_amd/csrc/conv32ws.hip
+++ b/cdnet_amd/csrc/conv32ws.hip
@@ -56,7 +56,7 @@
 __global__ __launch_bounds__(512) void conv_ws32_kernel(ConvArgs A) {
     static_assert(!BNS || (BN == 64 && !STATS), "the BatchNorm-backward statistics epilogue serves 64-channel blocks of backward-data launches");
     static_assert(!MIX || (!STATS && !BNS && NCS == 0), "one-tap chunks: inference launches with at least four nine-tap chunks");
-    static_assert(!POOL || (!STATS && !BNS && !MIX && NCS == 0), "fused max-pool: plain inference launches with at least four chunks");
+    static_assert(!POOL || (!BNS && !MIX && NCS == 0 && (BN == 64 || STATS)), "fused max-pool: plain launches with at least four chunks (inference: 64 output channels per workgroup)");
     using L = Ws32Lds<BN>;
     constexpr int TH = 16, TW = 16, CK = 16, TAPS = 9, PSTR = L::PSTR, HW_ = TW + 2, NPIX = L::NPIX;
     constexpr int NPW = BN / 32, MPW = 2;
@@ -356,6 +356,12 @@
         e_osh[ni] = BNS ? 0.f : fmaf((A.bias && cok) ? A.bias[co] : 0.f, e_osc[ni], (A.oshift && cok) ? A.oshift[co] : 0.f);
     }
     const bool orelu = A.orelu != 0;
+    float p_lim[NPW];
+#pragma unroll
+    for (int ni = 0; ni < NPW; ++ni) {
+        const int co = cout0 + ni * 32 + l31;
+        p_lim[ni] = __builtin_bit_cast(float, (POOL && STATS && co < A.Cout && A.eres_scale[co] < 0.f) ? 0xff800000u : 0x7f800000u);
+    }
     float b_sc[NPW], b_sh[NPW], b_mu[NPW], b_is[NPW], b_s1[NPW], b_s2[NPW], b_x = 0.f;
     if (BNS) {
 #pragma unroll
@@ -423,6 +429,17 @@
     };
     auto pool_sub = [&](const f32x16 (&P)[MPW][NPW], int u, int sub) {
         const int b_ = u / 4, k = u % 4, mi = b_ / NPW, ni = b_ % NPW, r0 = 2 * k;
+        if (STATS) {
+            if (sub == 0) pl_t0 = __builtin_amdgcn_fmed3f(fmaf(P[mi][ni][r0], e_osc[ni], e_osh[ni]), fmaf(P[mi][ni][r0 + 1], e_osc[ni], e_osh[ni]), p_lim[ni]);
+            else if (sub == 1) pl_t1 = __builtin_amdgcn_fmed3f(fmaf(P[mi][ni][r0 + 8], e_osc[ni], e_osh[ni]), fmaf(P[mi][ni][r0 + 9], e_osc[ni], e_osh[ni]), p_lim[ni]);
+            else if (e_ok[ni]) {
+                const float v = __builtin_amdgcn_fmed3f(pl_t0, pl_t1, p_lim[ni]);
+                char *sb = prow_base[mi] + ((unsigned)(((r0 >> 2) & 1) * 4 + ((r0 & 3) >> 1)) * ppix_b + (unsigned)(ni * 128));
+                asm volatile("" : "+s"(sb));
+                *(__attribute__((address_space(1))) float *)((__attribute__((address_space(1))) char *)sb + pl_off) = v;
+            }
+            return;
+        }
         if (sub == 0) pl_t0 = fmaxf(fmaf(P[mi][ni][r0], e_osc[ni], e_osh[ni]), fmaf(P[mi][ni][r0 + 1], e_osc[ni], e_osh[ni]));
         else if (sub == 1) pl_t1 = fmaxf(fmaf(P[mi][ni][r0 + 8], e_osc[ni], e_osh[ni]), fmaf(P[mi][ni][r0 + 9], e_osc[ni], e_osh[ni]));
         else {
@@ -480,7 +497,8 @@
                 constexpr int QEL = NEL / 4;
                 if ((EPI == 1 || EPI == 5 || EPI == 6) && STATS && g % 3 == 1 && 2 * (g / 3) + 1 < NEL) { stat_elem(P, 2 * (g / 3), par); stat_elem(P, 2 * (g / 3) + 1, par); }
                 if (EPI <= 4 && g % 6 == 3 && g / 6 < QEL) img_elem(P, (EPI - 1) * QEL + g / 6);
-                if (POOL && EPI <= 4 && g % 6 == 5 && g / 6 < 12) pool_sub(P, (EPI - 1) * 4 + (g / 6) / 3, (g / 6) % 3);
+                constexpr int WPI = MPW * NPW;
+                if (POOL && EPI <= 4 && g % 6 == 5 && g / 6 < 3 * WPI) pool_sub(P, (EPI - 1) * WPI + (g / 6) / 3, (g / 6) % 3);
                 if (EPI == 5 && g % 3 != 1 && 2 * (g / 3) + (g % 3 == 2 ? 1 : 0) < NEL) img_elem(P, 2 * (g / 3) + (g % 3 == 2 ? 1 : 0));
                 if ((EPI == 6 || EPI == 7) && g % 3 == 0 && g / 3 < NEL / 2) img_elem(P, (EPI - 6) * (NEL / 2) + g / 3);
                 if (BNS && EPI <= 4) {
@@ -675,7 +693,10 @@
     const int xf = all_plain ? 0 : (all_fast ? 1 : 2);
     if (A.nchunk < 4 && (BN != 64 || xf == 2)) return -1;
     const bool pool = A.pool_out != nullptr;
-    if (pool && (BN != 64 || bns || mix || A.stats || A.nchunk < 4 || xf != 0 || !A.orelu || A.out_coff || A.out_cstride != A.Cout)) return -1;
+    const bool pool_raw = pool && A.stats;
+    if (pool && ((BN != 64 && !pool_raw) || bns || mix || A.nchunk < 4 || A.out_coff || A.out_cstride != A.Cout)) return -1;
+    if (pool && !pool_raw && (xf != 0 || !A.orelu)) return -1;
+    if (pool_raw && (xf == 2 || A.orelu || A.oscale || A.oshift || A.eres || !A.eres_scale)) return -1;
     if (dry_run) return CDNET_OK;
     if (bns) {
         if constexpr (BN == 64) {
@@ -691,6 +712,11 @@
         });
     }
     if (!pool) return with_bool(A.stats != nullptr, [&](auto st_c) { return with_int<0, 1, 2>(xf, [&](auto xf_c) { return launch(xf_c, st_c); }); });
+    if (pool_raw) {
+        return with_int<0, 1>(xf, [&](auto xf_c) {
+            return launch_lds<conv_ws32_kernel<BN, decltype(xf_c)::value, true, false, 0, false, true>>(grid, 512, 160 * 1024, smem, st, "hipFuncSetAttribute(conv_ws32 pool raw)", "conv_ws32_kernel(pool raw)", A);
+        });
+    }
     if constexpr (BN == 64) {
         return launch_lds<conv_ws32_kernel<64, 0, false, false, 0, false, true>>(grid, 512, 160 * 1024, smem, st, "hipFuncSetAttribute(conv_ws32 pool)", "conv_ws32_kernel(pool)", A);
     }
diff --git a/cdnet_amd/csrc/dam_loss.hip b/cdnet_amd/csrc/dam_loss.hip
--- a/cdnet_amd/csrc/dam_loss.hip
+++ b/cdnet_amd/csrc/dam_loss.hip
@@ -62,14 +62,15 @@
         for (int i = 1; i < 16; ++i) {
             mn = s_min[i] < mn ? s_min[i] : mn; mx = s_max[i] > mx ? s_max[i] : mx; lm = s_lmax[i] > lm ? s_lmax[i] : lm;
         }
-        single[blockIdx.x] = (mn == mx) ? 1 : 0;
-        if (mx > nd - 1 || lm > 2) atomicOr(err, 1);
+        const bool bad = mx > nd - 1 || lm > 2;
+        single[blockIdx.x] = ((mn == mx) ? 1 : 0) | ((!err && bad) ? 2 : 0);
+        if (err && bad) atomicOr(err, 1);
     }
 }
 
 template <int ND>
 __device__ __forceinline__ int dice_target(const LossIn &L, int b, int i) {
-    if (L.single[b]) return 0;
+    if (L.single[b] & 1) return 0;
     int t = L.dirlab[(size_t)b * L.P + i];
     t = t > ND - 1 ? ND - 1 : t;
     if (L.quirk0) return L.label[i] != 0 ? t : -1;
@@ -130,50 +131,61 @@
     row_sum<TPB>(acc, tid, b, partial);
 }
 
-template <int ND>
-__global__ __launch_bounds__(256) void loss_finalize_kernel(const float *__restrict__ partial, int nchunk, int B, int P,
-                                                            float *__restrict__ sums, float *__restrict__ coef,
-                                                            float *__restrict__ losses, const int *__restrict__ err, unsigned terms) {
-    using Y = LossLay<ND>;
-    constexpr int NS = Y::SUMS;
-    const bool plain = !(terms & CDNET_LOSS_WMAP);
-    __shared__ float s_sum[64 * NS];
-    const int tid = threadIdx.x;
+template <int ND> struct LossTerms {
+    static constexpr int T_PREV = 3 + ND, T_NEXT = T_PREV + ND - 1, NT = T_NEXT + ND - 1;
+};
+
+__device__ __forceinline__ int loss_err_flag(const int *err, const int *single, int B) {
+    if (err) return *err;
+    int e = 0;
+    for (int b = 0; b < B; ++b) e |= single[b] >> 1;
+    return e;
+}
+
+template <int ND>
+__device__ __forceinline__ void loss_sample_coef(const float *S, float fB, bool plain, float *cf) {
+    using Y = LossLay<ND>;
+    mask_dice_coef(S, fB, cf);
+    float bsum[ND];
+    for (int i = 0; i < ND; ++i) bsum[i] = 0.f;
+    for (int j = 0; j < ND; ++j) {
+        {
+            const float U = S[Y::PW + j] + S[Y::TW + j], Sij = S[Y::SS + j], m = j == 0 && !plain ? 2.f : 1.f;
+            cf[6 + ND + j] = m * -2.f / (fB * (U + 1.f));
+            bsum[j] += m * 2.f * (Sij + 1.f) / (fB * (U + 1.f) * (U + 1.f));
+        }
+        if (plain) { cf[6 + 2 * ND + j] = 0.f; cf[6 + 3 * ND + j] = 0.f; }
+        else if (j >= 1) {
+            const int in = dnext<ND>(j), ip = dprev<ND>(j);
+            {   const float U = S[Y::PW + in] + S[Y::TW + j], Sij = S[Y::SN + j];
+                cf[6 + 2 * ND + j] = -2.f / (fB * (U + 1.f));
+                bsum[in] += 2.f * (Sij + 1.f) / (fB * (U + 1.f) * (U + 1.f)); }
+            {   const float U = S[Y::PW + ip] + S[Y::TW + j], Sij = S[Y::SP + j];
+                cf[6 + 3 * ND + j] = -2.f / (fB * (U + 1.f));
+                bsum[ip] += 2.f * (Sij + 1.f) / (fB * (U + 1.f) * (U + 1.f)); }
+        } else { cf[6 + 2 * ND] = 0.f; cf[6 + 3 * ND] = 0.f; }
+    }
+    for (int i = 0; i < ND; ++i) cf[6 + i] = bsum[i];
+}
+
+template <int ND>
+__device__ __forceinline__ void loss_all_sums(const float *__restrict__ partial, int nchunk, int B, float *__restrict__ sums, float *s_sum, int tid) {
+    constexpr int NS = LossLay<ND>::SUMS;
     for (int idx = tid; idx < B * NS; idx += 256) {
         const int b = idx / NS, k = idx % NS;
         const float s = chunk_sum<NS>(partial + (size_t)b * nchunk * NS + k, nchunk);
         s_sum[idx] = s;
         if (sums) sums[idx] = s;
     }
-    __syncthreads();
+}
+
+template <int ND>
+__device__ __forceinline__ void loss_write_losses(const float *s_sum, float *s_term, int B, int P, float *__restrict__ losses, int errflag, unsigned terms, int tid) {
+    using Y = LossLay<ND>;
+    using T = LossTerms<ND>;
+    constexpr int NS = Y::SUMS, T_PREV = T::T_PREV, T_NEXT = T::T_NEXT, NT = T::NT;
+    const bool plain = !(terms & CDNET_LOSS_WMAP);
     const float fB = (float)B;
-    for (int b = tid; b < B; b += 256) {
-        const float *S = s_sum + b * NS;
-        float *cf = coef + (size_t)b * Y::COEF;
-        mask_dice_coef(S, fB, cf);
-        float bsum[ND];
-        for (int i = 0; i < ND; ++i) bsum[i] = 0.f;
-        for (int j = 0; j < ND; ++j) {
-            {
-                const float U = S[Y::PW + j] + S[Y::TW + j], Sij = S[Y::SS + j], m = j == 0 && !plain ? 2.f : 1.f;
-                cf[6 + ND + j] = m * -2.f / (fB * (U + 1.f));
-                bsum[j] += m * 2.f * (Sij + 1.f) / (fB * (U + 1.f) * (U + 1.f));
-            }
-            if (plain) { cf[6 + 2 * ND + j] = 0.f; cf[6 + 3 * ND + j] = 0.f; }
-            else if (j >= 1) {
-                const int in = dnext<ND>(j), ip = dprev<ND>(j);
-                {   const float U = S[Y::PW + in] + S[Y::TW + j], Sij = S[Y::SN + j];
-                    cf[6 + 2 * ND + j] = -2.f / (fB * (U + 1.f));
-                    bsum[in] += 2.f * (Sij + 1.f) / (fB * (U + 1.f) * (U + 1.f)); }
-                {   const float U = S[Y::PW + ip] + S[Y::TW + j], Sij = S[Y::SP + j];
-                    cf[6 + 3 * ND + j] = -2.f / (fB * (U + 1.f));
-                    bsum[ip] += 2.f * (Sij + 1.f) / (fB * (U + 1.f) * (U + 1.f)); }
-            } else { cf[6 + 2 * ND] = 0.f; cf[6 + 3 * ND] = 0.f; }
-        }
-        for (int i = 0; i < ND; ++i) cf[6 + i] = bsum[i];
-    }
-    constexpr int T_PREV = 3 + ND, T_NEXT = T_PREV + ND - 1, NT = T_NEXT + ND - 1;
-    __shared__ float s_term[NT];
     if (tid < NT) {
         int num, da, db;
         if (tid < 3) { num = tid; da = 3 + tid; db = 6 + tid; }
@@ -203,18 +215,34 @@
         losses[0] = (terms & CDNET_LOSS_CE) ? ce + dice + dce + wd + mse : dice + dce + wd + mse;
         losses[1] = dce; losses[2] = wd; losses[3] = mse; losses[4] = ce; losses[5] = dice;
         pixel_metrics<NS>(s_sum, Y::SC + 3, B, P, losses + 6);
-        poison_on_error(err, losses, 11);
-    }
-}
-
-template <int ND>
-__global__ __launch_bounds__(256) void loss_grad_kernel(LossIn L, const float *__restrict__ coef, float *__restrict__ dmask,
-                                                        float *__restrict__ dpoint, float *__restrict__ ddir) {
-    const int b = blockIdx.y;
-    const float *cf = coef + (size_t)b * LossLay<ND>::COEF;
+        poison_on_error(&errflag, losses, 11);
+    }
+}
+
+template <int ND>
+__global__ __launch_bounds__(256) void loss_finalize_kernel(const float *__restrict__ partial, int nchunk, int B, int P,
+                                                            float *__restrict__ sums, float *__restrict__ coef,
+                                                            float *__restrict__ losses, const int *__restrict__ err, const int *__restrict__ single,
+                                                            unsigned terms) {
+    using Y = LossLay<ND>;
+    constexpr int NS = Y::SUMS;
+    const bool plain = !(terms & CDNET_LOSS_WMAP);
+    __shared__ float s_sum[64 * NS];
+    __shared__ float s_term[LossTerms<ND>::NT];
+    const int tid = threadIdx.x;
+    loss_all_sums<ND>(partial, nchunk, B, sums, s_sum, tid);
+    __syncthreads();
+    const float fB = (float)B;
+    for (int b = tid; b < B; b += 256) loss_sample_coef<ND>(s_sum + b * NS, fB, plain, coef + (size_t)b * Y::COEF);
+    loss_write_losses<ND>(s_sum, s_term, B, P, losses, tid == 0 ? loss_err_flag(err, single, B) : 0, terms, tid);
+}
+
+template <int ND>
+__device__ __forceinline__ void loss_grad_pixels(const LossIn &L, const float *cf, int b, int i0, int step, float *__restrict__ dmask,
+                                                 float *__restrict__ dpoint, float *__restrict__ ddir) {
     const float inv_n = 1.f / ((float)L.B * (float)L.P);
     const size_t ob = (size_t)b * L.P;
-    for (int i = blockIdx.x * 256 + threadIdx.x; i < L.P; i += gridDim.x * 256) {
+    for (int i = i0; i < L.P; i += step) {
         float l3[3], p3[3], lp3[3], l9[ND], p9[ND], lp9[ND];
 #pragma unroll
         for (int c = 0; c < 3; ++c) l3[c] = L.mask[((size_t)b * 3 + c) * L.P + i];
@@ -253,6 +281,38 @@
             ddir[((size_t)b * ND + c) * L.P + i] = p9[c] * (gq[c] - dotq) + w * inv_n * (p9[c] - (c == dl ? 1.f : 0.f));
         if (dpoint) dpoint[ob + i] = 2.f * inv_n * (L.point[ob + i] - h2f(L.point_t[ob + i]));
     }
+}
+
+template <int ND>
+__global__ __launch_bounds__(256) void loss_grad_kernel(LossIn L, const float *__restrict__ coef, float *__restrict__ dmask,
+                                                        float *__restrict__ dpoint, float *__restrict__ ddir) {
+    const int b = blockIdx.y;
+    loss_grad_pixels<ND>(L, coef + (size_t)b * LossLay<ND>::COEF, b, blockIdx.x * 256 + threadIdx.x, gridDim.x * 256, dmask, dpoint, ddir);
+}
+
+template <int ND>
+__global__ __launch_bounds__(256) void loss_grad_fin_kernel(LossIn L, const float *__restrict__ partial, int nchunk, float *__restrict__ sums,
+                                                            float *__restrict__ coef, float *__restrict__ losses, float *__restrict__ dmask,
+                                                            float *__restrict__ dpoint, float *__restrict__ ddir) {
+    using Y = LossLay<ND>;
+    constexpr int NS = Y::SUMS;
+    __shared__ float s_sum[64 * NS];
+    __shared__ float s_term[LossTerms<ND>::NT];
+    __shared__ float s_cf[Y::COEF];
+    const int tid = threadIdx.x, b = blockIdx.y, gx = (int)gridDim.x - 1;
+    if ((int)blockIdx.x == gx) {
+        if (b != 0) return;
+        loss_all_sums<ND>(partial, nchunk, L.B, sums, s_sum, tid);
+        __syncthreads();
+        loss_write_losses<ND>(s_sum, s_term, L.B, L.P, losses, tid == 0 ? loss_err_flag(nullptr, L.single, L.B) : 0, L.terms, tid);
+        return;
+    }
+    if (tid < NS) s_sum[tid] = chunk_sum<NS>(partial + (size_t)b * nchunk * NS + tid, nchunk);
+    __syncthreads();
+    if (tid == 0) loss_sample_coef<ND>(s_sum, (float)L.B, !(L.terms & CDNET_LOSS_WMAP), s_cf);
+    __syncthreads();
+    if (blockIdx.x == 0 && tid < Y::COEF) coef[(size_t)b * Y::COEF + tid] = s_cf[tid];
+    loss_grad_pixels<ND>(L, s_cf, b, blockIdx.x * 256 + tid, gx * 256, dmask, dpoint, ddir);
 }
 
 template <int ND> struct ValLay {
@@ -347,12 +407,23 @@
     float *sums = coef + (size_t)B * Y::COEF;
     int *err = reinterpret_cast<int *>(sums + (size_t)B * Y::SUMS);
     int *single = reinterpret_cast<int *>(sums + (size_t)B * Y::SUMS + 16);
-    if (hipMemsetAsync(err, 0, sizeof(int), st) != hipSuccess) return check_launch("cdnet_dam_loss(memset)");
     L.single = single;
-    loss_single_kernel<<<B, 1024, 0, st>>>(L.dirlab, L.label, P, ND, single, err);
+    const char *five = getenv("CDNET_LOSS_FIVE_LAUNCH");
+    if (five && atoi(five) != 0) {
+        if (hipMemsetAsync(err, 0, sizeof(int), st) != hipSuccess) return check_launch("cdnet_dam_loss(memset)");
+        loss_single_kernel<<<B, 1024, 0, st>>>(L.dirlab, L.label, P, ND, single, err);
+        loss_reduce_kernel<ND><<<dim3(nchunk, B), Y::TPB, 0, st>>>(L, partial);
+        loss_finalize_kernel<ND><<<1, 256, 0, st>>>(partial, nchunk, B, P, sums, coef, losses, err, single, L.terms);
+        if (dmask) loss_grad_kernel<ND><<<dim3(lin_grid((size_t)P, 256), B), 256, 0, st>>>(L, coef, dmask, dpoint, ddir);
+        return check_launch("cdnet_dam_loss");
+    }
+    loss_single_kernel<<<B, 1024, 0, st>>>(L.dirlab, L.label, P, ND, single, nullptr);
     loss_reduce_kernel<ND><<<dim3(nchunk, B), Y::TPB, 0, st>>>(L, partial);
-    loss_finalize_kernel<ND><<<1, 256, 0, st>>>(partial, nchunk, B, P, sums, coef, losses, err, L.terms);
-    if (dmask) loss_grad_kernel<ND><<<dim3(lin_grid((size_t)P, 256), B), 256, 0, st>>>(L, coef, dmask, dpoint, ddir);
+    if (dmask) {
+        loss_grad_fin_kernel<ND><<<dim3(lin_grid((size_t)P, 64) + 1, B), 256, 0, st>>>(L, partial, nchunk, sums, coef, losses, dmask, dpoint, ddir);
+    } else {
+        loss_finalize_kernel<ND><<<1, 256, 0, st>>>(partial, nchunk, B, P, sums, coef, losses, nullptr, single, L.terms);
+    }
     return check_launch("cdnet_dam_loss");
 }
 
diff --git a/cdnet_amd/engine.py b/cdnet_amd/engine.py
--- a/cdnet_amd/engine.py
+++ b/cdnet_amd/engine.py
@@ -191,7 +191,7 @@
 
 def conv_forward(srcs, wpacked, Cout, cfg, taps=9, transposed=False, bias=None, oscale=None, oshift=None,
                  orelu=False, out=None, stats=None, H=None, W=None, out_dtype=torch.bfloat16, eres=None, query_ws=False, bns=None, taps1=0, pool_out=None, dot=None,
-                 pad_chunks=0, debug_or=0):
+                 pad_chunks=0, debug_or=0, pool_sign=None):
     tile, CK, BN = cfg[:3]
     s0 = srcs[0]
     f32 = s0.f32
@@ -232,6 +232,9 @@
     a.ws = 0
     a.taps1 = taps1
     a.pool_out = _dp(pool_out)
+    if pool_sign is not None:
+        assert pool_out is not None and stats is not None and eres is None and bns is None and pool_sign.dtype == torch.float32 and pool_sign.numel() == Cout
+        a.eres_scale = pool_sign.data_ptr()
     a.debug = CONV_DEBUG | debug_or
     a.f32 = int(f32)
     assert out is None or (out.dtype == torch.float32) == f32
diff --git a/cdnet_amd/models/dam/model_unet_rev1.py b/cdnet_amd/models/dam/model_unet_rev1.py
--- a/cdnet_amd/models/dam/model_unet_rev1.py
+++ b/cdnet_amd/models/dam/model_unet_rev1.py
@@ -199,7 +199,8 @@
                 if not training and idx + 1 < len(enc) and enc[idx + 1][0] == 'pool' and not getattr(runtime, 'DEBUG_NORELU', False):
                     t, tp = layer.forward_eval_pool([t])
                 else:
-                    t = layer.forward([t], training)
+                    t = layer.forward([t], training, pool_raw=training and idx + 1 < len(enc) and enc[idx + 1][0] == 'pool')
+                    tp = getattr(t, 'pooled_raw', None)
             else:
                 t, tp = (tp if tp is not None else pooled(t)), None
             if out_name in self.shortcut_features:
diff --git a/cdnet_amd/runtime.py b/cdnet_amd/runtime.py
--- a/cdnet_amd/runtime.py
+++ b/cdnet_amd/runtime.py
@@ -213,7 +213,18 @@
                 return Src(out), Src(pout)
         return self.forward(srcs, False), None
 
-    def forward(self, srcs, training, relu=True, H=None, W=None, out_dtype=None, eres=None, debug_or=0):
+    def _pool_raw_eligible(self, srcs, N, H, W):
+        if PRECISION != 'fp32' or not POOL_RAW or self.bn is None or self.transposed or self.taps != 9 or H % 2 or W % 2:
+            return False
+        key = (N, H, W, tuple((s.C, s.scale is not None, bool(s.relu), s.res is not None, tuple(s.off), s.Hs, s.Ws) for s in srcs), engine.CONV_DEBUG)
+        elig = self.__dict__.setdefault('_pool_raw_elig', {})
+        if key not in elig:
+            praw = torch.empty((N, H // 2, W // 2, self.Cout), dtype=torch.float32, device=self.weight.device)
+            elig[key] = engine.conv_forward(srcs, self.wp, self.Cout, self.cfg, self.taps, self.transposed, stats=self.stats, H=H, W=W,
+                                            out_dtype=raw_dtype(), pool_out=praw, pool_sign=self.bn.weight.detach(), query_ws=True) == 1
+        return elig[key]
+
+    def forward(self, srcs, training, relu=True, H=None, W=None, out_dtype=None, eres=None, debug_or=0, pool_raw=False):
         if PRECISION == 'fp32':
             out_dtype = torch.float32
         elif out_dtype is None:
@@ -249,8 +260,12 @@
         T = N * npar * ((H + tile - 1) // tile) * ((W + tile - 1) // tile)
         if self.stats is None or self.stats.shape[0] != T:
             self.stats = torch.empty((T, 2, self.Cout), dtype=torch.float32, device=self.weight.device)
+        praw = None
+        if pool_raw and self._pool_raw_eligible(srcs, N, H, W):
+            praw = torch.empty((N, H // 2, W // 2, self.Cout), dtype=torch.float32, device=self.weight.device)
+        kw = {} if praw is None else dict(pool_out=praw, pool_sign=self.bn.weight.detach())
         raw, _ = engine.conv_forward(srcs, self.wp, self.Cout, self.cfg, self.taps, self.transposed, stats=self.stats,
-                                     H=H, W=W, out_dtype=raw_dtype())
+                                     H=H, W=W, out_dtype=raw_dtype(), **kw)
         count = float(N * H * W * npar)
         bn = self.bn
         _lib.call('cdnet_bn_finalize_train', _lib.ptr(self.stats), T, self.Cout, count, _lib.ptr(bn.weight.detach()),
@@ -263,7 +278,11 @@
         self.fold_version = None
         if TAPE is not None:
             TAPE.append(self)
-        return Src(raw, self.scale, self.shift, relu=relu)
+        out = Src(raw, self.scale, self.shift, relu=relu)
+        if praw is not None:
+            out.pooled_raw = Src(praw, self.scale, self.shift, relu=relu)
+            out.pooled_raw.grad_to = (raw, 1)
+        return out
 
 
 class FuseTerm(C.Structure):
@@ -382,6 +401,7 @@
     return out
 
 
+POOL_RAW = _os.environ.get('CDNET_POOL_RAW', '1') != '0'
 POOL_MATERIALIZE = True
 RU_MATERIALIZE = True
 RU_FUSE = True
diff --git a/cdnet_amd/trainer.py b/cdnet_amd/trainer.py
--- a/cdnet_amd/trainer.py
+++ b/cdnet_amd/trainer.py
@@ -26,6 +26,7 @@
 _WGRAD_WGS_F32 = 160
 _RU_1X1_SIDE = True
 WGRAD_STREAM = True
+DBETA_TWICE = True
 HEAD_BWD_FUSE = True
 _WGRAD_DEFER = 0x100
 _WGRAD_DEEP_HW = 16384
@@ -461,8 +462,13 @@
         draw = self.buf(('draw', L.name), (No, Ho, Wo, Co), runtime.act_dtype())
         ws = self._ws('bn', _lib.load().cdnet_bn_backward_workspace_floats(Co))
         bn = L.bn
-        _lib.call('cdnet_bn_backward', C.byref(a), _lib.ptr(bn.weight.detach()), _lib.ptr(bn.weight.grad), _lib.ptr(bn.bias.grad),
-                  _lib.ptr(ws), ws.numel(), _lib.ptr(draw), None, _lib.stream_ptr())
+        dbias = self._dbias_of(L)
+        if dbias is not None:
+            _lib.call('cdnet_bn_backward_dbias', C.byref(a), _lib.ptr(bn.weight.detach()), _lib.ptr(bn.weight.grad), _lib.ptr(bn.bias.grad),
+                      _lib.ptr(dbias), _lib.ptr(ws), ws.numel(), _lib.ptr(draw), None, _lib.stream_ptr())
+        else:
+            _lib.call('cdnet_bn_backward', C.byref(a), _lib.ptr(bn.weight.detach()), _lib.ptr(bn.weight.grad), _lib.ptr(bn.bias.grad),
+                      _lib.ptr(ws), ws.numel(), _lib.ptr(draw), None, _lib.stream_ptr())
         add(L.node_res, _G(g.t, Ho, Wo))
         return draw
 
@@ -531,13 +537,28 @@
             dz = self.buf(('dz', L.name), (No, Ho, Wo, Co), runtime.act_dtype())
         ws = self._ws('bn', _lib.load().cdnet_bn_backward_workspace_floats(Co))
         bn = L.bn
-        _lib.call('cdnet_bn_backward', C.byref(a), _lib.ptr(bn.weight.detach()) if has_bn else None,
-                  _lib.ptr(bn.weight.grad) if has_bn else None, _lib.ptr(bn.bias.grad) if has_bn else None,
-                  _lib.ptr(ws), ws.numel(), _lib.ptr(draw), _lib.ptr(dz), _lib.stream_ptr())
+        dbias = self._dbias_of(L) if has_bn else None
+        if dbias is not None:
+            _lib.call('cdnet_bn_backward_dbias', C.byref(a), _lib.ptr(bn.weight.detach()), _lib.ptr(bn.weight.grad), _lib.ptr(bn.bias.grad),
+                      _lib.ptr(dbias), _lib.ptr(ws), ws.numel(), _lib.ptr(draw), _lib.ptr(dz), _lib.stream_ptr())
+        else:
+            _lib.call('cdnet_bn_backward', C.byref(a), _lib.ptr(bn.weight.detach()) if has_bn else None,
+                      _lib.ptr(bn.weight.grad) if has_bn else None, _lib.ptr(bn.bias.grad) if has_bn else None,
+                      _lib.ptr(ws), ws.numel(), _lib.ptr(draw), _lib.ptr(dz), _lib.stream_ptr())
         if res is not None:
             add(getattr(L, 'node_res_grad_to', None) if getattr(L, 'node_res_grad_to', None) is not None else res, _G(dz, Ho, Wo))
             L.node_res_grad_to = None
         return draw
+
+    def _dbias_of(self, L):
+        if not DBETA_TWICE:
+            return None
+        for Lt in self.tape:
+            if getattr(Lt, 'bias_grad_from', None) is L and Lt.bias is not None and Lt.bn is None and Lt.bias.grad is not None \
+                    and Lt.bias.grad.dtype == torch.float32 and Lt.bias.grad.numel() == L.Cout:
+                Lt._dbias_written = True
+                return Lt.bias.grad
+        return None
 
     def _side_stream(self):
         if not WGRAD_STREAM or self.dev.type != 'cuda':
@@ -586,7 +607,8 @@
         if L.bias is not None and L.bn is None:
             owner = getattr(L, 'bias_grad_from', None)
             if owner is not None:
-                L.bias.grad.copy_(owner.bn.bias.grad)
+                if not L.__dict__.pop('_dbias_written', False):
+                    L.bias.grad.copy_(owner.bn.bias.grad)
             else:
                 ws = self._ws('slab', lib.cdnet_bias_grad_workspace_floats(Cout), side=True)
                 _lib.call(_lib.entry('cdnet_bias_grad', g.dtype == torch.float32), _lib.ptr(g), g.numel() // Cout, Cout,
diff --git a/include/cdnet_hip.h b/include/cdnet_hip.h
--- a/include/cdnet_hip.h
+++ b/include/cdnet_hip.h
@@ -213,6 +213,8 @@
                                int nb, float *ktab, void *stream);
 int cdnet_bn_backward(const cdnet_bn_bwd_args *args, const float *gamma, float *dgamma, float *dbeta, float *workspace,
                       size_t workspace_floats, uint16_t *draw, uint16_t *dz_out, void *stream);
+int cdnet_bn_backward_dbias(const cdnet_bn_bwd_args *args, const float *gamma, float *dgamma, float *dbeta, float *dbias, float *workspace,
+                            size_t workspace_floats, uint16_t *draw, uint16_t *dz_out, void *stream);
 
 size_t cdnet_dam_head_backward_workspace_floats(int N, int H, int W);
 int cdnet_dam_head_backward(const cdnet_head_feat *f1, const cdnet_head_feat *f2, const cdnet_head_feat *f3,
```
